# EDAPINENUT/CBGBench

Measured on AMD Instinct MI355X. Metric: denoising graph-steps/s (pocket+ligand graphs x reverse-diffusion steps per second), higher is better.
Workload: dtype f32; 1 GPU; configs/denovo targetdiff sampling, BASELINE configs[1] job: 100 pockets x 10 samples = 1000 graphs per GPU, 3 resident batch(es) of <= 340; N_rec~U[350,650], N_lig~U[10,45], k=32, 9 layers; bench step = 1 reverse-diffusion step of the job at each of 5 time blocks; graphs_per_gpu=1000, nodes_per_gpu=521351, denoising_steps_per_bench_step=5, graph_steps_per_bench_step_per_gpu=5000, ranks_seen=1, launch=stream launches, streams=3, edge_workgroups=256, devices_by_uuid=1

## Files before the change

cbgbench_amd/_native.py:

```python
import contextlib
import contextvars
import ctypes
import os

import torch

from .build import LIBPATH, XCHECK_LIBPATH

_LIB = None
_XLIB = None

_vp, _i, _sz = ctypes.c_void_p, ctypes.c_int, ctypes.c_size_t
FWD_H_ON_SOURCES, FWD_GEN_IS_LIGAND = 1, 2
ABI_VERSION = 6

EXPORTS = {
    "cbgx_abi_version": (_i, []),
    "cbgx_last_error": (ctypes.c_char_p, []),
    "cbgx_set_edge_workgroups": (_i, [_i]),
    "cbgx_packed_weights_floats": (_sz, [_i, _i]),
    "cbgx_pack_weights": (_i, [ctypes.POINTER(_vp), _i, _i, _i, _vp, _vp]),
    "cbgx_workspace_bytes": (_sz, [_i, _i]),
    "cbgx_unitransformer_forward": (_i, [_vp, _i, _i, _vp, _vp, _vp, _vp, _vp, _i, _i, _vp, _vp, _vp, _vp, _sz, _vp]),
    "cbgx_unitransformer_forward_v2": (_i, [_vp, _i, _i, _vp, _vp, _vp, _vp, _vp, _i, _i, _vp, _vp, _vp, ctypes.c_uint, _vp, _sz, _vp]),
    "cbgx_unitransformer_forward_cached": (_i, [_vp, _i, _i, _vp, _vp, _vp, _vp, _vp, _i, _i, _vp, _vp, _vp, _vp, _vp, _vp,
                                                _vp, _vp, _vp, ctypes.c_uint, _vp, _sz, _vp]),
    "cbgx_knn_graph": (_i, [_vp, _vp, _i, _i, _i, _vp, _vp, _vp]),
    "cbgx_edge_gate": (_i, [_vp, _vp, _vp, _vp, _i, _vp, _vp]),
    "cbgx_x2h_attention": (_i, [_vp, _i, _vp, _vp, _vp, _vp, _vp, _vp, _i, _vp, _vp, _sz, _vp]),
    "cbgx_h2x_attention": (_i, [_vp, _i, _vp, _vp, _vp, _vp, _vp, _vp, _vp, _i, _vp, _vp, _vp, _sz, _vp]),
    "cbgx_h2x_attention_v2": (_i, [_vp, _i, _vp, _vp, _vp, _vp, _vp, _vp, _vp, _i, _vp, _vp, ctypes.c_uint, _vp, _sz, _vp]),
    "cbgx_classifier": (_i, [_vp, _i, _i, _vp, _i, _vp, _vp, _sz, _vp]),
    "cbgx_node_stage": (_i, [_vp, _i, _i, _vp, _vp, _i, _vp, _vp, _i, _vp, _vp, _vp, _vp]),
    "cbgx_packed_h2x_stack_floats": (_sz, [_i]),
    "cbgx_pack_h2x_stack": (_i, [ctypes.POINTER(_vp), _i, _i, _vp, _vp]),
    "cbgx_h2x_stack_forward": (_i, [_vp, _i, _vp, _vp, _vp, _vp, _vp, _i, _i, _vp, _vp, _sz, _vp]),
    "cbgx_h2x_stack_forward_v2": (_i, [_vp, _i, _vp, _vp, _vp, _vp, _vp, _i, _i, _vp, ctypes.c_uint, _vp, _sz, _vp]),
    "cbgx_targetdiff_prologue": (_i, [_vp, _vp, _vp, _i, _i, _vp, _vp, _vp, _vp, _vp, _vp, _vp]),
    "cbgx_targetdiff_epilogue": (_i, [_vp, _vp, _vp, _vp, _vp, _vp, _i, _i, _i, _i, ctypes.POINTER(_vp), _vp, _vp, _vp, _vp,
                                      _vp, _vp]),
    "cbgx_targetdiff_step_boundary": (_i, [_vp, _vp, _vp, _vp, _vp, _vp, _i, _i, _i, _i, ctypes.POINTER(_vp), _vp, _vp, _vp, _vp,
                                           _vp, _vp, _vp, _vp, _vp, _vp, _vp]),
    "cbgx_targetdiff_prologue_traj": (_i, [_vp, _vp, _vp, _vp, _i, _i, _vp, _vp, _vp, _vp, _vp, _vp, _vp]),
    "cbgx_targetdiff_epilogue_traj": (_i, [_vp, _vp, _vp, _vp, _vp, _vp, _i, _i, _vp, ctypes.POINTER(_vp), _vp, _vp, _vp]),
    "cbgx_diffbp_epilogue": (_i, [_vp, _vp, _vp, _vp, _vp, _vp, _vp, _vp, _vp, _i, _i, _i, _i, _i, _vp, _vp, _i, _vp, _vp, _vp,
                                  _vp, _vp]),
    "cbgx_diffsbdd_step": (_i, [_vp, _vp, _vp, _vp, _vp, _vp, _vp, _vp, _i, _i, _i, ctypes.c_float, ctypes.c_float,
                                ctypes.c_float, _i, _i, _vp, _vp, _vp, _vp, _vp, _vp, _vp, _vp, _vp, _vp, _vp, _vp, _vp]),
    "cbgx_noise_fill": (_i, [_vp, _vp, _i, _i, _i, _i, _i, _i, _vp, _vp, _vp]),
    "cbgx_targetdiff_epilogue_rng": (_i, [_vp, _vp, _vp, _vp, _vp, _vp, _i, _i, _i, _i, ctypes.POINTER(_vp), _vp, _vp, _vp, _i, _i,
                                          _vp, _vp, _vp, _vp]),
    "cbgx_targetdiff_step_boundary_rng": (_i, [_vp, _vp, _vp, _vp, _vp, _vp, _i, _i, _i, _i, ctypes.POINTER(_vp), _vp, _vp, _vp, _i,
                                               _i, _vp, _vp, _vp, _vp, _vp, _vp, _vp, _vp, _vp]),
    "cbgx_targetdiff_epilogue_traj_rng": (_i, [_vp, _vp, _vp, _vp, _vp, _vp, _i, _i, _vp, ctypes.POINTER(_vp), _vp, _vp, _vp, _i, _i,
                                               _vp]),
    "cbgx_targetdiff_train_noise": (_i, [_vp, _vp, _vp, _vp, _vp, _i, _i, _vp, _vp, _vp, _vp, _vp, _vp, _vp, _vp, _vp]),
    "cbgx_train_noise_draw": (_i, [_vp, _vp, _i, _i, _i, _i, _vp, _vp, _vp, _vp, _i, _i, _i, _vp]),
    "cbgx_targetdiff_train_noise_rng": (_i, [_vp, _vp, _vp, _vp, _i, _i, _vp, _vp, _vp, _vp, _vp, _i, _i, _i, _vp, _vp, _vp, _vp, _vp,
                                             _vp]),
    "cbgx_train_transform": (_i, [_vp] * 5 + [_i, _i, _i, ctypes.c_float, _i, _vp] + [_vp] * 4),
    "cbgx_train_transform_rng": (_i, [_vp] * 5 + [_i, _i, _i, ctypes.c_float, _i, _vp, _i] + [_vp] * 4),
    "cbgx_train_transform_choose": (_i, [_vp] * 8 + [_i] * 5 + [ctypes.c_float, _i, _vp] + [_vp] * 6),
    "cbgx_train_transform_choose_rng": (_i, [_vp] * 7 + [_i] * 5 + [ctypes.c_float, _i, _vp, _i] + [_vp] * 6),
    "cbgx_targetdiff_loss": (_i, [_vp, _vp, _vp, _vp, _vp, _vp, _vp, _vp, _vp, _i, _i, _i, ctypes.POINTER(_vp), _vp, _vp, _vp,
                                  _vp, _vp, _vp]),
    "cbgx_targetdiff_loss_backward": (_i, [_vp, _vp, _vp, _i, _i, _i, _vp, _vp, _vp, _vp, _vp]),
    "cbgx_diffsbdd_train_noise": (_i, [_vp] * 9 + [_i] * 4 + [_vp, _vp, _i] + [_vp] * 5),
    "cbgx_diffsbdd_loss": (_i, [_vp] * 7 + [_i] * 4 + [_vp] * 8),
    "cbgx_compose_plan": (_i, [_vp, _vp, _i, _i, _i] + [_vp] * 7),
    "cbgx_embed_compose": (_i, [_vp] * 8 + [_i] * 5 + [ctypes.POINTER(_vp)] + [_vp] * 5),
    "cbgx_embed_compose_backward": (_i, [_vp, _vp, _i, _i, _i, _i, _vp, _i, _vp, _vp]),
    "cbgx_diffbp_loss": (_i, [_vp] * 13 + [_i, _i, _i, _i, _vp, _vp, ctypes.c_float, ctypes.c_float] + [_vp] * 9 + [_vp]),
    "cbgx_diffbp_loss_knn": (_i, [_vp] * 13 + [_i, _i, _i, _i, _vp, _vp, ctypes.c_float, ctypes.c_float] + [_vp] * 9 + [_vp, _vp]),
    "cbgx_diffbp_train_noise": (_i, [_vp] * 8 + [_i] * 4 + [_vp, _i, _i] + [_vp] * 6 + [_vp]),
    "cbgx_train_tape_bytes": (_sz, [_i, _i]),
    "cbgx_train_workspace_bytes": (_sz, [_i]),
    "cbgx_unitransformer_forward_train": (_i, [_vp, _i, _i, _vp, _vp, _vp, _vp, _vp, _i, _i, _vp, _vp, _vp, _vp, _sz,
                                               _vp, _sz, _vp]),
    "cbgx_unitransformer_forward_train_ex": (_i, [_vp, _i, _i, _vp, _vp, _vp, _vp, _vp, _i, _i, _vp, _vp, _vp, ctypes.c_uint, _vp, _sz,
                                                  _vp, _sz, _vp]),
    "cbgx_unitransformer_backward": (_i, [_vp, _i, _i, _vp, _sz, _vp, _vp, _i, _vp, _vp, _vp, ctypes.POINTER(_vp), _i,
                                          _vp, _vp, _sz, _vp]),
    "cbgx_unitransformer_backward_ex": (_i, [_vp, _i, _i, _vp, _sz, _vp, _vp, _i, _vp, _vp, _vp, ctypes.POINTER(_vp), _i,
                                             _vp, _vp, _vp, _sz, _vp]),
    "cbgx_x2h_attention_backward": (_i, [_vp, _i, _vp, _vp, _vp, _vp, _vp, _vp, _i, _vp, _vp, _vp, _vp,
                                         ctypes.POINTER(_vp), _vp, _sz, _vp]),
    "cbgx_h2x_attention_backward": (_i, [_vp, _i, _vp, _vp, _vp, _vp, _vp, _vp, _vp, _i, _vp, _vp, _vp, _vp,
                                         ctypes.POINTER(_vp), _vp, _sz, _vp]),
    "cbgx_h2x_stack_tape_bytes": (_sz, [_i, _i]),
    "cbgx_h2x_stack_forward_train": (_i, [_vp, _i, _vp, _vp, _vp, _vp, _vp, _i, _i, _vp, _vp, _sz, _vp, _sz, _vp]),
    "cbgx_h2x_stack_backward": (_i, [_vp, _i, _vp, _sz, _vp, _vp, _vp, _i, _vp, ctypes.POINTER(_vp), _i, _vp, _vp, _sz,
                                     _vp]),
    "cbgx_h2x_stack_backward_ex": (_i, [_vp, _i, _vp, _sz, _vp, _vp, _vp, _i, _vp, ctypes.POINTER(_vp), _i, _vp, _vp, _vp,
                                        _sz, _vp]),
    "cbgx_ligand_geometry": (_i, [_vp, _vp, _vp, _i, _vp, _vp, _vp, _i, _i, _vp, _vp, _vp, _vp]),
    "cbgx_ligand_geometry_tables": (_i, [_vp] * 7),
    "cbgx_ligand_bonds_count": (_i, [_vp, _vp, _vp, _i, _i, _vp, _vp, _vp, _vp]),
    "cbgx_ligand_bonds_fill": (_i, [_vp, _vp, _vp, _i, _i, _vp, _i, _vp, _vp, _vp, _vp]),
    "cbgx_ligand_rings": (_i, [_vp, _i, _i, _vp, _vp, _i, _vp, _vp, _vp]),
    "cbgx_ligand_aromatic": (_i, [_vp, _vp, _vp, _vp, _i, _i, _vp, _vp, _i, _vp, _vp, _vp, _vp]),
    "cbgx_ligand_pair_hist": (_i, [_vp, _vp, _vp, _i, _i, _vp, _i, _vp, _i, _vp, _vp]),
    "cbgx_ligand_angles": (_i, [_vp, _vp, _vp, _i, _i, _vp, _vp, _vp, _i, _vp, _i, _vp, _i, _vp, _vp, _vp, _vp, _vp]),
    "cbgx_profile_begin": (_i, [_i]),
    "cbgx_profile_end": (_i, [ctypes.POINTER(ctypes.c_double), ctypes.POINTER(_i), _i]),
}

XCHECK_EXPORTS = {
    "cbgx_debug_set_edge_kernel": (_i, [_i]),
    "cbgx_debug_gate_backward": (_i, [_vp, _vp, _vp, _vp, _i, _vp, _vp, _vp, ctypes.POINTER(_vp), _vp, _vp, _sz, _vp]),
    "cbgx_debug_forward_view": (_i, [_vp, _i, ctypes.POINTER(_vp)]),
}

PROFILE_CLASSES = ("knn", "gate", "node_gemm", "node_query", "edge_x2h", "edge_h2x", "edge_x2h_listed",
                   "edge_x2h_bwd", "edge_h2x_bwd", "train_gemm", "edge_x2h_bwd_listed", "edge_rows_reduce")


class NativeError(RuntimeError):
    pass


def _load(path, extra=None):
    dll = ctypes.CDLL(path)
    exports = dict(EXPORTS)
    exports.update(extra or {})
    for name, (res, args) in exports.items():
        fn = getattr(dll, name)
        fn.restype = res
        fn.argtypes = args
    if dll.cbgx_abi_version() != ABI_VERSION:
        raise NativeError(f"{path}: ABI version {dll.cbgx_abi_version()} != {ABI_VERSION} (stale build? run `python -m cbgbench_amd.build`)")
    return dll


_OVERRIDE = contextvars.ContextVar("cbgx_library_override", default=None)


def lib():
    global _LIB
    over = _OVERRIDE.get()
    if over is not None:
        return over
    if _LIB is None:
        path = os.environ.get("CBGX_LIBRARY", LIBPATH)
        if not os.path.exists(path):
            raise NativeError(
                f"{path} not found: build it with `python -m cbgbench_amd.build` "
                "(there is no CPU / PyTorch fallback for the message-passing path)")
        _LIB = _load(path)
    return _LIB


@contextlib.contextmanager
def first_generation_kernels(impl=1):
    global _XLIB
    if _XLIB is None:
        if not os.path.exists(XCHECK_LIBPATH):
            raise NativeError(f"{XCHECK_LIBPATH} not found: build it with `python -m cbgbench_amd.build`")
        _XLIB = _load(XCHECK_LIBPATH, XCHECK_EXPORTS)
    old = _XLIB.cbgx_debug_set_edge_kernel(impl)
    token = _OVERRIDE.set(_XLIB)
    try:
        yield _XLIB
    finally:
        _OVERRIDE.reset(token)
        _XLIB.cbgx_debug_set_edge_kernel(old)


def check(rc, what):
    if rc != 0:
        msg = lib().cbgx_last_error().decode(errors="replace")
        if rc == -1:
            raise ValueError(f"{what}: {msg}")
        raise NativeError(f"{what} failed ({rc}): {msg}")


def ptr(t):
    if t is None:
        return None
    if not t.is_contiguous():
        raise ValueError("libcbgx needs contiguous tensors")
    return ctypes.c_void_p(t.data_ptr())


def current_stream(device):
    return ctypes.c_void_p(torch.cuda.current_stream(device).cuda_stream)



def version(t):
    if t.is_inference():
        return _NeverEqual()
    return t._version


class _NeverEqual:
    __slots__ = ()

    def __eq__(self, other):
        return False

    def __ne__(self, other):
        return True

    def __hash__(self):
        return id(self)
```

cbgbench_amd/csrc/api.hip:

```cpp
#include <hip/hip_runtime.h>

#include <cmath>
#include <cstdarg>
#include <cstdio>
#include <cstring>
#include <cstdlib>
#include <vector>

#include "../../include/cbgx.h"
#ifdef CBGX_XCHECK
#include "../../include/cbgx_xcheck.h"
#endif
#include "kernels.h"
#include "layout.h"
#include "workspace.h"

using namespace cbgx;

static thread_local char g_err[512] = "";

namespace cbgx {
int set_error(int code, const char* fmt, ...) {
    va_list ap;
    va_start(ap, fmt);
    vsnprintf(g_err, sizeof(g_err), fmt, ap);
    va_end(ap);
    return code;
}
}
static constexpr auto& fail = cbgx::set_error;

#define HIP_TRY(expr)                                                                          \
    do {                                                                                       \
        hipError_t _e = (expr);                                                                \
        if (_e != hipSuccess) return fail(CBGX_E_HIP, "%s: %s", #expr, hipGetErrorString(_e)); \
    } while (0)

struct Workspace {
    int32_t *nbr, *deg;
    float* e_w;
    NodeBufs set[3];
    NodeList act;
    NodeList A1, A2, A3;
    NodeList D1, S1, D2, S2;
    NodeList all_gen, all_pp, D2_gen, D2_pp, A1_gen, A1_pp, A2_gen, A2_pp;
    NodeList empty;
    uint8_t *fa1, *fa2, *fa3, *fD1, *fD2, *fS1, *fS2;
    uint8_t* d1flag;
    float *hbuf[2], *xbuf[2];
    unsigned* newmask;
    void* counters;
    size_t counters_bytes, total;
};

static Workspace carve(void* base, int n) {
    Workspace w;
    Carver c(base);
    size_t N = (size_t)(n > 0 ? n : 1);
    w.nbr = c.take<int32_t>(N * KNN * 4);
    w.deg = c.take<int32_t>(N * 4);
    w.e_w = c.take<float>(N * KNN * 4);
    for (NodeBufs& b : w.set) {
        b.P = c.take<float>(N * PROW * 4);
        b.Qt = c.take<float>(N * HEADS * H * 4);
        b.q = c.take<float>(N * H * 4);
    }
    for (NodeList* l : {&w.act, &w.A1, &w.A2, &w.A3, &w.D1, &w.S1, &w.D2, &w.S2}) l->rows = c.take<int>(N * 4);
    for (float*& h : w.hbuf) h = c.take<float>(N * H * 4);
    for (float*& x : w.xbuf) x = c.take<float>(N * 3 * 4);
    for (NodeList* l : {&w.all_gen, &w.all_pp, &w.D2_gen, &w.D2_pp, &w.A1_gen, &w.A1_pp, &w.A2_gen, &w.A2_pp})
        l->rows = c.take<int>(N * 4);
    w.empty.rows = w.all_pp.rows;
    w.newmask = c.take<unsigned>(N * 4);
    const size_t fl = align_up(N);
    w.counters_bytes = 8 * fl + 256 + 256 + 256 + 4 * 128 + 256;
    uint8_t* f = c.take<uint8_t>(w.counters_bytes);
    w.counters = f;
    w.d1flag = f; w.fa1 = w.d1flag + fl; w.fa2 = w.fa1 + fl; w.fa3 = w.fa2 + fl;
    w.fD1 = w.fa3 + fl; w.fD2 = w.fD1 + fl; w.fS1 = w.fD2 + fl; w.fS2 = w.fS1 + fl;
    auto counts = [&](size_t region, std::initializer_list<NodeList*> lists) {
        int k = 0;
        for (NodeList* l : lists) l->count = (int*)(f + 8 * fl + region + 64 * k++);
    };
    counts(0, {&w.act});
    counts(256, {&w.A1, &w.A2, &w.A3});
    counts(512, {&w.D1, &w.S1, &w.D2, &w.S2});
    counts(768, {&w.all_gen, &w.all_pp, &w.D2_gen, &w.D2_pp, &w.A1_gen, &w.A1_pp, &w.A2_gen, &w.A2_pp});
    counts(768 + 4 * 128, {&w.empty});
    w.total = c.off;
    return w;
}

static int carve_checked(const char* who, void* workspace, size_t workspace_bytes, int n_nodes, Workspace& w) {
    w = carve(workspace, n_nodes);
    if (workspace_bytes < w.total) return fail(CBGX_E_WORKSPACE, "%s: workspace %zu < %zu", who, workspace_bytes, w.total);
    return CBGX_OK;
}

constexpr int MAX_AUX = 8;
struct AuxTable {
    int dev = -1;
    int n = 0;
    int next_victim = 0;
    AuxStream e[MAX_AUX];
};
static thread_local AuxTable g_aux_table;
namespace cbgx {
AuxStream* aux_for(hipStream_t caller) {
    int dev = -1;
    if (hipGetDevice(&dev) != hipSuccess) return nullptr;
    AuxTable& t = g_aux_table;
    if (t.n && t.dev != dev) return nullptr;
    for (int k = 0; k < t.n; ++k)
        if (t.e[k].owner == caller) return &t.e[k];
    if (t.n == MAX_AUX) {
        AuxStream& e = t.e[t.next_victim];
        t.next_victim = (t.next_victim + 1) % MAX_AUX;
        e.owner = caller;
        return &e;
    }
    AuxStream a;
    a.owner = caller;
    static const bool low = [] { const char* e = getenv("CBGX_AUX_PRIORITY"); return e && e[0] == 'l'; }();
    int least = 0, greatest = 0;
    if (low && hipDeviceGetStreamPriorityRange(&least, &greatest) == hipSuccess && least != greatest) {
        if (hipStreamCreateWithPriority(&a.s, hipStreamNonBlocking, least) != hipSuccess) return nullptr;
    } else if (hipStreamCreateWithFlags(&a.s, hipStreamNonBlocking) != hipSuccess) return nullptr;
    if (hipEventCreateWithFlags(&a.fork, hipEventDisableTiming) != hipSuccess ||
        hipEventCreateWithFlags(&a.join, hipEventDisableTiming) != hipSuccess ||
        hipEventCreateWithFlags(&a.done[0], hipEventDisableTiming) != hipSuccess ||
        hipEventCreateWithFlags(&a.done[1], hipEventDisableTiming) != hipSuccess) {
        (void)hipStreamDestroy(a.s);
        return nullptr;
    }
    t.dev = dev;
    t.e[t.n] = a;
    return &t.e[t.n++];
}
}

extern "C" {

int cbgx_abi_version(void) { return CBGX_ABI_VERSION; }
const char* cbgx_last_error(void) { return g_err; }

#ifdef CBGX_XCHECK
int cbgx_debug_set_edge_kernel(int impl) {
    if (impl < 0 || impl > 2) return fail(CBGX_E_INVALID, "debug_set_edge_kernel: impl must be 0 (current), 1 (valu) or 2 (mfma, second-generation x2h backward)");
    int old = g_edge_impl;
    g_edge_impl = impl;
    return old;
}

int cbgx_debug_forward_view(void* workspace, int n_nodes, void** out) {
    if (!workspace || !out || n_nodes < 1) return fail(CBGX_E_INVALID, "debug_forward_view: bad argument");
    const Workspace w = carve(workspace, n_nodes);
    int k = 0;
    out[k++] = w.nbr; out[k++] = w.deg; out[k++] = w.e_w; out[k++] = w.d1flag; out[k++] = w.fD1;
    const NodeList lists[] = {w.act,     w.A1,     w.A2,     w.A3,    w.D1,     w.S1,    w.D2,     w.S2,
                              w.all_gen, w.all_pp, w.D2_gen, w.D2_pp, w.A1_gen, w.A1_pp, w.A2_gen, w.A2_pp};
    for (const NodeList& l : lists) { out[k++] = l.rows; out[k++] = l.count; }
    static_assert(sizeof(lists) / sizeof(lists[0]) == CBGX_FWD_VIEW_LISTS, "cbgx_debug_forward_view: list count");
    static_assert(CBGX_FWD_VIEW_PTRS == 5 + 2 * 16, "cbgx_debug_forward_view: list count");
    return k == CBGX_FWD_VIEW_PTRS ? CBGX_OK : fail(CBGX_E_INVALID, "debug_forward_view: %d pointers", k);
}
#endif

int cbgx_set_edge_workgroups(int n) { return set_edge_workgroup_limit(n); }

size_t cbgx_packed_weights_floats(int num_layers, int num_classes) {
    if (num_layers < 0 || num_classes < 1 || num_classes > CBGX_MAX_CLASSES) return 0;
    return packed_floats(num_layers, num_classes);
}

static thread_local PackBatch g_pack;
static int flush_pack(hipStream_t s) {
    if (g_pack.n) {
        HIP_TRY(launch_pack_copy_multi(g_pack, s));
        g_pack.n = 0;
    }
    return CBGX_OK;
}
static int queue_pack(const float* src, int ld, int off, int tr, float* dst, int dld, int rows, int cols, hipStream_t s) {
    if (g_pack.n == PACK_MAX) { int rc = flush_pack(s); if (rc) return rc; }
    g_pack.p[g_pack.n++] = PackPiece{src, dst, ld, off, tr, dld, rows, cols};
    return CBGX_OK;
}
#define CP(src, ld, off, tr, dst, dld, rows, cols)                                 \
    do {                                                                           \
        int _rc = queue_pack(src, ld, off, tr, dst, dld, rows, cols, s);           \
        if (_rc) return _rc;                                                       \
    } while (0)

static int pack_gate_section(const float* const* t, float* packed, hipStream_t s) {
    CP(t[0], G, 0, 0, packed + GATE_W1, G, GH, G);
    CP(t[1], GH, 0, 0, packed + GATE_B1, GH, 1, GH);
    CP(t[2], GH, 0, 0, packed + GATE_LNG, GH, 1, GH);
    CP(t[3], GH, 0, 0, packed + GATE_LNB, GH, 1, GH);
    CP(t[4], GH, 0, 0, packed + GATE_W2, GH, 1, GH);
    CP(t[5], 1, 0, 0, packed + GATE_B2, 1, 1, 1);
    HIP_TRY(launch_pack_gate_img(t[0], t[1], t[2], t[3], t[4], packed + GATE_IMG, s));
    return flush_pack(s);
}

struct BlockRef { const float* const* p; int blk; float* a; };

static int queue_block_copies(const BlockRef& r, hipStream_t s) {
    const float* const* p = r.p;
    float* a = r.a;
    const int blk = r.blk;
    const float *wk0 = p[0], *bk0 = p[1], *gk = p[2], *bek = p[3], *wk1 = p[4];
    const float *wv0 = p[6], *bv0 = p[7], *gv = p[8], *bev = p[9], *wv1 = p[10], *bv1 = p[11];
    const float *wq0 = p[12], *bq0 = p[13], *gq = p[14], *beq = p[15], *wq1 = p[16], *bq1 = p[17];
    CP(wk0, KV_IN, NT + NT * G, 1, a + A_WN + 0 * H, PROW, H, H);
    CP(wv0, KV_IN, NT + NT * G, 1, a + A_WN + 1 * H, PROW, H, H);
    CP(wk0, KV_IN, NT + NT * G + H, 1, a + A_WN + 2 * H, PROW, H, H);
    CP(wv0, KV_IN, NT + NT * G + H, 1, a + A_WN + 3 * H, PROW, H, H);
    CP(wq0, H, 0, 1, a + A_WN + 4 * H, PROW, H, H);
    CP(bk0, H, 0, 0, a + A_BN + 0 * H, H, 1, H);
    CP(bv0, H, 0, 0, a + A_BN + 1 * H, H, 1, H);
    CP(bq0, H, 0, 0, a + A_BN + 4 * H, H, 1, H);
    CP(wk0, KV_IN, 0, 1, a + A_WT, 2 * H, NT, H);
    CP(wv0, KV_IN, 0, 1, a + A_WT + H, 2 * H, NT, H);
    CP(wk0, KV_IN, NT, 1, a + A_WR, 2 * H, NT * G, H);
    CP(wv0, KV_IN, NT, 1, a + A_WR + H, 2 * H, NT * G, H);
    CP(gk, H, 0, 0, a + A_LNK_G, H, 1, H);
    CP(bek, H, 0, 0, a + A_LNK_B, H, 1, H);
    CP(gv, H, 0, 0, a + A_LNV_G, H, 1, H);
    CP(bev, H, 0, 0, a + A_LNV_B, H, 1, H);
    CP(gq, H, 0, 0, a + A_LNQ_G, H, 1, H);
    CP(beq, H, 0, 0, a + A_LNQ_B, H, 1, H);
    CP(wq1, H, 0, 1, a + A_WQ1T, H, H, H);
    CP(bq1, H, 0, 0, a + A_BQ1, H, 1, H);
    CP(wk1, H, 0, 0, a + A_WBK, H, H, H);
    CP(wk1, H, 0, 1, a + A_WBKT, H, H, H);
    CP(wq1, H, 0, 0, a + A_WQ1O, H, H, H);
    for (int ty = 0; ty < NT; ++ty) {
        CP(wk0, KV_IN, NT + G * ty, 0, a + A_WRT + (size_t)ty * 2 * H * 32, 32, H, G);
        CP(wv0, KV_IN, NT + G * ty, 0, a + A_WRT + ((size_t)ty * 2 * H + H) * 32, 32, H, G);
    }
    float* img = a + A_IMG;
    CP(gk, H, 0, 0, img + IMG_LN + 0 * H, H, 1, H);
    CP(bek, H, 0, 0, img + IMG_LN + 1 * H, H, 1, H);
    CP(gv, H, 0, 0, img + IMG_LN + 2 * H, H, 1, H);
    CP(bev, H, 0, 0, img + IMG_LN + 3 * H, H, 1, H);
    if (blk == 0) {
        CP(wv1, H, 0, 1, a + A_WBV, H, H, H);
        CP(bv1, H, 0, 0, a + A_BBV, H, 1, H);
    } else {
        CP(wv1, H, 0, 0, a + A_WBV, H, HEADS, H);
        CP(bv1, HEADS, 0, 0, a + A_BBV, HEADS, 1, HEADS);
    }
    return CBGX_OK;
}

static int queue_centred_copies(const BlockRef& r, hipStream_t s) {
    float* a = r.a;
    CP(a + A_WAKC, KV_IN, NT, 1, a + A_WRC, 2 * H, NT * G, H);
    CP(a + A_WAVC, KV_IN, NT, 1, a + A_WRC + H, 2 * H, NT * G, H);
    return CBGX_OK;
}

static int pack_attention_blocks(const BlockRef* refs, int n_blocks, hipStream_t s) {
    for (int k0 = 0; k0 < n_blocks; k0 += PACK_BLOCKS_MAX) {
        const int nb = n_blocks - k0 < PACK_BLOCKS_MAX ? n_blocks - k0 : PACK_BLOCKS_MAX;
        PackBlocks pb;
        memset(&pb, 0, sizeof(pb));
        pb.n = nb;
        for (int k = 0; k < nb; ++k) {
            const BlockRef& r = refs[k0 + k];
            pb.wk0[k] = r.p[0]; pb.bk0[k] = r.p[1]; pb.wk1[k] = r.p[4];
            pb.wv0[k] = r.p[6]; pb.bv0[k] = r.p[7]; pb.wv1[k] = r.p[10];
            pb.wq0[k] = r.p[12]; pb.bq0[k] = r.p[13]; pb.wq1[k] = r.p[16];
            pb.att[k] = r.a;
            pb.nsrc[k][0] = r.a + A_WAKC; pb.nsrc[k][1] = r.a + A_WAVC; pb.nsrc[k][2] = r.a + A_WAKC; pb.nsrc[k][3] = r.a + A_WAVC;
            pb.nsrc[k][4] = r.p[12];
            pb.x2h[k] = r.blk == 0;
            int rc = queue_block_copies(r, s);
            if (rc) return rc;
        }
        { int rc = flush_pack(s); if (rc) return rc; }
        HIP_TRY(launch_pack_stage1(pb, s));
        for (int k = 0; k < nb; ++k) { int rc = queue_centred_copies(refs[k0 + k], s); if (rc) return rc; }
        { int rc = flush_pack(s); if (rc) return rc; }
        HIP_TRY(launch_pack_stage2(pb, s));
    }
    return CBGX_OK;
}

int cbgx_pack_weights(const float* const* t, int num_tensors, int L, int C, float* packed, void* stream) {
    if (C > CBGX_MAX_CLASSES) return fail(CBGX_E_INVALID, "pack_weights: num_classes=%d > %d", C, CBGX_MAX_CLASSES);
    if (!t || !packed) return fail(CBGX_E_INVALID, "pack_weights: NULL pointer");
    if (L < 1 || C < 1) return fail(CBGX_E_INVALID, "pack_weights: num_layers=%d num_classes=%d", L, C);
    if (num_tensors != 6 + 36 * L + 4)
        return fail(CBGX_E_INVALID, "pack_weights: expected %d tensors, got %d", 6 + 36 * L + 4, num_tensors);
    for (int i = 0; i < num_tensors; ++i)
        if (!t[i]) return fail(CBGX_E_INVALID, "pack_weights: tensor %d is NULL", i);
    hipStream_t s = (hipStream_t)stream;
    HIP_TRY(hipMemsetAsync(packed, 0, packed_floats(L, C) * sizeof(float), s));
    { int rc = pack_gate_section(t, packed, s); if (rc) return rc; }
    {
        std::vector<BlockRef> refs;
        for (int l = 0; l < L; ++l)
            for (int blk = 0; blk < 2; ++blk)
                refs.push_back(BlockRef{t + 6 + 36 * l + 18 * blk , blk, packed + (blk == 0 ? x2h_off(l) : h2x_off(l))});
        int rc = pack_attention_blocks(refs.data(), (int)refs.size(), s);
        if (rc) return rc;
    }
    const float* const* c = t + 6 + 36 * L;
    float* cp = packed + cls_off(L);
    CP(c[0], H, 0, 1, cp + C_W0T, H, H, H);
    CP(c[1], H, 0, 0, cp + C_B0, H, 1, H);
    CP(c[2], H, 0, 1, cp + C_W1T, C, H, C);
    CP(c[3], C, 0, 0, cp + cls_b1(C), C, 1, C);
    return flush_pack(s);
}

size_t cbgx_packed_h2x_stack_floats(int num_layers) {
    if (num_layers < 1) return 0;
    return GATE_SIZE + (size_t)num_layers * ATT_SIZE;
}

int cbgx_pack_h2x_stack(const float* const* t, int num_tensors, int L, float* packed, void* stream) {
    if (!t || !packed) return fail(CBGX_E_INVALID, "pack_h2x_stack: NULL pointer");
    if (L < 1 || num_tensors != 6 + 18 * L)
        return fail(CBGX_E_INVALID, "pack_h2x_stack: expected %d tensors for %d layers, got %d", 6 + 18 * L, L, num_tensors);
    for (int i = 0; i < num_tensors; ++i)
        if (!t[i]) return fail(CBGX_E_INVALID, "pack_h2x_stack: tensor %d is NULL", i);
    hipStream_t s = (hipStream_t)stream;
    HIP_TRY(hipMemsetAsync(packed, 0, cbgx_packed_h2x_stack_floats(L) * sizeof(float), s));
    { int rc = pack_gate_section(t, packed, s); if (rc) return rc; }
    std::vector<BlockRef> refs;
    for (int l = 0; l < L; ++l) refs.push_back(BlockRef{t + 6 + 18 * l, 1, packed + GATE_SIZE + (size_t)l * ATT_SIZE});
    { int rc = pack_attention_blocks(refs.data(), (int)refs.size(), s); if (rc) return rc; }
    return flush_pack(s);
}

static bool h2x_lig_selected(unsigned flags) { return (flags & CBGX_FWD_GEN_IS_LIGAND) && g_edge_impl != 1 && h2x_fold_enabled(); }

int cbgx_h2x_stack_forward_v2(const float* packed, int num_layers, const float* x, const float* h,
                              const int32_t* graph_ptr, const uint8_t* lig_flag, const uint8_t* gen_flag, int n_nodes,
                              int n_graphs, float* x_out, unsigned flags, void* workspace, size_t workspace_bytes, void* stream) {
    if (n_nodes < 0 || n_graphs < 0 || num_layers < 1) return fail(CBGX_E_INVALID, "h2x_stack: bad sizes");
    if (flags & ~CBGX_FWD_GEN_IS_LIGAND) return fail(CBGX_E_INVALID, "h2x_stack: unknown flags 0x%x", flags);
    if (n_nodes == 0) return CBGX_OK;
    if (!packed || !x || !h || !graph_ptr || !lig_flag || !gen_flag || !x_out || !workspace)
        return fail(CBGX_E_INVALID, "h2x_stack: NULL pointer");
    Workspace w;
    if (int rc = carve_checked("h2x_stack", workspace, workspace_bytes, n_nodes, w)) return rc;
    hipStream_t s = (hipStream_t)stream;
    HIP_TRY(launch_build_active(gen_flag, n_nodes, w.act, s));
    if (g_edge_impl == 1) {
        HIP_TRY(launch_knn(x, graph_ptr, n_graphs, n_nodes, w.nbr, w.deg, s));
        HIP_TRY(launch_gate(packed, x, w.nbr, w.deg, n_nodes, w.e_w, s));
    } else {
        HIP_TRY(launch_knn_reg(x, graph_ptr, n_graphs, n_nodes, w.nbr, w.deg, s, w.act));
        HIP_TRY(launch_gate_mfma(packed, x, w.nbr, w.deg, n_nodes, w.e_w, s, w.act));
    }
    RowList src;
    if (g_edge_impl != 1) {
        HIP_TRY(launch_mark_seed(gen_flag, gen_flag, n_nodes, w.fa1, s));
        HIP_TRY(walk_receptive_field(w.fa1, w.act, w.nbr, w.deg, n_nodes, {w.A1}, s));
        src = w.A1;
    }
    const Graph g{w.nbr, w.deg, w.e_w, lig_flag, gen_flag, n_nodes};
    const float* xc = x;
    for (int l = 0; l < num_layers; ++l) {
        float* xn = (l == num_layers - 1) ? x_out : w.xbuf[l & 1];
        HIP_TRY(launch_attention(false, packed + GATE_SIZE + (size_t)l * ATT_SIZE, g, xc, h, w.set[0], xn, nullptr, w.act, src, s,
                                 h2x_lig_selected(flags)));
        xc = xn;
    }
    return CBGX_OK;
}

int cbgx_h2x_stack_forward(const float* packed, int num_layers, const float* x, const float* h,
                           const int32_t* graph_ptr, const uint8_t* lig_flag, const uint8_t* gen_flag, int n_nodes,
                           int n_graphs, float* x_out, void* workspace, size_t workspace_bytes, void* stream) {
    return cbgx_h2x_stack_forward_v2(packed, num_layers, x, h, graph_ptr, lig_flag, gen_flag, n_nodes, n_graphs, x_out, 0u, workspace,
                                     workspace_bytes, stream);
}

size_t cbgx_workspace_bytes(int n_nodes, int n_graphs) {
    (void)n_graphs;
    return carve(nullptr, n_nodes).total;
}

int cbgx_knn_graph(const float* x, const int32_t* graph_ptr, int n_graphs, int n_nodes, int k, int32_t* nbr,
                   int32_t* deg, void* stream) {
    if (k != KNN) return fail(CBGX_E_INVALID, "knn_graph: only k=%d is supported (got %d)", KNN, k);
    if (n_nodes < 0 || n_graphs < 0) return fail(CBGX_E_INVALID, "knn_graph: negative size");
    if (n_nodes == 0) return CBGX_OK;
    if (!x || !graph_ptr || !nbr || !deg || n_graphs < 1) return fail(CBGX_E_INVALID, "knn_graph: NULL pointer");
    HIP_TRY(launch_knn(x, graph_ptr, n_graphs, n_nodes, nbr, deg, (hipStream_t)stream));
    return CBGX_OK;
}

int cbgx_edge_gate(const float* packed, const float* x, const int32_t* nbr, const int32_t* deg, int n_nodes,
                   float* e_w, void* stream) {
    if (n_nodes == 0) return CBGX_OK;
    if (!packed || !x || !nbr || !deg || !e_w || n_nodes < 0) return fail(CBGX_E_INVALID, "edge_gate: bad argument");
    HIP_TRY(launch_gate(packed, x, nbr, deg, n_nodes, e_w, (hipStream_t)stream));
    return CBGX_OK;
}

int cbgx_x2h_attention(const float* packed, int layer, const float* x, const float* h, const int32_t* nbr,
                       const int32_t* deg, const uint8_t* lig_flag, const float* e_w, int n_nodes, float* h_out,
                       void* workspace, size_t workspace_bytes, void* stream) {
    if (n_nodes == 0) return CBGX_OK;
    if (!packed || !x || !h || !nbr || !deg || !lig_flag || !e_w || !h_out || !workspace || layer < 0 || n_nodes < 0)
        return fail(CBGX_E_INVALID, "x2h_attention: bad argument");
    Workspace w;
    if (int rc = carve_checked("x2h_attention", workspace, workspace_bytes, n_nodes, w)) return rc;
    const NodeBufs& b = w.set[0];
    const Graph g{nbr, deg, e_w, lig_flag, nullptr, n_nodes};
    const float* att = packed + x2h_off(layer);
    hipStream_t s = (hipStream_t)stream;
    if (g_edge_impl == 1) {
        HIP_TRY(launch_attention(true, att, g, x, h, b, h_out, nullptr, {}, {}, s));
        return CBGX_OK;
    }
    HIP_TRY(launch_mark_from_nbr(lig_flag, nbr, deg, n_nodes, w.d1flag, s));
    HIP_TRY(launch_split_list({}, n_nodes, w.d1flag, w.all_gen, w.all_pp, s));
    NodeStageOpts o;
    o.large_lists = true;
    o.fold = w.all_gen;
    HIP_TRY(launch_node_mfma(att, h, lig_flag, n_nodes, b, {}, {}, s, o));
    HIP_TRY(launch_edge_x2h_dual(att, g, x, h, b, h_out, w.all_pp, w.all_gen, true, s));
    return CBGX_OK;
}

int cbgx_h2x_attention_v2(const float* packed, int layer, const float* x, const float* h, const int32_t* nbr,
                          const int32_t* deg, const uint8_t* lig_flag, const uint8_t* gen_flag, const float* e_w,
                          int n_nodes, float* x_out, float* delta_x, unsigned flags, void* workspace, size_t workspace_bytes,
                          void* stream) {
    if (flags & ~CBGX_FWD_GEN_IS_LIGAND) return fail(CBGX_E_INVALID, "h2x_attention: unknown flags 0x%x", flags);
    if (n_nodes == 0) return CBGX_OK;
    if (!packed || !x || !h || !nbr || !deg || !lig_flag || !gen_flag || !e_w || !x_out || !workspace || layer < 0 ||
        n_nodes < 0)
        return fail(CBGX_E_INVALID, "h2x_attention: bad argument");
    Workspace w;
    if (int rc = carve_checked("h2x_attention", workspace, workspace_bytes, n_nodes, w)) return rc;
    const Graph g{nbr, deg, e_w, lig_flag, gen_flag, n_nodes};
    HIP_TRY(launch_build_active(gen_flag, n_nodes, w.act, (hipStream_t)stream));
    HIP_TRY(launch_attention(false, packed + h2x_off(layer), g, x, h, w.set[0], x_out, delta_x, w.act, {}, (hipStream_t)stream,
                             h2x_lig_selected(flags)));
    return CBGX_OK;
}

int cbgx_h2x_attention(const float* packed, int layer, const float* x, const float* h, const int32_t* nbr,
                       const int32_t* deg, const uint8_t* lig_flag, const uint8_t* gen_flag, const float* e_w,
                       int n_nodes, float* x_out, float* delta_x, void* workspace, size_t workspace_bytes,
                       void* stream) {
    return cbgx_h2x_attention_v2(packed, layer, x, h, nbr, deg, lig_flag, gen_flag, e_w, n_nodes, x_out, delta_x, 0u, workspace,
                                 workspace_bytes, stream);
}

int cbgx_node_stage(const float* packed, int layer, int x2h, const float* h, const uint8_t* lig_flag, int n_nodes,
                    const int32_t* rows, const int32_t* n_rows, int q_direct, float* P, float* q, float* Qt, void* stream) {
    if (n_nodes == 0) return CBGX_OK;
    if (!packed || !h || !lig_flag || !P || !q || !Qt || layer < 0 || n_nodes < 0 || (rows == nullptr) != (n_rows == nullptr))
        return fail(CBGX_E_INVALID, "node_stage: bad argument");
    NodeStageOpts o;
    o.large_lists = true;
    o.q_direct = q_direct != 0;
    HIP_TRY(launch_node_mfma(packed + (x2h ? x2h_off(layer) : h2x_off(layer)), h, lig_flag, n_nodes, NodeBufs{P, q, Qt},
                             RowList{rows, n_rows}, {}, (hipStream_t)stream, o));
    return CBGX_OK;
}

static int classifier_head(const float* packed, int num_layers, int num_classes, const float* h, int n_nodes, float* hidden,
                           float* logits, RowList rows, hipStream_t s) {
    const float* c = packed + cls_off(num_layers);
    HIP_TRY(launch_node_gemm(h, H, c + C_W0T, c + C_B0, hidden, H, n_nodes, H, 1, s, rows));
    HIP_TRY(launch_node_gemm(hidden, H, c + C_W1T, c + cls_b1(num_classes), logits, num_classes, n_nodes, num_classes, 0, s, rows));
    return CBGX_OK;
}

int cbgx_classifier(const float* packed, int num_layers, int num_classes, const float* h, int n_nodes, float* logits,
                    void* workspace, size_t workspace_bytes, void* stream) {
    if (num_classes > CBGX_MAX_CLASSES) return fail(CBGX_E_INVALID, "classifier: num_classes=%d > %d", num_classes, CBGX_MAX_CLASSES);
    if (n_nodes == 0) return CBGX_OK;
    if (!packed || !h || !logits || !workspace || num_layers < 0 || num_classes < 1 || n_nodes < 0)
        return fail(CBGX_E_INVALID, "classifier: bad argument");
    Workspace w;
    if (int rc = carve_checked("classifier", workspace, workspace_bytes, n_nodes, w)) return rc;
    return classifier_head(packed, num_layers, num_classes, h, n_nodes, w.set[0].P, logits, {}, (hipStream_t)stream);
}

struct LayerPlan {
    NodeList dst, src;
    NodeList gen, pp;
    bool full_layer;
    const uint8_t* fold_flag;
};

struct Forward {
    const float* packed; int num_layers, num_classes; const float *x, *h; const int32_t* graph_ptr; const uint8_t *lig_flag, *gen_flag;
    int n_nodes, n_graphs; float *x_out, *h_out, *logits;
    const float *static_h1, *static_h2; const int32_t *static_nbr, *static_deg; const float *static_ew, *static_r32sq;
    unsigned flags; void* workspace; size_t workspace_bytes; hipStream_t s;
    Workspace w;
    Graph graph;
    bool cached, graph_cached, prune, dual;
    bool h2x_lig;
    std::vector<LayerPlan> plan;
};

static int forward_graph_stage(const Forward& f) {
    const Workspace& w = f.w;
    const int n_nodes = f.n_nodes, n_graphs = f.n_graphs;
    hipStream_t s = f.s;
    if (!f.graph_cached) {
        HIP_TRY(launch_knn(f.x, f.graph_ptr, n_graphs, n_nodes, w.nbr, w.deg, s));
        HIP_TRY(launch_gate(f.packed, f.x, w.nbr, w.deg, n_nodes, w.e_w, s));
        return CBGX_OK;
    }
    HIP_TRY(launch_graph_cache_begin(f.x, f.graph_ptr, n_graphs, f.lig_flag, f.static_r32sq, n_nodes, w.fD1, w.D1.rows, w.D1.count,
                                     f.static_nbr, f.static_deg, f.static_ew, w.nbr, w.deg, w.e_w, f.static_h1, f.static_h2, w.hbuf[0],
                                     w.hbuf[1], s));
    static const int merge_gate = [] { const char* e = getenv("CBGX_MERGE_GATE"); return e ? atoi(e) : 1; }();
    if (merge_gate && n_nodes <= GRAPH_LISTS_MAX_NODES) {
        HIP_TRY(launch_knn_merge_gate(f.packed, f.x, f.graph_ptr, n_graphs, n_nodes, f.lig_flag, f.static_nbr, f.static_deg, f.static_ew,
                                      w.nbr, w.deg, w.e_w, s, w.D1));
    } else {
        const bool carry = merge_gate != 0;
        HIP_TRY(launch_knn_merge(f.x, f.graph_ptr, n_graphs, n_nodes, f.lig_flag, f.static_nbr, f.static_deg, w.nbr, w.deg, s, w.D1,
                                 carry ? f.static_ew : nullptr, carry ? w.e_w : nullptr, carry ? w.newmask : nullptr));
        HIP_TRY(launch_gate_mfma(f.packed, f.x, w.nbr, w.deg, n_nodes, w.e_w, s, w.D1, carry ? w.newmask : nullptr));
    }
    return CBGX_OK;
}

static int forward_list_stage(const Forward& f) {
    const Workspace& w = f.w;
    hipStream_t s = f.s;
    const bool per_graph = f.n_nodes <= GRAPH_LISTS_MAX_NODES && g_edge_impl != 1;
    const GraphFlags gf{f.gen_flag, f.lig_flag, f.graph_cached ? w.fD1 : w.d1flag, w.d1flag, w.fa1, w.fa2, w.fa3, w.fD2, w.fS1, w.fS2};
    const uint8_t* flag_ptr[GF_COUNT] = {f.gen_flag, f.lig_flag, gf.D1, w.d1flag, w.fa1, w.fa2, w.fa3, w.fD2, w.fS1, w.fS2};
    ListJobs jobs;
    GraphListJobs gjobs;
    memset(&jobs, 0, sizeof(jobs));
    memset(&gjobs, 0, sizeof(gjobs));
    bool jobs_overflow = false;
    auto add = [&](int flag, int flag2, int want2, NodeList l) {
        if (jobs.n_jobs >= LIST_JOBS_MAX) { jobs_overflow = true; return; }
        const int k = jobs.n_jobs++;
        jobs.flag[k] = flag == GF_ALL ? nullptr : flag_ptr[flag]; jobs.flag2[k] = flag2 == GF_ALL ? nullptr : flag_ptr[flag2];
        jobs.want2[k] = want2; jobs.list[k] = l.rows; jobs.count[k] = l.count;
        gjobs.flag[k] = (signed char)flag; gjobs.flag2[k] = (signed char)flag2; gjobs.want2[k] = (signed char)want2;
        gjobs.list[k] = l.rows; gjobs.count[k] = l.count;
        gjobs.n_jobs = jobs.n_jobs;
    };
    auto pair = [&](int flag, NodeList gen, NodeList pp) { add(flag, GF_d1, 1, gen); add(flag, GF_d1, 0, pp); };
    add(GF_GEN, GF_ALL, 0, w.act);
    add(GF_a1, GF_ALL, 0, w.A1);
    if (f.prune) {
        add(GF_a2, GF_ALL, 0, w.A2);
        add(GF_a3, GF_ALL, 0, w.A3);
    }
    if (f.cached) {
        if (!f.graph_cached) add(GF_d1, GF_ALL, 0, w.D1);
        add(GF_D2, GF_ALL, 0, w.D2);
        add(GF_S1, GF_ALL, 0, w.S1);
        add(GF_S2, GF_ALL, 0, w.S2);
    }
    if (f.dual) {
        pair(GF_ALL, w.all_gen, w.all_pp);
        if (f.cached) pair(GF_D2, w.D2_gen, w.D2_pp);
        if (f.prune) { pair(GF_a1, w.A1_gen, w.A1_pp); pair(GF_a2, w.A2_gen, w.A2_pp); }
    }
    if (jobs_overflow) return fail(CBGX_E_INVALID, "forward: more than %d node lists (LIST_JOBS_MAX)", LIST_JOBS_MAX);
    if (per_graph) {
        HIP_TRY(launch_graph_lists(f.gen_flag, f.lig_flag, f.graph_cached ? w.fD1 : nullptr, w.nbr, w.deg, f.graph_ptr, f.n_graphs, gjobs,
                                   f.cached, f.prune, w.d1flag, s));
    } else {
        HIP_TRY(launch_list_level(gf, w.nbr, w.deg, f.n_nodes, 0, f.cached, f.prune, s));
        if (f.cached || f.prune) {
            HIP_TRY(launch_list_level(gf, w.nbr, w.deg, f.n_nodes, 1, f.cached, f.prune, s));
            HIP_TRY(launch_list_level(gf, w.nbr, w.deg, f.n_nodes, 2, f.cached, f.prune, s));
        }
        HIP_TRY(launch_build_lists(jobs, f.n_nodes, s));
    }
    return CBGX_OK;
}

static void plan_layers(Forward& f) {
    const Workspace& w = f.w;
    const int L = f.num_layers;
    const NodeList every{nullptr, nullptr};
    f.plan.assign(L, LayerPlan{every, every, w.all_gen, w.all_pp, true, w.d1flag});
    if (f.cached) {
        f.plan[0] = LayerPlan{w.D1, w.S1, w.D1, w.empty, false, nullptr};
        f.plan[1] = LayerPlan{w.D2, w.S2, w.D2_gen, w.D2_pp, false, w.d1flag};
    }
    if (f.prune) {
        f.plan[L - 2] = LayerPlan{w.A2, w.A3, w.A2_gen, w.A2_pp, false, w.d1flag};
        f.plan[L - 1] = LayerPlan{w.A1, w.A2, w.A1_gen, w.A1_pp, false, w.d1flag};
    }
}

static hipError_t begin_layer(const Forward& f, int l, float*& hn, float*& xn) {
    const bool last = l == f.num_layers - 1;
    hn = (last && f.h_out) ? f.h_out : f.w.hbuf[l & 1];
    xn = last ? f.x_out : f.w.xbuf[l & 1];
    if (!f.cached || l >= 2 || f.graph_cached) return hipSuccess;
    return hipMemcpyAsync(hn, l == 0 ? f.static_h1 : f.static_h2, (size_t)f.n_nodes * H * sizeof(float), hipMemcpyDeviceToDevice, f.s);
}

static hipError_t edge_x2h(const Forward& f, int l, const NodeBufs& b, const float* xc, const float* hc, float* hn) {
    const LayerPlan& p = f.plan[l];
    return launch_edge_x2h_dual(f.packed + x2h_off(l), f.graph, xc, hc, b, hn, p.pp, p.gen, p.full_layer, f.s);
}
static hipError_t node_x2h(const Forward& f, int l, const NodeBufs& b, const float* h_in, hipStream_t on) {
    const LayerPlan& p = f.plan[l];
    NodeStageOpts o;
    o.large_lists = true;
    o.fold = p.gen;
    o.q_direct = node_qdirect_enabled();
    return launch_node_mfma(f.packed + x2h_off(l), h_in, f.lig_flag, f.n_nodes, b, p.dst, p.src, on, o);
}
static hipError_t block_h2x(const Forward& f, int l, const NodeBufs& b, const float* xc, const float* hn, float* xn) {
    return launch_attention(false, f.packed + h2x_off(l), f.graph, xc, hn, b, xn, nullptr, f.w.act, f.w.A1, f.s, f.h2x_lig);
}

static int forward_fused(const Forward& f) {
    const Workspace& w = f.w;
    hipStream_t s = f.s;
    auto add_x2h = [&](NodeStageJobs& jobs, int l) {
        const LayerPlan& p = f.plan[l];
        add_node_stage_jobs(jobs, f.packed + x2h_off(l), w.set[l & 1], p.dst, p.src, p.fold_flag);
    };
    NodeStageJobs jobs;
    jobs.n = 0;
    add_x2h(jobs, 0);
    HIP_TRY(launch_node_stage_jobs(jobs, f.h, f.lig_flag, f.n_nodes, s));
    const float *xc = f.x, *hc = f.h;
    for (int l = 0; l < f.num_layers; ++l) {
        float *hn, *xn;
        HIP_TRY(begin_layer(f, l, hn, xn));
        HIP_TRY(edge_x2h(f, l, w.set[l & 1], xc, hc, hn));
        jobs.n = 0;
        add_node_stage_jobs(jobs, f.packed + h2x_off(l), w.set[2], w.act, w.A1, nullptr, f.h2x_lig);
        if (l + 1 < f.num_layers) add_x2h(jobs, l + 1);
        HIP_TRY(launch_node_stage_jobs(jobs, hn, f.lig_flag, f.n_nodes, s));
        if (f.h2x_lig) HIP_TRY(launch_edge_h2x_lig(f.packed + h2x_off(l), f.graph, xc, hn, w.set[2], xn, nullptr, w.act, s));
        else HIP_TRY(launch_edge_mfma(false, f.packed + h2x_off(l), f.graph, xc, hn, w.set[2], xn, nullptr, w.act, s));
        xc = xn;
        hc = hn;
    }
    return CBGX_OK;
}

static int forward_two_streams(const Forward& f, AuxStream* aux) {
    hipStream_t s = f.s;
    HIP_TRY(node_x2h(f, 0, f.w.set[0], f.h, s));
    const float *xc = f.x, *hc = f.h;
    for (int l = 0; l < f.num_layers; ++l) {
        float *hn, *xn;
        HIP_TRY(begin_layer(f, l, hn, xn));
        if (l > 0) HIP_TRY(hipStreamWaitEvent(s, aux->join, 0));
        HIP_TRY(edge_x2h(f, l, f.w.set[l & 1], xc, hc, hn));
        if (l + 1 < f.num_layers) {
            HIP_TRY(hipEventRecord(aux->fork, s));
            HIP_TRY(hipStreamWaitEvent(aux->s, aux->fork, 0));
            HIP_TRY(node_x2h(f, l + 1, f.w.set[(l + 1) & 1], hn, aux->s));
            HIP_TRY(hipEventRecord(aux->join, aux->s));
        }
        HIP_TRY(block_h2x(f, l, f.w.set[2], xc, hn, xn));
        xc = xn;
        hc = hn;
    }
    return CBGX_OK;
}

static int forward_serial(const Forward& f) {
    const Workspace& w = f.w;
    const NodeBufs& b = w.set[0];
    const float *xc = f.x, *hc = f.h;
    for (int l = 0; l < f.num_layers; ++l) {
        float *hn, *xn;
        HIP_TRY(begin_layer(f, l, hn, xn));
        if (f.dual) {
            HIP_TRY(node_x2h(f, l, b, hc, f.s));
            HIP_TRY(edge_x2h(f, l, b, xc, hc, hn));
        } else {
            const LayerPlan& p = f.plan[l];
            HIP_TRY(launch_attention(true, f.packed + x2h_off(l), f.graph, xc, hc, b, hn, nullptr, p.dst, p.src, f.s));
        }
        HIP_TRY(block_h2x(f, l, b, xc, hn, xn));
        xc = xn;
        hc = hn;
    }
    return CBGX_OK;
}

static int forward_impl(Forward f) {
    if (f.n_nodes < 0 || f.n_graphs < 0 || f.num_layers < 1) return fail(CBGX_E_INVALID, "forward: bad sizes");
    if (f.flags & ~(CBGX_FWD_H_ON_SOURCES | CBGX_FWD_GEN_IS_LIGAND)) return fail(CBGX_E_INVALID, "forward: unknown flags 0x%x", f.flags);
    if (f.num_classes > CBGX_MAX_CLASSES) return fail(CBGX_E_INVALID, "forward: num_classes=%d > %d", f.num_classes, CBGX_MAX_CLASSES);
    if (f.n_nodes == 0) return CBGX_OK;
    if (!f.packed || !f.x || !f.h || !f.graph_ptr || !f.lig_flag || !f.gen_flag || !f.x_out || !f.workspace)
        return fail(CBGX_E_INVALID, "forward: NULL pointer");
    if (f.logits && f.num_classes < 1) return fail(CBGX_E_INVALID, "forward: num_classes=%d", f.num_classes);
    if (int rc = carve_checked("forward", f.workspace, f.workspace_bytes, f.n_nodes, f.w)) return rc;
    f.graph = Graph{f.w.nbr, f.w.deg, f.w.e_w, f.lig_flag, f.gen_flag, f.n_nodes};
    HIP_TRY(hipMemsetAsync(f.w.counters, 0, f.w.counters_bytes, f.s));
    f.cached = f.static_h1 && f.static_h2 && f.num_layers >= 4;
    f.graph_cached = f.cached && f.static_nbr && f.static_deg && f.static_ew && f.static_r32sq && g_edge_impl != 1;
    f.prune = (f.h_out == nullptr || (f.flags & CBGX_FWD_H_ON_SOURCES)) && f.num_layers >= 3;
    f.dual = g_edge_impl != 1;
    f.h2x_lig = h2x_lig_selected(f.flags);
    if (int rc = forward_graph_stage(f)) return rc;
    if (int rc = forward_list_stage(f)) return rc;
    plan_layers(f);
    static const bool overlap_env = [] { const char* e = getenv("CBGX_OVERLAP"); return !e || atoi(e) != 0; }();
    AuxStream* aux = (overlap_env && g_edge_impl != 1 && !profile_is_on() && f.num_layers > 1) ? aux_for(f.s) : nullptr;
    static const int fuse_rows = [] { const char* e = getenv("CBGX_FUSE_ROWS"); return e ? atoi(e) : NODE_STAGE_MAX_ROWS; }();
    int rc;
    if (f.dual && f.num_layers > 1 && f.n_nodes <= fuse_rows && f.n_nodes <= NODE_STAGE_MAX_ROWS) rc = forward_fused(f);
    else if (aux) rc = forward_two_streams(f, aux);
    else rc = forward_serial(f);
    if (rc || !f.logits) return rc;
    return classifier_head(f.packed, f.num_layers, f.num_classes, f.h_out ? f.h_out : f.w.hbuf[(f.num_layers - 1) & 1], f.n_nodes,
                           f.w.set[0].P, f.logits, f.prune ? RowList(f.w.A1) : RowList(), f.s);
}

int cbgx_unitransformer_forward_v2(const float* packed, int num_layers, int num_classes, const float* x, const float* h,
                                   const int32_t* graph_ptr, const uint8_t* lig_flag, const uint8_t* gen_flag,
                                   int n_nodes, int n_graphs, float* x_out, float* h_out, float* logits, unsigned flags,
                                   void* workspace, size_t workspace_bytes, void* stream) {
    return forward_impl(Forward{packed, num_layers, num_classes, x, h, graph_ptr, lig_flag, gen_flag, n_nodes, n_graphs, x_out,
                                h_out, logits, nullptr, nullptr, nullptr, nullptr, nullptr, nullptr, flags, workspace, workspace_bytes,
                                (hipStream_t)stream});
}

int cbgx_unitransformer_forward(const float* packed, int num_layers, int num_classes, const float* x, const float* h,
                                const int32_t* graph_ptr, const uint8_t* lig_flag, const uint8_t* gen_flag,
                                int n_nodes, int n_graphs, float* x_out, float* h_out, float* logits, void* workspace,
                                size_t workspace_bytes, void* stream) {
    return cbgx_unitransformer_forward_v2(packed, num_layers, num_classes, x, h, graph_ptr, lig_flag, gen_flag, n_nodes, n_graphs,
                                          x_out, h_out, logits, 0u, workspace, workspace_bytes, stream);
}

int cbgx_unitransformer_forward_cached(const float* packed, int num_layers, int num_classes, const float* x,
                                       const float* h, const int32_t* graph_ptr, const uint8_t* lig_flag,
                                       const uint8_t* gen_flag, int n_nodes, int n_graphs, const float* static_h1,
                                       const float* static_h2, const int32_t* static_nbr, const int32_t* static_deg,
                                       const float* static_ew, const float* static_r32sq, float* x_out, float* h_out,
                                       float* logits, unsigned flags, void* workspace, size_t workspace_bytes, void* stream) {
    if (!static_h1 || !static_h2) return fail(CBGX_E_INVALID, "forward_cached: NULL static context");
    return forward_impl(Forward{packed, num_layers, num_classes, x, h, graph_ptr, lig_flag, gen_flag, n_nodes, n_graphs, x_out,
                                h_out, logits, static_h1, static_h2, static_nbr, static_deg, static_ew, static_r32sq, flags, workspace,
                                workspace_bytes, (hipStream_t)stream});
}

static int noise_args(const char* who, const uint64_t* keys, const int32_t* lig_graph, bool need_graph, const int32_t* lig_ptr,
                      int n_graphs, int purpose_base) {
    if (!keys || !lig_ptr || (need_graph && !lig_graph)) return fail(CBGX_E_INVALID, "%s: NULL pointer (noise)", who);
    if (n_graphs < 1) return fail(CBGX_E_INVALID, "%s: n_graphs=%d", who, n_graphs);
    if (purpose_base < 0 || purpose_base % CBGX_NOISE_PURPOSE_STRIDE)
        return fail(CBGX_E_INVALID, "%s: purpose_base=%d is not a non-negative multiple of %d", who, purpose_base,
                    CBGX_NOISE_PURPOSE_STRIDE);
    return CBGX_OK;
}

struct StepArgs {
    const char* who = "";
    const float *x_den = nullptr, *logits = nullptr, *x_lig = nullptr, *c_lig = nullptr;
    const int32_t* lig_rows = nullptr;
    const uint8_t* gen_lig = nullptr;
    int n_lig = 0, num_classes = 0, t = 0, num_timesteps = 0;
    const float* const* tables = nullptr;
    float *x_next = nullptr, *c_next = nullptr;
    int32_t* v_next = nullptr;
    bool traj = false;
    int32_t* t_dev = nullptr;
    bool counter = false;
    StepNoise noise;
    bool boundary = false;
    const float *lig_emb_w = nullptr, *lig_emb_b = nullptr, *ind_w = nullptr, *ind_b = nullptr;
    float *x = nullptr, *h = nullptr;
};

static int step_prologue(const char* who, const float* x_lig, const float* c_lig, bool traj, const int32_t* t_dev,
                         const int32_t* lig_rows, int n_lig, int num_classes, const float* lig_emb_w, const float* lig_emb_b,
                         const float* ind_w, const float* ind_b, float* x, float* h, void* stream) {
    if (n_lig == 0) return CBGX_OK;
    if (n_lig < 0 || num_classes < 1 || num_classes > 32) return fail(CBGX_E_INVALID, "%s: bad sizes", who);
    if (!x_lig || !c_lig || (traj && !t_dev) || !lig_rows || !lig_emb_w || !lig_emb_b || !ind_w || !ind_b || !x || !h)
        return fail(CBGX_E_INVALID, "%s: NULL pointer", who);
    HIP_TRY(launch_step_prologue(x_lig, c_lig, lig_rows, n_lig, num_classes, lig_emb_w, lig_emb_b, ind_w, ind_b, x, h,
                                 (hipStream_t)stream, t_dev));
    return CBGX_OK;
}

static int step_epilogue_check(const StepArgs& a) {
    if (a.n_lig < 0 || a.num_classes < 1 || a.num_classes > 32 || (!a.traj && (a.t < 0 || a.t >= a.num_timesteps))) {
        if (a.traj) return fail(CBGX_E_INVALID, "%s: bad sizes", a.who);
        return fail(CBGX_E_INVALID, "%s: bad sizes (n_lig=%d C=%d t=%d T=%d)", a.who, a.n_lig, a.num_classes, a.t, a.num_timesteps);
    }
    if (!a.x_den || !a.logits || !a.lig_rows || !a.x_lig || !a.c_lig || !a.gen_lig || !a.tables || !a.x_next || !a.c_next ||
        (a.traj && !a.t_dev) || (!a.counter && (!a.noise.eps || !a.noise.u)) ||
        (a.boundary && (!a.lig_emb_w || !a.lig_emb_b || !a.ind_w || !a.ind_b || !a.x || !a.h)))
        return fail(CBGX_E_INVALID, "%s: NULL pointer", a.who);
    for (int i = 0; i < 7; ++i)
        if (!a.tables[i]) return fail(CBGX_E_INVALID, "%s: table %d is NULL", a.who, i);
    if (a.counter)
        return noise_args(a.who, a.noise.keys, a.noise.lig_graph, true, a.noise.lig_ptr, a.noise.n_graphs, a.noise.purpose_base);
    return CBGX_OK;
}

static int step_epilogue(const StepArgs& a, void* stream) {
    if (a.n_lig == 0) return CBGX_OK;
    if (int rc = step_epilogue_check(a)) return rc;
    const float log_c = (float)log((double)a.num_classes);
    if (a.boundary)
        HIP_TRY(launch_step_boundary(a.x_den, a.logits, a.lig_rows, a.x_lig, a.c_lig, a.gen_lig, a.n_lig, a.num_classes, a.t, a.tables,
                                     log_c, a.noise, a.x_next, a.c_next, a.lig_emb_w, a.lig_emb_b, a.ind_w, a.ind_b, a.x, a.h,
                                     (hipStream_t)stream));
    else
        HIP_TRY(launch_step_epilogue(a.x_den, a.logits, a.lig_rows, a.x_lig, a.c_lig, a.gen_lig, a.n_lig, a.num_classes, a.t, a.tables,
                                     log_c, a.noise, a.x_next, a.c_next, a.v_next, (hipStream_t)stream, a.t_dev));
    return CBGX_OK;
}

int cbgx_targetdiff_prologue(const float* x_lig, const float* c_lig, const int32_t* lig_rows, int n_lig, int num_classes,
                             const float* lig_emb_w, const float* lig_emb_b, const float* ind_w, const float* ind_b,
                             float* x, float* h, void* stream) {
    return step_prologue("prologue", x_lig, c_lig, false, nullptr, lig_rows, n_lig, num_classes, lig_emb_w, lig_emb_b, ind_w, ind_b, x, h,
                         stream);
}

int cbgx_targetdiff_epilogue(const float* x_den, const float* logits, const int32_t* lig_rows, const float* x_lig,
                             const float* c_lig, const uint8_t* gen_lig, int n_lig, int num_classes, int t,
                             int num_timesteps, const float* const* tables, const float* eps, const float* u,
                             float* x_next, float* c_next, int32_t* v_next, void* stream) {
    StepArgs a;
    a.who = "epilogue";
    a.x_den = x_den, a.logits = logits, a.lig_rows = lig_rows, a.x_lig = x_lig, a.c_lig = c_lig, a.gen_lig = gen_lig;
    a.n_lig = n_lig, a.num_classes = num_classes, a.t = t, a.num_timesteps = num_timesteps, a.tables = tables;
    a.noise.eps = eps, a.noise.u = u;
    a.x_next = x_next, a.c_next = c_next, a.v_next = v_next;
    return step_epilogue(a, stream);
}

int cbgx_targetdiff_step_boundary(const float* x_den, const float* logits, const int32_t* lig_rows, const float* x_lig,
                                  const float* c_lig, const uint8_t* gen_lig, int n_lig, int num_classes, int t,
                                  int num_timesteps, const float* const* tables, const float* eps, const float* u,
                                  float* x_next, float* c_next, const float* lig_emb_w, const float* lig_emb_b,
                                  const float* ind_w, const float* ind_b, float* x, float* h, void* stream) {
    StepArgs a;
    a.who = "step_boundary";
    a.x_den = x_den, a.logits = logits, a.lig_rows = lig_rows, a.x_lig = x_lig, a.c_lig = c_lig, a.gen_lig = gen_lig;
    a.n_lig = n_lig, a.num_classes = num_classes, a.t = t, a.num_timesteps = num_timesteps, a.tables = tables;
    a.noise.eps = eps, a.noise.u = u;
    a.x_next = x_next, a.c_next = c_next;
    a.boundary = true, a.lig_emb_w = lig_emb_w, a.lig_emb_b = lig_emb_b, a.ind_w = ind_w, a.ind_b = ind_b, a.x = x, a.h = h;
    return step_epilogue(a, stream);
}

int cbgx_diffbp_epilogue(const float* x_den, const float* x_com, const float* x_in, const float* logits,
                         const int32_t* lig_rows, const int32_t* lig_ptr, const float* x_lig, const float* c_lig,
                         const uint8_t* gen_lig, int n_lig, int n_graphs, int num_classes, int t, int num_timesteps,
                         const float* alphas_cumprod, const float* betas, int absorbing_state, const float* eps,
                         const float* u, float* x_next, float* c_next, void* stream) {
    if (n_lig == 0 || n_graphs == 0) return CBGX_OK;
    if (n_lig < 0 || n_graphs < 0 || num_classes < 1 || num_classes > 32 || t < 0 || t >= num_timesteps ||
        absorbing_state < 0 || absorbing_state >= num_classes)
        return fail(CBGX_E_INVALID, "diffbp_epilogue: bad sizes (n_lig=%d B=%d C=%d t=%d T=%d)", n_lig, n_graphs, num_classes, t,
                    num_timesteps);
    if (!x_den || !x_com || !x_in || !logits || !lig_rows || !lig_ptr || !x_lig || !c_lig || !gen_lig || !alphas_cumprod ||
        !betas || !eps || !u || !x_next || !c_next)
        return fail(CBGX_E_INVALID, "diffbp_epilogue: NULL pointer");
    HIP_TRY(launch_diffbp_epilogue(x_den, x_com, x_in, logits, lig_rows, lig_ptr, x_lig, c_lig, gen_lig, n_graphs, num_classes, t,
                                   num_timesteps, alphas_cumprod, betas, absorbing_state, eps, u, x_next, c_next,
                                   (hipStream_t)stream));
    return CBGX_OK;
}

int cbgx_diffsbdd_step(const float* x_den, const float* logits, const int32_t* graph_ptr, const int32_t* lig_rows,
                       const int32_t* lig_ptr, const uint8_t* lig_flag, const float* x_lig, const float* c_lig, int n_lig,
                       int n_graphs, int num_classes, float inv_alpha, float coef, float sigma, int update_positions,
                       int update_types, const float* eps_x, const float* eps_c, const float* lig_emb_w,
                       const float* lig_emb_b, const float* ind_w, const float* ind_b, float* x_next, float* c_next,
                       float* x, float* h, float* shift, float* frame_shift, void* stream) {
    if (n_lig == 0 || n_graphs == 0) return CBGX_OK;
    if (n_lig < 0 || n_graphs < 0 || num_classes < 1 || num_classes > 32)
        return fail(CBGX_E_INVALID, "diffsbdd_step: bad sizes (n_lig=%d B=%d C=%d)", n_lig, n_graphs, num_classes);
    if (!x_den || !logits || !graph_ptr || !lig_rows || !lig_ptr || !lig_flag || !x_lig || !c_lig || !lig_emb_w || !lig_emb_b ||
        !ind_w || !ind_b || !x_next || !c_next || !x || !h || (update_positions && !eps_x) || (update_types && !eps_c))
        return fail(CBGX_E_INVALID, "diffsbdd_step: NULL pointer");
    HIP_TRY(launch_diffsbdd_step(x_den, logits, graph_ptr, lig_rows, lig_ptr, lig_flag, x_lig, c_lig, n_graphs, num_classes,
                                 inv_alpha, coef, sigma, update_positions, update_types, eps_x, eps_c, lig_emb_w, lig_emb_b, ind_w,
                                 ind_b, x_next, c_next, x, h, shift, frame_shift, (hipStream_t)stream));
    return CBGX_OK;
}

int cbgx_targetdiff_prologue_traj(const float* traj_x, const float* traj_c, const int32_t* t_dev, const int32_t* lig_rows,
                                  int n_lig, int num_classes, const float* lig_emb_w, const float* lig_emb_b,
                                  const float* ind_w, const float* ind_b, float* x, float* h, void* stream) {
    return step_prologue("prologue_traj", traj_x, traj_c, true, t_dev, lig_rows, n_lig, num_classes, lig_emb_w, lig_emb_b, ind_w, ind_b,
                         x, h, stream);
}

int cbgx_targetdiff_epilogue_traj(const float* x_den, const float* logits, const int32_t* lig_rows, float* traj_x,
                                  float* traj_c, const uint8_t* gen_lig, int n_lig, int num_classes, int32_t* t_dev,
                                  const float* const* tables, const float* eps, const float* u, void* stream) {
    StepArgs a;
    a.who = "epilogue_traj";
    a.x_den = x_den, a.logits = logits, a.lig_rows = lig_rows, a.x_lig = traj_x, a.c_lig = traj_c, a.gen_lig = gen_lig;
    a.n_lig = n_lig, a.num_classes = num_classes, a.tables = tables;
    a.noise.eps = eps, a.noise.u = u;
    a.x_next = traj_x, a.c_next = traj_c;
    a.traj = true, a.t_dev = t_dev;
    return step_epilogue(a, stream);
}

int cbgx_noise_fill(const uint64_t* stream_keys, const int32_t* lig_ptr, int n_graphs, int n_lig, int cols, int uniform,
                    int purpose, int step, const int32_t* step_dev, float* out, void* stream) {
    if (n_lig == 0 || n_graphs == 0 || cols == 0) return CBGX_OK;
    if (n_lig < 0 || n_graphs < 0 || cols < 0 || purpose < 0 || (!step_dev && step < 0))
        return fail(CBGX_E_INVALID, "noise_fill: bad sizes (n_lig=%d B=%d cols=%d purpose=%d step=%d)", n_lig, n_graphs, cols, purpose,
                    step);
    if (!stream_keys || !lig_ptr || !out) return fail(CBGX_E_INVALID, "noise_fill: NULL pointer");
    HIP_TRY(launch_noise_fill(stream_keys, lig_ptr, n_graphs, n_lig, cols, uniform, (uint32_t)purpose, step, step_dev, out,
                              (hipStream_t)stream));
    return CBGX_OK;
}

int cbgx_targetdiff_epilogue_rng(const float* x_den, const float* logits, const int32_t* lig_rows, const float* x_lig,
                                 const float* c_lig, const uint8_t* gen_lig, int n_lig, int num_classes, int t,
                                 int num_timesteps, const float* const* tables, const uint64_t* stream_keys,
                                 const int32_t* lig_graph, const int32_t* lig_ptr, int n_graphs, int purpose_base, float* x_next,
                                 float* c_next, int32_t* v_next, void* stream) {
    StepArgs a;
    a.who = "epilogue_rng";
    a.x_den = x_den, a.logits = logits, a.lig_rows = lig_rows, a.x_lig = x_lig, a.c_lig = c_lig, a.gen_lig = gen_lig;
    a.n_lig = n_lig, a.num_classes = num_classes, a.t = t, a.num_timesteps = num_timesteps, a.tables = tables;
    a.counter = true, a.noise.keys = stream_keys, a.noise.lig_graph = lig_graph, a.noise.lig_ptr = lig_ptr;
    a.noise.n_graphs = n_graphs, a.noise.purpose_base = purpose_base;
    a.x_next = x_next, a.c_next = c_next, a.v_next = v_next;
    return step_epilogue(a, stream);
}

int cbgx_targetdiff_step_boundary_rng(const float* x_den, const float* logits, const int32_t* lig_rows, const float* x_lig,
                                      const float* c_lig, const uint8_t* gen_lig, int n_lig, int num_classes, int t,
                                      int num_timesteps, const float* const* tables, const uint64_t* stream_keys,
                                      const int32_t* lig_graph, const int32_t* lig_ptr, int n_graphs, int purpose_base,
                                      float* x_next, float* c_next, const float* lig_emb_w, const float* lig_emb_b,
                                      const float* ind_w, const float* ind_b, float* x, float* h, void* stream) {
    StepArgs a;
    a.who = "step_boundary_rng";
    a.x_den = x_den, a.logits = logits, a.lig_rows = lig_rows, a.x_lig = x_lig, a.c_lig = c_lig, a.gen_lig = gen_lig;
    a.n_lig = n_lig, a.num_classes = num_classes, a.t = t, a.num_timesteps = num_timesteps, a.tables = tables;
    a.counter = true, a.noise.keys = stream_keys, a.noise.lig_graph = lig_graph, a.noise.lig_ptr = lig_ptr;
    a.noise.n_graphs = n_graphs, a.noise.purpose_base = purpose_base;
    a.x_next = x_next, a.c_next = c_next;
    a.boundary = true, a.lig_emb_w = lig_emb_w, a.lig_emb_b = lig_emb_b, a.ind_w = ind_w, a.ind_b = ind_b, a.x = x, a.h = h;
    return step_epilogue(a, stream);
}

int cbgx_targetdiff_epilogue_traj_rng(const float* x_den, const float* logits, const int32_t* lig_rows, float* traj_x,
                                      float* traj_c, const uint8_t* gen_lig, int n_lig, int num_classes, int32_t* t_dev,
                                      const float* const* tables, const uint64_t* stream_keys, const int32_t* lig_graph,
                                      const int32_t* lig_ptr, int n_graphs, int purpose_base, void* stream) {
    StepArgs a;
    a.who = "epilogue_traj_rng";
    a.x_den = x_den, a.logits = logits, a.lig_rows = lig_rows, a.x_lig = traj_x, a.c_lig = traj_c, a.gen_lig = gen_lig;
    a.n_lig = n_lig, a.num_classes = num_classes, a.tables = tables;
    a.counter = true, a.noise.keys = stream_keys, a.noise.lig_graph = lig_graph, a.noise.lig_ptr = lig_ptr;
    a.noise.n_graphs = n_graphs, a.noise.purpose_base = purpose_base;
    a.x_next = traj_x, a.c_next = traj_c;
    a.traj = true, a.t_dev = t_dev;
    return step_epilogue(a, stream);
}

}
```

cbgbench_amd/csrc/graph_mfma.hip:

```cpp
#include <hip/hip_runtime.h>
#include <stdint.h>

#include "kernels.h"
#include "layout.h"

namespace cbgx {

typedef float floatx4 __attribute__((ext_vector_type(4)));
#define MFMA(a, b, c) __builtin_amdgcn_mfma_f32_16x16x4f32((a), (b), (c), 0, 0, 0)

__constant__ float c_mu2[G] = {0.f, 1.f, 1.25f, 1.5f, 1.75f, 2.f, 2.25f, 2.5f, 2.75f, 3.f,
                               3.5f, 4.f, 4.5f, 5.f, 5.5f, 6.f, 7.f, 8.f, 9.f, 10.f};

template <int CTRL>
__device__ __forceinline__ unsigned dpp_u32(unsigned v) {
    return (unsigned)__builtin_amdgcn_update_dpp(0, (int)v, CTRL, 0xf, 0xf, false);
}
__device__ __forceinline__ float g_xrow_sum(float v) {
    auto r = __builtin_amdgcn_permlane16_swap(__float_as_uint(v), __float_as_uint(v), false, false);
    v = __uint_as_float(r[0]) + __uint_as_float(r[1]);
    r = __builtin_amdgcn_permlane32_swap(__float_as_uint(v), __float_as_uint(v), false, false);
    return __uint_as_float(r[0]) + __uint_as_float(r[1]);
}

// ... 209 lines not shown
    }
}

constexpr int GT = GH / 16;
#ifndef CBGX_GATE_WAVES_PER_EU
#define CBGX_GATE_WAVES_PER_EU 4
#endif
constexpr int GATE_WAVES_PER_EU = CBGX_GATE_WAVES_PER_EU;

__device__ __forceinline__ const float* gate_image_of_this_tile(const float* lds_img) {
    if (GATE_WAVES_PER_EU <= 1) return lds_img;
    int off = 0;
    asm volatile("" : "+v"(off));
    return lds_img + off;
}

__device__ __forceinline__ float gate_tile_value(const float* lds, const float (&mu)[5], float b2, int lane, int q,
                                                 float xi, float yi, float zi, float xj, float yj, float zj) {
    lds = gate_image_of_this_tile(lds);
    const float* l_frag = lds;
    const float* l_b1 = lds + GT * 5 * 64;
    const float* l_g = l_b1 + GH;
    const float* l_be = l_g + GH;
    const float* l_w2 = l_be + GH;
    const float rx = xi - xj, ry = yi - yj, rz = zi - zj;
    const float dist = sqrtf(rx * rx + ry * ry + rz * rz);
    float R[5];
#pragma unroll
    for (int s = 0; s < 5; ++s) { const float u = dist - mu[s]; R[s] = expf(-0.5f * (u * u)); }
    floatx4 acc[GT];
#pragma unroll
    for (int t = 0; t < GT; ++t) {
        const float4 b = *reinterpret_cast<const float4*>(l_b1 + 16 * t + 4 * q);
        acc[t] = floatx4{b.x, b.y, b.z, b.w};
    }
#pragma unroll
    for (int s = 0; s < 5; ++s)
#pragma unroll
        for (int t = 0; t < GT; ++t) acc[t] = MFMA(l_frag[(t * 5 + s) * 64 + lane], R[s], acc[t]);
    float v = 0.f;
#pragma unroll
    for (int t = 0; t < GT; ++t)
        v += (acc[t].x * acc[t].x + acc[t].y * acc[t].y) + (acc[t].z * acc[t].z + acc[t].w * acc[t].w);
    v = g_xrow_sum(v);
    const float rstd = 1.f / sqrtf(v * (1.f / GH) + 1e-5f);
    float z = 0.f;
#pragma unroll
    for (int t = 0; t < GT; ++t) {
        const float4 g = *reinterpret_cast<const float4*>(l_g + 16 * t + 4 * q);
        const float4 be = *reinterpret_cast<const float4*>(l_be + 16 * t + 4 * q);
        const float4 w2 = *reinterpret_cast<const float4*>(l_w2 + 16 * t + 4 * q);
        z = fmaf(fmaxf((acc[t].x * rstd) * g.x + be.x, 0.f), w2.x, z);
        z = fmaf(fmaxf((acc[t].y * rstd) * g.y + be.y, 0.f), w2.y, z);
        z = fmaf(fmaxf((acc[t].z * rstd) * g.z + be.z, 0.f), w2.z, z);
        z = fmaf(fmaxf((acc[t].w * rstd) * g.w + be.w, 0.f), w2.w, z);
    }
    z = g_xrow_sum(z) + b2;
    return 1.f / (1.f + expf(-z));
}

__global__ __launch_bounds__(256, GATE_WAVES_PER_EU) void edge_gate_mfma_kernel(const float* __restrict__ wts,
                                                             const float* __restrict__ x,
                                                             const int32_t* __restrict__ nbr,
                                                             const int32_t* __restrict__ deg, int n_nodes,
                                                             float* __restrict__ e_w, const int* __restrict__ rows,
                                                             const int* __restrict__ n_rows_ptr,
                                                             const unsigned* __restrict__ newmask) {
    __shared__ __attribute__((aligned(16))) float lds[GATE_IMG_SIZE];
    __shared__ int s_rank[4][KNN];
    {
        typedef float fx4 __attribute__((ext_vector_type(4)));
        constexpr int NV = ((int)GATE_IMG_SIZE / 4 + 255) / 256;
        fx4 v[NV];
#pragma unroll
        for (int u = 0; u < NV; ++u) {
            const int t = threadIdx.x + 256 * u;
            v[u] = reinterpret_cast<const fx4*>(wts + GATE_IMG)[t < (int)GATE_IMG_SIZE / 4 ? t : (int)GATE_IMG_SIZE / 4 - 1];
        }
        __builtin_amdgcn_sched_barrier(0);
#pragma unroll
        for (int u = 0; u < NV; ++u) {
            const int t = threadIdx.x + 256 * u;
            if (t < (int)GATE_IMG_SIZE / 4) reinterpret_cast<fx4*>(lds)[t] = v[u];
        }
    }
    __syncthreads();
    const float b2 = wts[GATE_B2];
    const int lane = threadIdx.x & 63, wave = threadIdx.x >> 6, c = lane & 15, q = lane >> 4;
    float mu[5];
#pragma unroll
    for (int s = 0; s < 5; ++s) mu[s] = c_mu2[4 * s + q];
    const int count = rows ? *n_rows_ptr : n_nodes;
    for (int idx = blockIdx.x * 4 + wave; idx < count; idx += gridDim.x * 4) {
        const int i = __builtin_amdgcn_readfirstlane(rows ? rows[idx] : idx);
        const int d = deg[i];
        const float xi = x[3 * i], yi = x[3 * i + 1], zi = x[3 * i + 2];
        if (newmask) {
            const unsigned m = newmask[i];
            const int cnt = __popc(m);
            __builtin_amdgcn_fence(__ATOMIC_ACQ_REL, "wavefront");
            __builtin_amdgcn_wave_barrier();
            if (lane < KNN && (m >> lane & 1u)) s_rank[wave][__popc(m & ((1u << lane) - 1u))] = lane;
            __builtin_amdgcn_fence(__ATOMIC_ACQ_REL, "wavefront");
            __builtin_amdgcn_wave_barrier();
            for (int t0 = 0; t0 < cnt; t0 += 16) {
                const int k = t0 + c;
                const bool valid = k < cnt;
                const int rank = valid ? s_rank[wave][k] : 0;
                const int j = valid ? nbr[(size_t)i * KNN + rank] : i;
                const float gv = gate_tile_value(lds, mu, b2, lane, q, xi, yi, zi, x[3 * j], x[3 * j + 1], x[3 * j + 2]);
                if (q == 0 && valid) e_w[(size_t)i * KNN + rank] = gv;
            }
            continue;
        }
#pragma unroll
        for (int hf = 0; hf < 2; ++hf) {
            const int e = c + 16 * hf;
            const bool valid = e < d;
            const int j = valid ? nbr[(size_t)i * KNN + e] : i;
            const float gv = gate_tile_value(lds, mu, b2, lane, q, xi, yi, zi, x[3 * j], x[3 * j + 1], x[3 * j + 2]);
            if (q == 0) e_w[(size_t)i * KNN + e] = valid ? gv : 0.f;
        }
    }
}

__device__ __forceinline__ void gm_wave_sync() {
    __builtin_amdgcn_fence(__ATOMIC_ACQ_REL, "wavefront");
    __builtin_amdgcn_wave_barrier();
}

__global__ __launch_bounds__(256, GATE_WAVES_PER_EU) void knn_merge_gate_kernel(
    const float* __restrict__ wts, const float* __restrict__ x, const int32_t* __restrict__ graph_ptr, int n_graphs,
    const uint8_t* __restrict__ lig, const int32_t* __restrict__ s_nbr, const int32_t* __restrict__ s_deg,
    const float* __restrict__ s_ew, int32_t* __restrict__ nbr, int32_t* __restrict__ deg, float* __restrict__ e_w,
    const int* __restrict__ rows, const int* __restrict__ n_rows_ptr) {
    __shared__ __attribute__((aligned(16))) float lds[GATE_IMG_SIZE];
    __shared__ int s_j[4][KNN], s_rank[4][KNN], s_sel[4][KNN];
    const int count = *n_rows_ptr;
    if ((int)blockIdx.x * 4 >= count) return;
    {
        typedef float fx4 __attribute__((ext_vector_type(4)));
        constexpr int NV = ((int)GATE_IMG_SIZE / 4 + 255) / 256;
        fx4 v[NV];
#pragma unroll
        for (int u = 0; u < NV; ++u) {
            const int t = threadIdx.x + 256 * u;
            v[u] = reinterpret_cast<const fx4*>(wts + GATE_IMG)[t < (int)GATE_IMG_SIZE / 4 ? t : (int)GATE_IMG_SIZE / 4 - 1];
        }
        __builtin_amdgcn_sched_barrier(0);
#pragma unroll
        for (int u = 0; u < NV; ++u) {
            const int t = threadIdx.x + 256 * u;
            if (t < (int)GATE_IMG_SIZE / 4) reinterpret_cast<fx4*>(lds)[t] = v[u];
        }
    }
    __syncthreads();
    const float b2 = wts[GATE_B2];
    const int lane = threadIdx.x & 63, wave = threadIdx.x >> 6, c = lane & 15, q = lane >> 4;
    float mu[5];
#pragma unroll
    for (int s = 0; s < 5; ++s) mu[s] = c_mu2[4 * s + q];
    const unsigned NONE = 0xffffffffu;
    for (int idx = blockIdx.x * 4 + wave; idx < count; idx += gridDim.x * 4) {
        const int i = __builtin_amdgcn_readfirstlane(rows[idx]);
        const unsigned lig_i = lig[i];
        const int sd_raw = s_deg[i];
        const int js_raw = s_nbr[(size_t)i * KNN + (lane & (KNN - 1))];
        const float ews = s_ew[(size_t)i * KNN + (lane & (KNN - 1))];
        const float xi = x[3 * i], yi = x[3 * i + 1], zi = x[3 * i + 2];
        int lo_g = 0, hi_g = n_graphs;
        while (hi_g - lo_g > 1) {
            const int mid = (lo_g + hi_g) >> 1;
            if (graph_ptr[mid] <= i) lo_g = mid; else hi_g = mid;
        }
        const int gs = graph_ptr[lo_g], ge = graph_ptr[lo_g + 1];
        const int r0 = ge - 1 - lane, r1 = ge - 65 - lane;
        const unsigned l0 = lig[r0 >= gs ? r0 : gs], l1 = lig[r1 >= gs ? r1 : gs];
        const unsigned long long b0 = __ballot((r0 >= gs) & (l0 != 0u));
        const unsigned long long b1 = __ballot((r1 >= gs) & (l1 != 0u));
        const int n0 = b0 == ~0ull ? 64 : __builtin_ctzll(~b0);
        const int n1 = n0 < 64 ? 0 : (b1 == ~0ull ? 64 : __builtin_ctzll(~b1));
        const int nl = n0 + n1;
        float* ew_out = e_w + (size_t)i * KNN;
        int jr;
        if (lig_i != 0u || nl >= 128 || ge - gs > 64 * KNN_SLOTS) {
            jr = knn_scan_node(x, graph_ptr, n_graphs, i, lane, nbr, deg);
            if (lane < KNN && jr < 0) ew_out[lane] = 0.f;
        } else {
            const int sd = __builtin_amdgcn_readfirstlane(sd_raw);
            const bool vs = lane < sd && lane < KNN;
            const int js = vs ? js_raw : i;
            const int ls = ge - nl;
            const bool v0 = lane < nl, v1 = lane + 64 < nl;
            const int j0 = v0 ? ls + lane : i, j1 = v1 ? ls + 64 + lane : i;
            const float sx = x[3 * js], sy = x[3 * js + 1], sz = x[3 * js + 2];
            const float ax = x[3 * j0], ay = x[3 * j0 + 1], az = x[3 * j0 + 2];
            const float bx = x[3 * j1], by = x[3 * j1 + 1], bz = x[3 * j1 + 2];
            const unsigned ks_h = vs ? __float_as_uint(dist2_exact2(xi, yi, zi, sx, sy, sz)) : NONE;
            const unsigned ks_l = vs ? (unsigned)js : NONE;
            const unsigned k0_h = v0 ? __float_as_uint(dist2_exact2(xi, yi, zi, ax, ay, az)) : NONE;
            const unsigned k1_h = v1 ? __float_as_uint(dist2_exact2(xi, yi, zi, bx, by, bz)) : NONE;
            const unsigned k0_l = v0 ? (unsigned)j0 : NONE, k1_l = v1 ? (unsigned)j1 : NONE;
            int rs = lane, r0k = 0, r1k = 0;
            for (int t = 0; t < min(nl, 64); ++t) {
                const unsigned bh = __builtin_amdgcn_readlane(k0_h, t), bl = __builtin_amdgcn_readlane(k0_l, t);
                rs += key_less(bh, bl, ks_h, ks_l) ? 1 : 0;
                r0k += key_less(bh, bl, k0_h, k0_l) ? 1 : 0;
                r1k += key_less(bh, bl, k1_h, k1_l) ? 1 : 0;
            }
            for (int t = 0; t < nl - 64; ++t) {
                const unsigned bh = __builtin_amdgcn_readlane(k1_h, t), bl = __builtin_amdgcn_readlane(k1_l, t);
                rs += key_less(bh, bl, ks_h, ks_l) ? 1 : 0;
                r0k += key_less(bh, bl, k0_h, k0_l) ? 1 : 0;
                r1k += key_less(bh, bl, k1_h, k1_l) ? 1 : 0;
            }
            for (int p = 0; p < min(sd, KNN); ++p) {
                const unsigned bh = __builtin_amdgcn_readlane(ks_h, p), bl = __builtin_amdgcn_readlane(ks_l, p);
                r0k += key_less(bh, bl, k0_h, k0_l) ? 1 : 0;
                r1k += key_less(bh, bl, k1_h, k1_l) ? 1 : 0;
            }
            const int d = min(KNN, min(sd, KNN) + nl);
            int32_t* out = nbr + (size_t)i * KNN;
            if (lane >= d && lane < KNN) { out[lane] = -1; ew_out[lane] = 0.f; }
            if (vs && rs < KNN) { out[rs] = js; ew_out[rs] = ews; }
            if (v0 && r0k < KNN) out[r0k] = j0;
            if (v1 && r1k < KNN) out[r1k] = j1;
            if (lane == 0) deg[i] = d;
            if (lane < KNN) s_j[wave][lane] = -1;
            gm_wave_sync();
            if (v0 && r0k < KNN) s_j[wave][r0k] = j0;
            if (v1 && r1k < KNN) s_j[wave][r1k] = j1;
            gm_wave_sync();
            jr = lane < KNN ? s_j[wave][lane] : -1;
        }
        const bool need = lane < KNN && jr >= 0;
        const unsigned m = (unsigned)(__ballot(need) & 0xffffffffull);
        const int cnt = __popc(m);
        if (need) {
            const int pos = __popc(m & ((1u << lane) - 1u));
            s_rank[wave][pos] = lane;
            s_sel[wave][pos] = jr;
        }
        gm_wave_sync();
        for (int t0 = 0; t0 < cnt; t0 += 16) {
            const int k = t0 + c;
            const bool valid = k < cnt;
            const int j = valid ? s_sel[wave][k] : i;
            const int rank = valid ? s_rank[wave][k] : 0;
            const float gv = gate_tile_value(lds, mu, b2, lane, q, xi, yi, zi, x[3 * j], x[3 * j + 1], x[3 * j + 2]);
            if (q == 0 && valid) ew_out[rank] = gv;
        }
        gm_wave_sync();
    }
}

hipError_t launch_knn_merge_gate(const float* packed, const float* x, const int32_t* graph_ptr, int n_graphs, int n_nodes,
                                 const uint8_t* lig, const int32_t* s_nbr, const int32_t* s_deg, const float* s_ew, int32_t* nbr,
                                 int32_t* deg, float* e_w, hipStream_t s, RowList rows) {
    if (n_nodes == 0) return hipSuccess;
    int grid = (n_nodes + 3) / 4;
    if (grid > 2048) grid = 2048;
    profile_mark_begin(K_KNN, s);
    hipLaunchKernelGGL(knn_merge_gate_kernel, dim3(grid), dim3(256), 0, s, packed, x, graph_ptr, n_graphs, lig, s_nbr, s_deg, s_ew,
                       nbr, deg, e_w, rows.rows, rows.count);
    profile_mark_end(s);
    return hipGetLastError();
}

__global__ void pack_gate_img_kernel(const float* __restrict__ w1, const float* __restrict__ b1,
                                     const float* __restrict__ g, const float* __restrict__ be,
                                     const float* __restrict__ w2, float* __restrict__ img) {
    __shared__ float colmean[G + 1];
    if (threadIdx.x <= G) {
        float s = 0.f;
        for (int u = 0; u < GH; ++u) s += threadIdx.x < G ? w1[u * G + threadIdx.x] : b1[u];
        colmean[threadIdx.x] = s * (1.f / GH);
    }
    __syncthreads();
    for (int idx = threadIdx.x; idx < GT * 5 * 64; idx += blockDim.x) {
        const int lane = idx & 63, s = (idx >> 6) % 5, t = idx / 320;
        const int u = 16 * t + (lane & 15), gg = 4 * s + (lane >> 4);
        img[idx] = w1[u * G + gg] - colmean[gg];
    }
    float* p = img + GT * 5 * 64;
    for (int u = threadIdx.x; u < GH; u += blockDim.x) {
        p[u] = b1[u] - colmean[G];
        p[GH + u] = g[u];
        p[2 * GH + u] = be[u];
        p[3 * GH + u] = w2[u];
    }
}

hipError_t launch_pack_gate_img(const float* w1, const float* b1, const float* g, const float* be, const float* w2,
                                float* img, hipStream_t s) {
    hipLaunchKernelGGL(pack_gate_img_kernel, dim3(1), dim3(256), 0, s, w1, b1, g, be, w2, img);
    return hipGetLastError();
}

__global__ __launch_bounds__(1024) void graph_cache_begin_kernel(
    const float* __restrict__ x, const int32_t* __restrict__ graph_ptr, int n_graphs, const uint8_t* __restrict__ lig,
    const float* __restrict__ r32sq, int n, uint8_t* __restrict__ dirty, int* __restrict__ list, int* __restrict__ count,
    const int32_t* __restrict__ s_nbr, const int32_t* __restrict__ s_deg, const float* __restrict__ s_ew,
    int32_t* __restrict__ nbr, int32_t* __restrict__ deg, float* __restrict__ ew, const float* __restrict__ h1,
    const float* __restrict__ h2, float* __restrict__ out1, float* __restrict__ out2) {
    __shared__ int s_cnt[16];
    __shared__ int s_base;
    const long t = (long)blockIdx.x * 1024 + threadIdx.x;
    if (t < (long)n * (KNN / 4)) {
        reinterpret_cast<int4*>(nbr)[t] = reinterpret_cast<const int4*>(s_nbr)[t];
        reinterpret_cast<float4*>(ew)[t] = reinterpret_cast<const float4*>(s_ew)[t];
        if ((t & (KNN / 4 - 1)) == 0) deg[t / (KNN / 4)] = s_deg[t / (KNN / 4)];
    }
    if (t < (long)n * (H / 4)) {
        reinterpret_cast<float4*>(out1)[t] = reinterpret_cast<const float4*>(h1)[t];
        reinterpret_cast<float4*>(out2)[t] = reinterpret_cast<const float4*>(h2)[t];
    }
    if ((long)blockIdx.x * 1024 >= n) return;
    const int i = (int)t;
    bool a = false;
    if (i < n) {
        if (lig[i]) a = true;
        else {
            int g = 0;
            {
                const int first = (int)blockIdx.x * 1024;
                int lo_g = 0, hi_g = n_graphs;
                while (hi_g - lo_g > 1) {
                    const int mid = (lo_g + hi_g) >> 1;
                    if (graph_ptr[mid] <= first) lo_g = mid; else hi_g = mid;
                }
                g = lo_g;
            }
            while (g + 1 < n_graphs && graph_ptr[g + 1] <= i) ++g;
            const int gs = graph_ptr[g], ge = graph_ptr[g + 1];
            const float xi = x[3 * i], yi = x[3 * i + 1], zi = x[3 * i + 2];
            const float lim = r32sq[i];
            bool alive = true;
            for (int j = ge - 1; alive && j >= gs; j -= 4) {
                unsigned lf[4];
                float px[4], py[4], pz[4];
#pragma unroll
                for (int u = 0; u < 4; ++u) {
                    const int jj = j - u >= gs ? j - u : gs;
                    lf[u] = lig[jj];
                    px[u] = x[3 * jj]; py[u] = x[3 * jj + 1]; pz[u] = x[3 * jj + 2];
                }
#pragma unroll
                for (int u = 0; u < 4; ++u) {
                    alive = alive & (j - u >= gs) & (lf[u] != 0u);
                    a |= alive & (dist2_exact2(xi, yi, zi, px[u], py[u], pz[u]) < lim);
                }
            }
        }
        dirty[i] = a ? 1 : 0;
    }
    const unsigned long long m = __ballot(a);
    const int lane = threadIdx.x & 63, wave = threadIdx.x >> 6;
    if (lane == 0) s_cnt[wave] = __popcll(m);
    __syncthreads();
    if (threadIdx.x == 0) {
        int tot = 0;
#pragma unroll
        for (int w = 0; w < 16; ++w) { const int c = s_cnt[w]; s_cnt[w] = tot; tot += c; }
        s_base = tot ? atomicAdd(count, tot) : 0;
    }
    __syncthreads();
    if (a) list[s_base + s_cnt[wave] + __popcll(m & ((1ull << lane) - 1ull))] = i;
}

hipError_t launch_graph_cache_begin(const float* x, const int32_t* graph_ptr, int n_graphs, const uint8_t* lig, const float* r32sq,
                                    int n, uint8_t* dirty, int* list, int* count, const int32_t* s_nbr, const int32_t* s_deg,
                                    const float* s_ew, int32_t* nbr, int32_t* deg, float* ew, const float* h1, const float* h2,
                                    float* out1, float* out2, hipStream_t s) {
    if (n == 0) return hipSuccess;
    const long threads = (long)n * (H / 4);
    hipLaunchKernelGGL(graph_cache_begin_kernel, dim3((unsigned)((threads + 1023) / 1024)), dim3(1024), 0, s, x, graph_ptr, n_graphs,
                       lig, r32sq, n, dirty, list, count, s_nbr, s_deg, s_ew, nbr, deg, ew, h1, h2, out1, out2);
    return hipGetLastError();
}

hipError_t launch_knn_reg(const float* x, const int32_t* graph_ptr, int n_graphs, int n_nodes, int32_t* nbr,
                          int32_t* deg, hipStream_t s, RowList rows) {
    if (n_nodes == 0) return hipSuccess;
    profile_mark_begin(K_KNN, s);
    hipLaunchKernelGGL(knn_graph_reg_kernel, dim3((n_nodes + 3) / 4), dim3(256), 0, s, x, graph_ptr, n_graphs, n_nodes,
                       nbr, deg, rows.rows, rows.count);
    profile_mark_end(s);
    return hipGetLastError();
}

hipError_t launch_knn_merge(const float* x, const int32_t* graph_ptr, int n_graphs, int n_nodes, const uint8_t* lig,
                            const int32_t* s_nbr, const int32_t* s_deg, int32_t* nbr, int32_t* deg, hipStream_t s, RowList rows,
                            const float* s_ew, float* e_w, unsigned* newmask) {
    if (n_nodes == 0) return hipSuccess;
    profile_mark_begin(K_KNN, s);
    hipLaunchKernelGGL(knn_merge_kernel, dim3((n_nodes + 3) / 4), dim3(256), 0, s, x, graph_ptr, n_graphs, lig, s_nbr, s_deg, nbr,
                       deg, rows.rows, rows.count, s_ew, e_w, newmask);
    profile_mark_end(s);
    return hipGetLastError();
}

hipError_t launch_gate_mfma(const float* packed, const float* x, const int32_t* nbr, const int32_t* deg, int n_nodes,
                            float* e_w, hipStream_t s, RowList rows, const unsigned* newmask) {
    if (n_nodes == 0) return hipSuccess;
    int grid = (n_nodes + 3) / 4;
    if (grid > 2048) grid = 2048;
    profile_mark_begin(K_GATE, s);
    hipLaunchKernelGGL(edge_gate_mfma_kernel, dim3(grid), dim3(256), 0, s, packed, x, nbr, deg, n_nodes, e_w, rows.rows, rows.count, newmask);
    profile_mark_end(s);
    return hipGetLastError();
}

}
```

cbgbench_amd/csrc/kernels.h:

```cpp
#pragma once
#include <hip/hip_runtime.h>
#include <stdint.h>

namespace cbgx {

struct AuxStream {
    hipStream_t owner = nullptr;
    hipStream_t s = nullptr;
    hipEvent_t fork = nullptr, join = nullptr, done[2] = {nullptr, nullptr};
};
AuxStream* aux_for(hipStream_t caller);

struct NodeList {
    int* rows;
    int* count;
};
struct RowList {
    const int* rows = nullptr;
    const int* count = nullptr;
    RowList() = default;
    RowList(const int* r, const int* c) : rows(r), count(c) {}
    RowList(NodeList l) : rows(l.rows), count(l.count) {}
};
struct NodeBufs { float *P, *q, *Qt; };
struct Graph {
    const int32_t *nbr, *deg;
    const float* e_w;
    const uint8_t *lig, *gen;
    int n_nodes;
};

enum KernelClass { K_KNN = 0, K_GATE, K_NODE_GEMM, K_NODE_QUERY, K_EDGE_X2H, K_EDGE_H2X, K_EDGE_X2H_LISTED, K_EDGE_X2H_BWD, K_EDGE_H2X_BWD,
                   K_TRAIN_GEMM, K_EDGE_X2H_BWD_LISTED, K_EDGE_ROWS_REDUCE, K_NUM_CLASSES };
void profile_mark_begin(int cls, hipStream_t s);
void profile_mark_end(hipStream_t s);
bool profile_is_on();

hipError_t launch_knn(const float* x, const int32_t* graph_ptr, int n_graphs, int n_nodes, int32_t* nbr,
                      int32_t* deg, hipStream_t s);
hipError_t launch_gate(const float* packed, const float* x, const int32_t* nbr, const int32_t* deg, int n_nodes,
                       float* e_w, hipStream_t s);
hipError_t launch_node_gemm(const float* A, int lda, const float* Wt, const float* bias, float* C, int ldc, int M,
                            int nout, int act, hipStream_t s, RowList rows = {});
hipError_t launch_attention(bool x2h, const float* att, const Graph& g, const float* x, const float* h, const NodeBufs& b, float* out,
                            float* dx_out, RowList dst, RowList src, hipStream_t s, bool h2x_lig = false);
#ifdef CBGX_XCHECK
extern int g_edge_impl;
hipError_t launch_knn_v1(const float* x, const int32_t* graph_ptr, int n_graphs, int n_nodes, int32_t* nbr, int32_t* deg,
                         hipStream_t s);
hipError_t launch_gate_v1(const float* packed, const float* x, const int32_t* nbr, const int32_t* deg, int n_nodes,
                          float* e_w, hipStream_t s);
hipError_t launch_node_gemm_v1(const float* A, int lda, const float* Wt, const float* bias, float* C, int ldc, int M, int nout, int act,
                               hipStream_t s, RowList rows);
hipError_t launch_node_query_v1(const float* att, const float* P, float* Qt, int n_nodes, hipStream_t s);
hipError_t launch_attention_v1(bool x2h, const float* att, const Graph& g, const float* x, const float* h, const NodeBufs& b,
                               float* out, float* dx_out, hipStream_t s);
#else
constexpr int g_edge_impl = 0;
#endif
constexpr int PACK_BLOCKS_MAX = 20;
struct PackBlocks {
    const float* wk0[PACK_BLOCKS_MAX];
    const float* bk0[PACK_BLOCKS_MAX];
    const float* wv0[PACK_BLOCKS_MAX];
    const float* bv0[PACK_BLOCKS_MAX];
    const float* wq0[PACK_BLOCKS_MAX];
    const float* bq0[PACK_BLOCKS_MAX];
    const float* wq1[PACK_BLOCKS_MAX];
    const float* wk1[PACK_BLOCKS_MAX];
    const float* wv1[PACK_BLOCKS_MAX];
    float* att[PACK_BLOCKS_MAX];
    const float* nsrc[PACK_BLOCKS_MAX][5];
    unsigned char x2h[PACK_BLOCKS_MAX];
    int n;
};
hipError_t launch_pack_stage1(const PackBlocks& pb, hipStream_t s);
hipError_t launch_pack_stage2(const PackBlocks& pb, hipStream_t s);
hipError_t launch_pack_gate_img(const float* w1, const float* b1, const float* g, const float* be, const float* w2,
                                float* img, hipStream_t s);
hipError_t launch_knn_reg(const float* x, const int32_t* graph_ptr, int n_graphs, int n_nodes, int32_t* nbr,
                          int32_t* deg, hipStream_t s, RowList rows = {});
hipError_t launch_knn_merge(const float* x, const int32_t* graph_ptr, int n_graphs, int n_nodes, const uint8_t* lig,
                            const int32_t* s_nbr, const int32_t* s_deg, int32_t* nbr, int32_t* deg, hipStream_t s, RowList rows,
                            const float* s_ew = nullptr, float* e_w = nullptr, unsigned* newmask = nullptr);
hipError_t launch_knn_merge_gate(const float* packed, const float* x, const int32_t* graph_ptr, int n_graphs, int n_nodes,
                                 const uint8_t* lig, const int32_t* s_nbr, const int32_t* s_deg, const float* s_ew, int32_t* nbr,
                                 int32_t* deg, float* e_w, hipStream_t s, RowList rows);
hipError_t launch_gate_mfma(const float* packed, const float* x, const int32_t* nbr, const int32_t* deg, int n_nodes,
                            float* e_w, hipStream_t s, RowList rows = {}, const unsigned* newmask = nullptr);
hipError_t launch_graph_cache_begin(const float* x, const int32_t* graph_ptr, int n_graphs, const uint8_t* lig, const float* r32sq,
                                    int n, uint8_t* dirty, int* list, int* count, const int32_t* s_nbr, const int32_t* s_deg,
                                    const float* s_ew, int32_t* nbr, int32_t* deg, float* ew, const float* h1, const float* h2,
                                    float* out1, float* out2, hipStream_t s);
hipError_t launch_pack_node_tables(const PackBlocks& pb, hipStream_t s);
hipError_t launch_build_active(const uint8_t* flag, int n, NodeList out, hipStream_t s, bool counter_zeroed = false);
hipError_t launch_mark_seed(const uint8_t* a, const uint8_t* b, int n, uint8_t* m, hipStream_t s);
hipError_t launch_mark_from_nbr(const uint8_t* flag, const int32_t* nbr, const int32_t* deg, int n, uint8_t* out,
                                hipStream_t s);
hipError_t launch_mark_nbr(RowList rows, int n_upper, const int32_t* nbr, const int32_t* deg, uint8_t* m, hipStream_t s);
struct NodeStageOpts {
    bool large_lists = false;
    RowList fold;
    bool q_direct = false;
    bool no_fold = false;
};
hipError_t launch_node_mfma(const float* att, const float* h, const uint8_t* lig, int n_nodes, const NodeBufs& b, RowList dst,
                            RowList src, hipStream_t s, const NodeStageOpts& o = {});
bool node_qdirect_enabled();
struct NodeStageJob {
    const float* att;
    float *P, *q, *Qt;
    const int *rows, *n_rows;
    unsigned chunk_mask;
    int proj_only;
    const uint8_t* fold_flag;
    int no_fold;
};
constexpr int NS_JOBS_MAX = 4;
struct NodeStageJobs { NodeStageJob j[NS_JOBS_MAX]; int n; };
constexpr int NODE_STAGE_MAX_ROWS = 8192;
bool add_node_stage_jobs(NodeStageJobs& jobs, const float* att, const NodeBufs& b, RowList dst, RowList src,
                         const uint8_t* fold_flag = nullptr, bool no_fold = false);
hipError_t launch_node_stage_jobs(const NodeStageJobs& jobs, const float* h, const uint8_t* lig, int n_nodes, hipStream_t s);
struct GraphFlags {
    const uint8_t *gen, *lig;
    const uint8_t* D1;
    uint8_t *d1, *a1, *a2, *a3, *D2, *S1, *S2;
};
constexpr int LIST_JOBS_MAX = 20;
struct ListJobs {
    const uint8_t* flag[LIST_JOBS_MAX];
    const uint8_t* flag2[LIST_JOBS_MAX];
    int want2[LIST_JOBS_MAX];
    int* list[LIST_JOBS_MAX];
    int* count[LIST_JOBS_MAX];
    int n_jobs;
};
hipError_t launch_list_level(const GraphFlags& f, const int32_t* nbr, const int32_t* deg, int n, int level, bool cached, bool prune,
                             hipStream_t s);
enum GraphFlagId { GF_GEN = 0, GF_LIG, GF_D1IN, GF_d1, GF_a1, GF_a2, GF_a3, GF_D2, GF_S1, GF_S2, GF_COUNT, GF_ALL = -1 };
constexpr int GRAPH_LISTS_MAX_NODES = 8192;
struct GraphListJobs {
    signed char flag[LIST_JOBS_MAX];
    signed char flag2[LIST_JOBS_MAX];
    signed char want2[LIST_JOBS_MAX];
    int* list[LIST_JOBS_MAX];
    int* count[LIST_JOBS_MAX];
    int n_jobs;
};
hipError_t launch_graph_lists(const uint8_t* gen, const uint8_t* lig, const uint8_t* d1_in, const int32_t* nbr, const int32_t* deg,
                              const int32_t* graph_ptr, int n_graphs, const GraphListJobs& jobs, bool cached, bool prune,
                              uint8_t* d1_out, hipStream_t s);
hipError_t launch_build_lists(const ListJobs& jobs, int n, hipStream_t s);
hipError_t launch_split_list(RowList in, int n, const uint8_t* flag, NodeList out1, NodeList out0, hipStream_t s,
                             bool counters_zeroed = false);
int set_edge_workgroup_limit(int n);
hipError_t launch_edge_mfma(bool x2h, const float* att, const Graph& g, const float* x, const float* h, const NodeBufs& b, float* out,
                            float* dx_out, RowList dst, hipStream_t s);
hipError_t launch_edge_x2h_dual(const float* att, const Graph& g, const float* x, const float* h, const NodeBufs& b, float* out,
                                RowList pp, RowList gen, bool full_layer, hipStream_t s);
hipError_t launch_edge_h2x_lig(const float* att, const Graph& g, const float* x, const float* h, const NodeBufs& b, float* out,
                               float* dx_out, RowList dst, hipStream_t s);
hipError_t launch_pack_h2l_image(const PackBlocks& pb, hipStream_t s);
bool h2x_fold_enabled();
void launch_edge_x2h_f16_grid(int grid, const float* att, const Graph& g, const float* x, const float* h, const NodeBufs& b,
                              float* out, RowList pp, RowList gen, bool full_layer, hipStream_t s);
hipError_t launch_step_prologue(const float* x_lig, const float* c_lig, const int32_t* lig_rows, int n_lig, int C,
                                const float* emb_w, const float* emb_b, const float* ind_w, const float* ind_b, float* x,
                                float* h, hipStream_t s, const int32_t* t_ptr = nullptr);
struct StepNoise {
    const float *eps = nullptr, *u = nullptr;
    const uint64_t* keys = nullptr;
    const int32_t *lig_graph = nullptr, *lig_ptr = nullptr;
    int n_graphs = 0, purpose_base = 0;
};
hipError_t launch_step_epilogue(const float* x_den, const float* logits, const int32_t* lig_rows, const float* x_lig,
                                const float* c_lig, const uint8_t* gen_lig, int n_lig, int C, int t,
                                const float* const* tabs, float log_c, const StepNoise& noise, float* x_next, float* c_next,
                                int32_t* v_next, hipStream_t s, int32_t* t_ptr = nullptr);
hipError_t launch_step_boundary(const float* x_den, const float* logits, const int32_t* lig_rows, const float* x_lig,
                                const float* c_lig, const uint8_t* gen_lig, int n_lig, int C, int t, const float* const* tabs,
                                float log_c, const StepNoise& noise, float* x_next, float* c_next, const float* emb_w,
                                const float* emb_b, const float* ind_w, const float* ind_b, float* x, float* h, hipStream_t s);
hipError_t launch_noise_fill(const uint64_t* keys, const int32_t* lig_ptr, int n_graphs, int n_lig, int cols, int uniform,
                             uint32_t purpose, int step, const int32_t* step_ptr, float* out, hipStream_t s);
hipError_t launch_diffbp_epilogue(const float* x_den, const float* x_com, const float* x_in, const float* logits,
                                  const int32_t* lig_rows, const int32_t* lig_ptr, const float* x_lig, const float* c_lig,
                                  const uint8_t* gen_lig, int n_graphs, int C, int t, int T, const float* acp_tab,
                                  const float* beta_tab, int absorbing, const float* eps, const float* u, float* x_next,
                                  float* c_next, hipStream_t s);
hipError_t launch_diffsbdd_step(const float* x_den, const float* logits, const int32_t* graph_ptr, const int32_t* lig_rows,
                                const int32_t* lig_ptr, const uint8_t* lig_flag, const float* x_lig, const float* c_lig,
                                int n_graphs, int C, float inv_alpha, float coef, float sigma, int do_x, int do_c,
                                const float* eps_x, const float* eps_c, const float* emb_w, const float* emb_b,
                                const float* ind_w, const float* ind_b, float* x_next, float* c_next, float* x, float* h,
                                float* shift_out, float* frame, hipStream_t s);
hipError_t launch_ligand_geometry(const float* x_lig, const uint8_t* z_lig, const int32_t* lig_ptr, int n_lig, const float* x_rec,
                                  const uint8_t* z_rec, const int32_t* rec_ptr, int n_rec, int n_graphs, int32_t* nr_bonds,
                                  uint8_t* flags, int32_t* graph_out, hipStream_t s);
void ligand_geometry_tables(int32_t* bond_pm, int32_t* margins, int32_t* allowed, uint8_t* elements, uint8_t* vdw_z, double* vdw_r,
                            double* tolerance);
hipError_t launch_ligand_bonds_count(const float* x_lig, const uint8_t* z_lig, const int32_t* lig_ptr, int n_lig, int n_graphs,
                                     int32_t* deg_up, int32_t* fragment, int32_t* graph_out, hipStream_t s);
hipError_t launch_ligand_bonds_fill(const float* x_lig, const uint8_t* z_lig, const int32_t* lig_ptr, int n_lig, int n_graphs,
                                    const int32_t* bond_ptr, int n_bonds, int32_t* bond_index, uint8_t* bond_order, double* bond_length,
                                    hipStream_t s);
hipError_t launch_ligand_rings(const int32_t* lig_ptr, int n_lig, int n_graphs, const int32_t* bond_ptr, const int32_t* bond_index,
                               int n_bonds, uint8_t* atom_ring_min, int32_t* graph_out, hipStream_t s);
hipError_t launch_ligand_aromatic(const uint8_t* z_lig, const uint8_t* flag_lig, const uint8_t* atom_ring_min, const int32_t* lig_ptr,
                                  int n_lig, int n_graphs, const int32_t* bond_ptr, const int32_t* bond_index, int n_bonds,
                                  uint8_t* atom_out, uint8_t* bond_aromatic, int32_t* graph_out, hipStream_t s);
hipError_t launch_ligand_pair_hist(const float* x_lig, const uint8_t* z_lig, const int32_t* lig_ptr, int n_lig, int n_graphs,
                                   const double* edges_all, int n_edges_all, const double* edges_cc, int n_edges_cc, int32_t* pair_hist,
                                   hipStream_t s);
hipError_t launch_ligand_angles(const float* x_lig, const uint8_t* z_lig, const int32_t* lig_ptr, int n_lig, int n_graphs,
                                const int32_t* adj_ptr, const int32_t* adj_nbr, const uint8_t* adj_order, int n_adj,
                                const int32_t* angle_ptr, int n_angles, const double* cos_edges, int n_cos_edges, int32_t* angle_index,
                                double* angle_cos, uint8_t* angle_bin, int16_t* angle_type, hipStream_t s);
constexpr int PACK_MAX = 64;
struct PackPiece {
    const float* src; float* dst; int src_ld, src_off, transpose, dst_ld, rows, cols;
};
struct PackBatch {
    PackPiece p[PACK_MAX]; int n;
};
hipError_t launch_pack_copy_multi(const PackBatch& b, hipStream_t s);
hipError_t launch_pack_copy(const float* src, int src_ld, int src_off, int transpose, float* dst, int dst_ld,
                            int rows, int cols, hipStream_t s);

}
```

cbgbench_amd/csrc/node_mfma.hip:

```cpp
#include <hip/hip_runtime.h>
#include <stdint.h>
#include <stdlib.h>

#include "kernels.h"
#include "layout.h"

namespace cbgx {

typedef float floatx4 __attribute__((ext_vector_type(4)));
#define MFMA(a, b, c) __builtin_amdgcn_mfma_f32_16x16x4f32((a), (b), (c), 0, 0, 0)
typedef _Float16 half8 __attribute__((ext_vector_type(8)));
#define MFMAH32(a, b, c) __builtin_amdgcn_mfma_f32_16x16x32_f16((a), (b), (c), 0, 0, 0)

__device__ __forceinline__ float4 nld4(const float* p) { return *reinterpret_cast<const float4*>(p); }

__device__ __forceinline__ float nxrow_sum(float v) {
    auto r = __builtin_amdgcn_permlane16_swap(__float_as_uint(v), __float_as_uint(v), false, false);
    v = __uint_as_float(r[0]) + __uint_as_float(r[1]);
    r = __builtin_amdgcn_permlane32_swap(__float_as_uint(v), __float_as_uint(v), false, false);
    return __uint_as_float(r[0]) + __uint_as_float(r[1]);
}

__device__ __forceinline__ float nxrow_max(float v) {
    auto r = __builtin_amdgcn_permlane16_swap(__float_as_uint(v), __float_as_uint(v), false, false);
// ... 1026 lines not shown
            const bool a = f.a2[i] != 0;
            if (e == 0 && a) f.a3[i] = 1;
            if (a && valid) f.a3[j] = 1;
        }
        if (cached) {
            const bool d = f.D2[i] != 0;
            if (e == 0 && d) f.S2[i] = 1;
            if (d && valid) f.S2[j] = 1;
        }
    }
}

__global__ __launch_bounds__(BA_THREADS) void build_lists_kernel(ListJobs jobs, int n) {
    __shared__ int s_cnt[BA_THREADS / 64];
    __shared__ int s_base;
    const int job = blockIdx.y;
    const uint8_t* __restrict__ fa = jobs.flag[job];
    const uint8_t* __restrict__ fb = jobs.flag2[job];
    const int idx = blockIdx.x * BA_THREADS + threadIdx.x;
    bool a = idx < n && (fa == nullptr || fa[idx] != 0);
    if (a && fb) a = (fb[idx] != 0) == (jobs.want2[job] != 0);
    const unsigned long long m = __ballot(a);
    const int lane = threadIdx.x & 63, wave = threadIdx.x >> 6;
    if (lane == 0) s_cnt[wave] = __popcll(m);
    __syncthreads();
    if (threadIdx.x == 0) {
        int tot = 0;
#pragma unroll
        for (int w = 0; w < BA_THREADS / 64; ++w) { const int c = s_cnt[w]; s_cnt[w] = tot; tot += c; }
        s_base = tot ? atomicAdd(jobs.count[job], tot) : 0;
    }
    __syncthreads();
    if (a) jobs.list[job][s_base + s_cnt[wave] + __popcll(m & ((1ull << lane) - 1ull))] = idx;
}

__global__ __launch_bounds__(1024) void graph_lists_kernel(const uint8_t* __restrict__ gen, const uint8_t* __restrict__ lig,
                                                           const uint8_t* __restrict__ d1_in, const int32_t* __restrict__ nbr,
                                                           const int32_t* __restrict__ deg, const int32_t* __restrict__ graph_ptr,
                                                           GraphListJobs jobs, int cached, int prune,
                                                           uint8_t* __restrict__ d1_out) {
    __shared__ unsigned F[GRAPH_LISTS_MAX_NODES];
    __shared__ int s_cnt[LIST_JOBS_MAX][16];
    __shared__ int s_base[LIST_JOBS_MAX];
    const int gs = graph_ptr[blockIdx.x], n = graph_ptr[blockIdx.x + 1] - gs;
    if (n <= 0 || n > GRAPH_LISTS_MAX_NODES) return;
    const int tid = threadIdx.x, lane = tid & 63, wave = tid >> 6;
    const uint8_t* __restrict__ d1p = d1_in ? d1_in : lig;
    constexpr int GL_KEEP = 24;
    const int n_pairs = n * KNN;
    const bool keep = n_pairs <= GL_KEEP * 1024;
    int jl[GL_KEEP];
    if (keep) {
#pragma unroll
        for (int u = 0; u < GL_KEEP; ++u) {
            const int t = tid + 1024 * u;
            jl[u] = nbr[(size_t)gs * KNN + min(t, n_pairs - 1)];
        }
    }
    for (int k0 = 0; k0 < n; k0 += 1024) {
        const int k = min(k0 + tid, n - 1);
        const unsigned fg = gen[gs + k], fl = lig[gs + k], fd = d1p[gs + k];
        if (k0 + tid < n)
            F[k] = (fg ? 1u << GF_GEN : 0u) | (fl ? 1u << GF_LIG : 0u) | ((d1_in != nullptr && fd) ? 1u << GF_D1IN : 0u);
    }
    __syncthreads();
    const unsigned Dx = d1_in ? GF_D1IN : GF_d1;
    const int levels = (cached || prune) ? 3 : 1;
    const bool hi = lane >= 32;
    const bool e0 = (lane & 31) == 0;
    for (int level = 0; level < levels; ++level) {
        for (int u0 = 0; u0 * 1024 < n_pairs; u0 += GL_KEEP) {
            if (!keep) {
#pragma unroll
                for (int u = 0; u < GL_KEEP; ++u) {
                    const int t = tid + 1024 * (u0 + u);
                    jl[u] = nbr[(size_t)gs * KNN + min(t, n_pairs - 1)];
                }
            }
            constexpr int GL_BATCH = 12;
#pragma unroll
            for (int ub = 0; ub < GL_KEEP; ub += GL_BATCH) {
            if ((u0 + ub) * 1024 + (tid & ~63) >= n_pairs) break;
            unsigned fi_[GL_BATCH], fj_[GL_BATCH];
#pragma unroll
            for (int v = 0; v < GL_BATCH; ++v) {
                const int u = ub + v;
                const int t = tid + 1024 * (u0 + u);
                const int i = min(t, n_pairs - 1) >> 5;
                const bool valid = t < n_pairs && (unsigned)(jl[u] - gs) < (unsigned)n;
                fi_[v] = F[i];
                fj_[v] = F[valid ? jl[u] - gs : i];
            }
            __builtin_amdgcn_sched_barrier(0);
#pragma unroll
            for (int v = 0; v < GL_BATCH; ++v) {
                const int u = ub + v;
                if ((u0 + u) * 1024 + (tid & ~63) >= n_pairs) break;
                const int t = tid + 1024 * (u0 + u);
                const bool in = t < n_pairs;
                const int i = min(t, n_pairs - 1) >> 5;
                const bool valid = in && (unsigned)(jl[u] - gs) < (unsigned)n;
                const int j = valid ? jl[u] - gs : i;
                const unsigned fi = fi_[v], fj = fj_[v];
                unsigned from_j, to_j, self;
                if (level == 0) {
                    from_j = (valid && (fj >> GF_LIG & 1u)) ? 1u << GF_d1 : 0u;
                    self = ((fi >> GF_GEN | fi >> GF_LIG) & 1u) << GF_a1 | (fi >> GF_LIG & 1u) << GF_d1;
                    to_j = (valid && (fi >> GF_GEN & 1u)) ? 1u << GF_a1 : 0u;
                } else if (level == 1) {
                    const unsigned a = prune ? fi >> GF_a1 & 1u : 0u, d = cached ? fi >> Dx & 1u : 0u;
                    from_j = (cached && valid && (fj >> Dx & 1u)) ? 1u << GF_D2 : 0u;
                    self = a << GF_a2 | d << GF_D2 | d << GF_S1;
                    to_j = valid ? (a << GF_a2 | d << GF_S1) : 0u;
                } else {
                    const unsigned a = prune ? fi >> GF_a2 & 1u : 0u, d = cached ? fi >> GF_D2 & 1u : 0u;
                    from_j = 0u;
                    self = a << GF_a3 | d << GF_S2;
                    to_j = valid ? (a << GF_a3 | d << GF_S2) : 0u;
                }
                const unsigned long long bal = __ballot(from_j != 0u);
                const bool any = ((hi ? bal >> 32 : bal) & 0xffffffffull) != 0ull;
                const unsigned own = in ? (self | (any ? (level == 0 ? 1u << GF_d1 : 1u << GF_D2) : 0u)) : 0u;
                if (e0 && own) atomicOr(&F[i], own);
                if (__ballot(to_j != 0u) != 0ull) {
                    if (to_j) atomicOr(&F[j], to_j);
                }
            }
            }
        }
        __syncthreads();
    }
    if (d1_out)
        for (int k = tid; k < n; k += 1024) d1_out[gs + k] = (uint8_t)(F[k] >> GF_d1 & 1u);
    for (int base = 0; base < n; base += 1024) {
        const int k = base + tid;
        const unsigned fk = k < n ? F[k] : 0u;
        unsigned member = 0u;
        for (int job = 0; job < jobs.n_jobs; ++job) {
            const int fa = jobs.flag[job], fb = jobs.flag2[job];
            bool a = k < n && (fa == GF_ALL || (fk >> (fa == GF_D1IN ? Dx : (unsigned)fa) & 1u));
            if (a && fb != GF_ALL) a = ((fk >> (fb == GF_D1IN ? Dx : (unsigned)fb) & 1u) != 0u) == (jobs.want2[job] != 0);
            const unsigned long long m = __ballot(a);
            if (lane == 0) s_cnt[job][wave] = __popcll(m);
            member |= a ? 1u << job : 0u;
        }
        __syncthreads();
        if (tid < jobs.n_jobs) {
            int tot = 0;
#pragma unroll
            for (int w = 0; w < 16; ++w) { const int c = s_cnt[tid][w]; s_cnt[tid][w] = tot; tot += c; }
            s_base[tid] = tot ? atomicAdd(jobs.count[tid], tot) : 0;
        }
        __syncthreads();
        for (int job = 0; job < jobs.n_jobs; ++job) {
            const bool a = (member >> job) & 1u;
            const unsigned long long m = __ballot(a);
            if (a) jobs.list[job][s_base[job] + s_cnt[job][wave] + __popcll(m & ((1ull << lane) - 1ull))] = gs + k;
        }
        __syncthreads();
    }
}

hipError_t launch_graph_lists(const uint8_t* gen, const uint8_t* lig, const uint8_t* d1_in, const int32_t* nbr, const int32_t* deg,
                              const int32_t* graph_ptr, int n_graphs, const GraphListJobs& jobs, bool cached, bool prune,
                              uint8_t* d1_out, hipStream_t s) {
    if (n_graphs == 0 || jobs.n_jobs == 0) return hipSuccess;
    hipLaunchKernelGGL(graph_lists_kernel, dim3(n_graphs), dim3(1024), 0, s, gen, lig, d1_in, nbr, deg, graph_ptr, jobs,
                       cached ? 1 : 0, prune ? 1 : 0, d1_out);
    return hipGetLastError();
}

hipError_t launch_list_level(const GraphFlags& f, const int32_t* nbr, const int32_t* deg, int n, int level, bool cached, bool prune,
                             hipStream_t s) {
    if (n == 0) return hipSuccess;
    const long threads = (long)n * 32;
    hipLaunchKernelGGL(list_level_kernel, dim3((unsigned)((threads + 255) / 256)), dim3(256), 0, s, f, nbr, deg, n, level,
                       cached ? 1 : 0, prune ? 1 : 0);
    return hipGetLastError();
}

hipError_t launch_build_lists(const ListJobs& jobs, int n, hipStream_t s) {
    if (n == 0 || jobs.n_jobs == 0) return hipSuccess;
    hipLaunchKernelGGL(build_lists_kernel, dim3((n + BA_THREADS - 1) / BA_THREADS, jobs.n_jobs), dim3(BA_THREADS), 0, s, jobs, n);
    return hipGetLastError();
}

__global__ void mark_seed_kernel(const uint8_t* __restrict__ a, const uint8_t* __restrict__ b, int n,
                                 uint8_t* __restrict__ m) {
    const int i = blockIdx.x * blockDim.x + threadIdx.x;
    if (i < n) m[i] = (a[i] | b[i]) ? 1 : 0;
}

__global__ void mark_nbr_kernel(const int* __restrict__ list, const int* __restrict__ count,
                                const int32_t* __restrict__ nbr, const int32_t* __restrict__ deg,
                                uint8_t* __restrict__ m) {
    const int t = blockIdx.x * blockDim.x + threadIdx.x;
    const int k = t >> 5, e = t & 31;
    if (k >= *count) return;
    const int i = list[k];
    if (e < deg[i]) m[nbr[(size_t)i * KNN + e]] = 1;
}

__global__ void mark_from_nbr_kernel(const uint8_t* __restrict__ flag, const int32_t* __restrict__ nbr,
                                     const int32_t* __restrict__ deg, int n, uint8_t* __restrict__ out) {
    const long t = (long)blockIdx.x * blockDim.x + threadIdx.x;
    const int i = (int)(t >> 5), e = (int)(t & 31);
    if (i >= n || e >= deg[i]) return;
    if (flag[nbr[(size_t)i * KNN + e]]) out[i] = 1;
}

hipError_t launch_mark_from_nbr(const uint8_t* flag, const int32_t* nbr, const int32_t* deg, int n, uint8_t* out,
                                hipStream_t s) {
    if (n == 0) return hipSuccess;
    hipError_t e = hipMemcpyAsync(out, flag, (size_t)n, hipMemcpyDeviceToDevice, s);
    if (e != hipSuccess) return e;
    const long threads = (long)n * 32;
    hipLaunchKernelGGL(mark_from_nbr_kernel, dim3((unsigned)((threads + 255) / 256)), dim3(256), 0, s, flag, nbr, deg, n, out);
    return hipGetLastError();
}

hipError_t launch_mark_seed(const uint8_t* a, const uint8_t* b, int n, uint8_t* m, hipStream_t s) {
    if (n == 0) return hipSuccess;
    hipLaunchKernelGGL(mark_seed_kernel, dim3((n + 255) / 256), dim3(256), 0, s, a, b, n, m);
    return hipGetLastError();
}

hipError_t launch_mark_nbr(RowList rows, int n_upper, const int32_t* nbr, const int32_t* deg, uint8_t* m, hipStream_t s) {
    if (n_upper == 0) return hipSuccess;
    const long threads = (long)n_upper * 32;
    hipLaunchKernelGGL(mark_nbr_kernel, dim3((unsigned)((threads + 255) / 256)), dim3(256), 0, s, rows.rows, rows.count, nbr, deg, m);
    return hipGetLastError();
}

hipError_t launch_build_active(const uint8_t* flag, int n, NodeList out, hipStream_t s, bool counter_zeroed) {
    if (!counter_zeroed) {
        hipError_t e = hipMemsetAsync(out.count, 0, sizeof(int), s);
        if (e != hipSuccess) return e;
    }
    if (n == 0) return hipSuccess;
    hipLaunchKernelGGL(build_active_kernel, dim3((n + BA_THREADS - 1) / BA_THREADS), dim3(BA_THREADS), 0, s, flag, n, out.rows, out.count);
    return hipGetLastError();
}

constexpr unsigned CHUNKS_ALL = 0x3ffu;
constexpr unsigned CHUNKS_PS = 0x0f0u;
constexpr unsigned CHUNKS_OWN = 0x30fu;
constexpr unsigned CHUNKS_QH = 0x300u;


bool add_node_stage_jobs(NodeStageJobs& jobs, const float* att, const NodeBufs& b, RowList dst, RowList src, const uint8_t* fold_flag,
                         bool no_fold) {
    if (jobs.n + (dst.rows ? 2 : 1) > NS_JOBS_MAX) return false;
    jobs.j[jobs.n++] = NodeStageJob{att, b.P, b.q, b.Qt, dst.rows, dst.count, dst.rows ? CHUNKS_OWN : CHUNKS_ALL, 0, fold_flag, no_fold ? 1 : 0};
    if (dst.rows) jobs.j[jobs.n++] = NodeStageJob{att, b.P, b.q, b.Qt, src.rows, src.count, CHUNKS_PS, 1, nullptr, 0};
    return true;
}

static void launch_node_stage_grid(const NodeStageJobs& jobs, const float* h, const uint8_t* lig, int n_nodes, hipStream_t s) {
    static const int forced = [] { const char* e = getenv("CBGX_NODE_STAGE_WAVES"); return e ? atoi(e) : 0; }();
    const int tiles = (n_nodes + 15) / 16;
    const int nw = (forced == 4 || forced == 8 || forced == 16) ? forced : NODE_STAGE_WAVES;
    const dim3 grid(min(tiles, 1024), jobs.n);
    if (nw == 4) hipLaunchKernelGGL(node_stage_kernel<4>, grid, dim3(256), 0, s, jobs, h, lig, n_nodes);
    else if (nw == 8) hipLaunchKernelGGL(node_stage_kernel<8>, grid, dim3(512), 0, s, jobs, h, lig, n_nodes);
    else hipLaunchKernelGGL(node_stage_kernel<16>, grid, dim3(1024), 0, s, jobs, h, lig, n_nodes);
}

hipError_t launch_node_stage_jobs(const NodeStageJobs& jobs, const float* h, const uint8_t* lig, int n_nodes, hipStream_t s) {
    if (n_nodes == 0 || jobs.n == 0) return hipSuccess;
    if (n_nodes > NODE_STAGE_MAX_ROWS || jobs.n > NS_JOBS_MAX) return hipErrorInvalidValue;
    profile_mark_begin(K_NODE_QUERY, s);
    launch_node_stage_grid(jobs, h, lig, n_nodes, s);
    profile_mark_end(s);
    return hipGetLastError();
}

bool node_qdirect_enabled() {
    static const bool on = [] { const char* e = getenv("CBGX_NODE_QDIRECT"); return !e || atoi(e) != 0; }();
    return on;
}

hipError_t launch_node_mfma(const float* att, const float* h, const uint8_t* lig, int n_nodes, const NodeBufs& b, RowList dst,
                            RowList src, hipStream_t s, const NodeStageOpts& o) {
    if (n_nodes == 0) return hipSuccess;
    const int tiles = (n_nodes + 63) / 64;
    const int grid = min(tiles, 512);
    const bool small = tiles <= 128 || (dst.rows != nullptr && !o.large_lists);
    auto proj_grid = [&](unsigned mask) {
        const int py = (__builtin_popcount(mask) + NP_CPW - 1) / NP_CPW;
        int gx = NP_RESIDENT_WGS / py;
        if (gx >= 8) gx &= ~7;
        return dim3((unsigned)min(tiles, gx), (unsigned)py);
    };
    const bool fused = n_nodes <= NODE_STAGE_MAX_ROWS;
    const bool direct = o.q_direct && !fused;
    const unsigned chunks_all = direct ? CHUNKS_ALL & ~CHUNKS_QH : CHUNKS_ALL, chunks_own = direct ? CHUNKS_OWN & ~CHUNKS_QH : CHUNKS_OWN;
    profile_mark_begin(K_NODE_GEMM, s);
    const bool two_jobs = fused && dst.rows != nullptr;
    if (!dst.rows) {
        if (!fused)
            hipLaunchKernelGGL(node_proj_kernel<false>, proj_grid(chunks_all), dim3(256), 0, s, att, h, lig, b.P, n_nodes,
                               (const int*)nullptr, (const int*)nullptr, chunks_all);
    } else {
        if (!two_jobs) {
            if (src.rows)
                hipLaunchKernelGGL(node_proj_kernel<true>, proj_grid(CHUNKS_PS), dim3(256), 0, s, att, h, lig, b.P, n_nodes, src.rows,
                                   src.count, CHUNKS_PS);
            else
                hipLaunchKernelGGL(node_proj_kernel<false>, proj_grid(CHUNKS_PS), dim3(256), 0, s, att, h, lig, b.P, n_nodes,
                                   (const int*)nullptr, (const int*)nullptr, CHUNKS_PS);
        }
        if (!fused)
            hipLaunchKernelGGL(node_proj_kernel<true>, proj_grid(chunks_own), dim3(256), 0, s, att, h, lig, b.P, n_nodes, dst.rows, dst.count,
                               chunks_own);
    }
    profile_mark_end(s);
    hipError_t e = hipGetLastError();
    if (e != hipSuccess) return e;
    profile_mark_begin(K_NODE_QUERY, s);
    if (fused) {
        NodeStageJobs jobs;
        jobs.n = 0;
        add_node_stage_jobs(jobs, att, b, dst, src, nullptr, o.no_fold);
        launch_node_stage_grid(jobs, h, lig, n_nodes, s);
    } else {
        if (direct)
            hipLaunchKernelGGL(node_query_kernel, dim3(min((n_nodes + NQK_ROWS - 1) / NQK_ROWS, NQK_GRID)), dim3(NQK_THREADS), 0, s, att, h,
                               b.q, n_nodes, dst.rows, dst.count);
        else
            hipLaunchKernelGGL(node_qmlp_kernel, dim3(grid, small ? 2 : 1), dim3(256), 0, s, att, b.P, b.q, n_nodes, dst.rows, dst.count);
        if (o.no_fold) {
        } else if (o.fold.rows)
            hipLaunchKernelGGL(node_qfold_kernel<4>, dim3(grid, 4), dim3(256), 0, s, att, b.q, b.Qt, n_nodes, o.fold.rows, o.fold.count);
        else if (small)
            hipLaunchKernelGGL(node_qfold_kernel<4>, dim3(grid, 4), dim3(256), 0, s, att, b.q, b.Qt, n_nodes, dst.rows, dst.count);
        else
            hipLaunchKernelGGL(node_qfold_kernel<16>, dim3(grid, 1), dim3(256), 0, s, att, b.q, b.Qt, n_nodes, dst.rows, dst.count);
    }
    profile_mark_end(s);
    return hipGetLastError();
}

}
```

cbgbench_amd/sampling.py:

```python
import os
import time

import torch
import torch.nn.functional as F

from . import _native
from . import noise as _noise
from .unitransformer import graph_ptr_from_batch

NUM_AA = 20

_OPERANDS = {"lig_rows32": ("lig_rows", torch.int32), "gen_l8": ("gen_l", torch.uint8), "lig8": ("lig_flag", torch.uint8),
             "gen8": ("gen_flag", torch.uint8)}


class _Lap:

    def __init__(self, timing, dev):
        self.timing, self.dev = timing, dev
        if timing is not None:
            if dev.type == "cuda":
                torch.cuda.synchronize(dev)
            self.t = time.perf_counter()

    def __call__(self, key):
        if self.timing is None:
            return
        if self.dev.type == "cuda":
            torch.cuda.synchronize(self.dev)
        now = time.perf_counter()
        self.timing[key] = self.timing.get(key, 0.0) + (now - self.t)
        self.t = now


class BatchesInFlight:

    _step_operands = ()

    @staticmethod
    def compose_plan(batch_idx_lig, batch_idx_rec, n_graphs=None):
        n_rec, n_lig = batch_idx_rec.shape[0], batch_idx_lig.shape[0]
        if (n_graphs is not None and batch_idx_rec.is_cuda and batch_idx_rec.dtype == torch.int64 and batch_idx_lig.dtype == torch.int64
                and 0 < n_graphs <= (1 << 20) and n_rec + n_lig > 0 and os.environ.get("CBGX_FUSED_COMPOSE", "1") != "0"):
            dev = batch_idx_rec.device
            N = n_rec + n_lig
            sort_idx = torch.empty(N, dtype=torch.int64, device=dev)
            batch_idx = torch.empty(N, dtype=torch.int64, device=dev)
            lig_flag = torch.empty(N, dtype=torch.bool, device=dev)
            lig_rows = torch.empty(n_lig, dtype=torch.int64, device=dev)
            graph_ptr = torch.empty(n_graphs + 1, dtype=torch.int32, device=dev)
            scratch = torch.empty(4 * n_graphs + 1, dtype=torch.int32, device=dev)
            _native.check(_native.lib().cbgx_compose_plan(
                _native.ptr(batch_idx_rec.contiguous()), _native.ptr(batch_idx_lig.contiguous()), n_rec, n_lig, int(n_graphs),
                _native.ptr(scratch), _native.ptr(sort_idx), _native.ptr(batch_idx), _native.ptr(lig_flag), _native.ptr(lig_rows),
                _native.ptr(graph_ptr), _native.current_stream(dev)), "cbgx_compose_plan")
            return sort_idx, batch_idx, lig_flag, lig_rows, graph_ptr
        batch_ctx = torch.cat([batch_idx_rec, batch_idx_lig], 0)
        sort_idx = torch.sort(batch_ctx, stable=True).indices
        batch_idx = batch_ctx[sort_idx]
        n_rec = batch_idx_rec.shape[0]
        lig_flag = sort_idx >= n_rec
        inv = torch.empty_like(sort_idx)
        inv[sort_idx] = torch.arange(sort_idx.numel(), device=sort_idx.device)
        lig_rows = inv[n_rec:]
        return sort_idx, batch_idx, lig_flag, lig_rows, graph_ptr_from_batch(batch_idx, n_graphs)

    def _plan_sampling(self, batch, noise, native, v_rec=None, pocket_order=False):
        x_rec = batch["protein_pos"]
        dev = x_rec.device
        bl, br = batch["ligand_element_batch"], batch["protein_element_batch"]
        gen_l = batch.get("ligand_gen_flag", batch["ligand_lig_flag"]).bool()
        gen_r = batch.get("protein_gen_flag", torch.zeros_like(batch["protein_lig_flag"])).bool()
        n_rec, n_lig = x_rec.shape[0], bl.shape[0]
        B = int(bl.max().item()) + 1
        sort_idx, batch_idx, lig_flag, lig_rows, graph_ptr = self.compose_plan(bl, br, B)
        gen_flag = torch.cat([gen_r, gen_l], 0)[sort_idx]
        rec_rows = torch.nonzero(~lig_flag).flatten()
        x = torch.empty(n_rec + n_lig, 3, dtype=torch.float32, device=dev)
        h = torch.empty(n_rec + n_lig, self.context_embedder.emb_dim, dtype=torch.float32, device=dev)
        if v_rec is None:
            v_rec = batch["protein_atom_feature"].float()
        h[rec_rows] = self.context_embedder.embed_protein(v_rec, F.one_hot(batch["protein_aa_type"], NUM_AA).float())
        st = {"B": B, "N": n_rec + n_lig, "n_lig": n_lig, "x": x, "h": h, "bl": bl, "br": br, "gen_l": gen_l, "batch_idx": batch_idx,
              "lig_flag": lig_flag, "gen_flag": gen_flag, "lig_rows": lig_rows, "rec_rows": rec_rows, "graph_ptr": graph_ptr,
              "traj_x": None, "traj_c": None, "static_h": None}
        st["gen_is_ligand"] = not bool(gen_r.any())
        csr = "lig_ptr" in self._step_operands
        if pocket_order:
            st["bl_sorted"], st["br_sorted"] = torch.stack([(bl[1:] >= bl[:-1]).all(), (br[1:] >= br[:-1]).all()]).tolist()
        elif noise is not None or (native and csr):
            st["bl_sorted"] = bool((bl[1:] >= bl[:-1]).all())
        st["native"] = bool(native and (st["bl_sorted"] if csr else True))
        if st.get("bl_sorted") and (noise is not None or (st["native"] and csr)):
            st["lig_ptr"] = _noise.ligand_csr(bl, B)
        if st["native"]:
            for key in self._step_operands:
                if key != "lig_ptr":
                    src, dtype = _OPERANDS[key]
                    st[key] = st[src].to(dtype).contiguous()
        return st

    def _finish_state(self, st, x_lig, c_lig, x_rec, keep_trajectory, static_cache, noise=None):
        dev, T, rec_rows = st["x"].device, self.num_diffusion_timesteps, st["rec_rows"]
        st["x"][rec_rows] = x_rec
        st["x_lig"], st["c_lig"] = x_lig.contiguous(), c_lig.contiguous()
        if dev.type == "cuda" and static_cache and st["gen_is_ligand"]:
            st["static_h"] = self.denoiser.static_context(x_rec, st["h"][rec_rows], st["br"], rec_rows, st["N"])
        if keep_trajectory:
            st["traj_x"] = torch.empty(T + 1, st["n_lig"], 3, dtype=torch.float32, device=dev)
            st["traj_c"] = torch.empty(T + 1, st["n_lig"], self.num_classes, dtype=torch.float32, device=dev)
            st["traj_x"][T], st["traj_c"][T] = x_lig, c_lig
        if noise is not None and st.get("noise") is None:
            self._attach_noise(st, noise)
        return st

    def _counter_refused(self, st):
        return None

    def _attach_noise(self, st, noise):
        why_not = self._counter_refused(st)
        if why_not is not None:
            raise ValueError(why_not)
        _noise.attach(st, noise, st["bl"], st["B"], lig_ptr=st.get("lig_ptr"), ordered=st.get("bl_sorted"))

    def _adopt_noise(self, st, noise):
        if st.get("noise") is None:
            self._attach_noise(st, noise)
        elif st["noise"] is not noise:
            raise ValueError("denoise_step: the state already runs on another CounterNoise")

    def _run_denoiser(self, st, need_h=True, h_on_sources=False, workspace=None):
        return self.denoiser(x=st["x"], h=st["h"], batch_idx=st["batch_idx"], lig_flag=st["lig_flag"], gen_flag=st["gen_flag"],
                             graph_ptr=st["graph_ptr"], need_h=need_h, static_h=st["static_h"], workspace=workspace,
                             h_on_sources=h_on_sources, gen_is_ligand=st["gen_is_ligand"])

    def _trajectory(self, st, out_dev, final=None):
        traj_x, traj_c, bl_out = st["traj_x"].to(out_dev), st["traj_c"].to(out_dev), st["bl"].to(out_dev)
        traj = {t - 1: (traj_x[t], traj_c[t], bl_out) for t in range(self.num_diffusion_timesteps + 1)}
        if final is not None:
            traj[0] = (final[0].to(out_dev), final[1].to(out_dev), bl_out)
        return traj

    def _begin(self, batch, noise, replay):
        if replay:
            batch = {k: v for k, v in batch.items() if k != "noise_keys"}
        return self.begin_sampling(batch, keep_trajectory=True, noise=None if replay else noise)

    def _many_begin(self, batch, tape, noise=None):
        return self._begin(batch, noise, tape is not None)

    def _many_step(self, st, t_idx, tape):
        self.denoise_step(st, t_idx, tape[t_idx] if tape is not None else None)

    def _many_finish(self, st, out_dev):
        return self._trajectory(st, out_dev)

    def _sample_loop(self, batch, tape, noise, return_device):
        st = self._many_begin(batch, tape, noise)
        for t_idx in reversed(range(self.num_diffusion_timesteps)):
            self._many_step(st, t_idx, tape)
        return self._many_finish(st, torch.device("cpu") if return_device is None else torch.device(return_device))

    def _side_streams(self, dev, n):
        pool = self.__dict__.setdefault("_stream_pool", {})
        have = pool.setdefault(str(dev), [])
        while len(have) < n:
            have.append(torch.cuda.Stream(dev))
        return have[:n]

    @torch.no_grad()
    def sample_many(self, batches, noise_tapes=None, return_device=None, streams=3, use_graph=False, noise_log=None, timing=None,
                    noise=None):
        dev = batches[0]["ligand_pos"].device
        lap = _Lap(timing, dev)
        out_dev = torch.device("cpu") if return_device is None else torch.device(return_device)
        tape = lambda k: None if noise_tapes is None else noise_tapes[k]
        if noise is not None and noise_tapes is not None:
            raise ValueError("sample_many: noise= (counter mode) and noise_tapes (replay) exclude each other")
        if noise is not None and len(noise) != len(batches):
            raise ValueError(f"sample_many: {len(noise)} noise entries for {len(batches)} batches")
        cn = lambda k: None if noise_tapes is not None else _noise.resolve(None if noise is None else noise[k], batches[k])
        T = self.num_diffusion_timesteps
        graphs = bool(use_graph) and noise_tapes is None and dev.type == "cuda" and hasattr(self, "make_step_graph")
        if dev.type != "cuda" or ((len(batches) == 1 or streams <= 1) and not graphs):
            out = []
            for k, b in enumerate(batches):
                st = self._many_begin(b, tape(k), cn(k))
                lap("begin_sampling_s")
                for t_idx in reversed(range(T)):
                    self._many_step(st, t_idx, tape(k))
                lap("steps_s")
                out.append(self._many_finish(st, out_dev))
                lap("traj_download_s")
            return out
        states = [self._many_begin(b, tape(k), cn(k)) for k, b in enumerate(batches)]
        lap("begin_sampling_s")
        cur = torch.cuda.current_stream(dev)
        side = self._side_streams(dev, max(1, min(streams, len(states))))
        for sx in side:
            sx.wait_stream(cur)
        if graphs:
            made = [self.make_step_graph(st, stream=side[k % len(side)]) for k, st in enumerate(states)]
            for n in range(T):
                for k, (st, (replay, done)) in enumerate(zip(states, made)):
                    if n < T - done:
                        with torch.cuda.stream(side[k % len(side)]):
                            replay()
                            if noise_log is not None and st.get("_noise") is not None:
                                side[k % len(side)].synchronize()
                                noise_log.append((k, T - 1 - done - n, st["_noise"][0].clone(), st["_noise"][1].clone()))
        else:
            for t_idx in reversed(range(T)):
                for k, st in enumerate(states):
                    with torch.cuda.stream(side[k % len(side)]):
                        self._many_step(st, t_idx, tape(k))
        for sx in side:
            cur.wait_stream(sx)
        lap("steps_s")
        out = [self._many_finish(st, out_dev) for st in states]
        lap("traj_download_s")
        return out
```

cbgbench_amd/unitransformer.py:

```python
import ctypes
import math

import torch
from torch import nn

from . import _native

RBF_OFFSETS = (0, 1, 1.25, 1.5, 1.75, 2, 2.25, 2.5, 2.75, 3, 3.5, 4, 4.5, 5, 5.5, 6, 7, 8, 9, 10)


class _Params(nn.Module):
    def forward(self, *a, **k):
        raise RuntimeError("parameter container: the computation lives in libcbgx (UniTransformer.forward)")


class GaussianSmearing(_Params):

    def __init__(self):
        super().__init__()
        self.register_buffer("offset", torch.tensor(RBF_OFFSETS, dtype=torch.float32))


class MLP(_Params):

    def __init__(self, in_dim, out_dim, hidden_dim):
        super().__init__()
        self.net = nn.Sequential(nn.Linear(in_dim, hidden_dim), nn.LayerNorm(hidden_dim), nn.ReLU(),
                                 nn.Linear(hidden_dim, out_dim))


class X2HAttention(_Params):

    def __init__(self, hidden, n_heads, kv_in):
        super().__init__()
        self.distance_expansion = GaussianSmearing()
        self.hk_func = MLP(kv_in, hidden, hidden)
        self.hv_func = MLP(kv_in, hidden, hidden)
        self.hq_func = MLP(hidden, hidden, hidden)


class H2XAttention(_Params):

    def __init__(self, hidden, n_heads, kv_in):
        super().__init__()
        self.distance_expansion = GaussianSmearing()
        self.xk_func = MLP(kv_in, hidden, hidden)
        self.xv_func = MLP(kv_in, n_heads, hidden)
        self.xq_func = MLP(hidden, hidden, hidden)


class E3DualAttentionLayer(_Params):
    def __init__(self, hidden, n_heads, kv_in):
        super().__init__()
        self.x2h_layers = nn.ModuleList([X2HAttention(hidden, n_heads, kv_in)])
        self.h2x_layers = nn.ModuleList([H2XAttention(hidden, n_heads, kv_in)])


_MLP_KEYS = ("net.0.weight", "net.0.bias", "net.1.weight", "net.1.bias", "net.3.weight", "net.3.bias")


def graph_ptr_from_batch(batch_idx, n_graphs=None):
    if n_graphs is None:
        n_graphs = int(batch_idx[-1].item()) + 1 if batch_idx.numel() else 0
    counts = torch.zeros(n_graphs, dtype=torch.int64, device=batch_idx.device).index_add_(0, batch_idx, torch.ones_like(batch_idx))
    ptr = torch.zeros(n_graphs + 1, dtype=torch.int32, device=batch_idx.device)
    ptr[1:] = torch.cumsum(counts, 0).to(torch.int32)
    return ptr


class _DenoiserFunction(torch.autograd.Function):

    @staticmethod
    def forward(ctx, module, ligand_outputs_only, x, h, graph_ptr, lig, gen, *params):
        h_on_sources = ligand_outputs_only == "h_on_sources"
        ligand_outputs_only = ligand_outputs_only is True
        device = x.device
        N, B = x.shape[0], graph_ptr.numel() - 1
        L, C = module.num_layers, module.out_classes
        lib = _native.lib()
        packed = module.packed_weights(device)
        tape = torch.empty(lib.cbgx_train_tape_bytes(N, L), dtype=torch.uint8, device=device)
        ws = module.train_workspace(N, device)
        x_out = torch.empty_like(x)
        h_out = None if ligand_outputs_only else torch.empty_like(h)
        logits = torch.empty(N, C, dtype=torch.float32, device=device)
        rc = lib.cbgx_unitransformer_forward_train_ex(
            _native.ptr(packed), L, C, _native.ptr(x), _native.ptr(h), _native.ptr(graph_ptr), _native.ptr(lig),
            _native.ptr(gen), N, B, _native.ptr(x_out), _native.ptr(h_out), _native.ptr(logits), 1 if h_on_sources else 0,
            _native.ptr(tape), tape.numel(), _native.ptr(ws), ws.numel(), _native.current_stream(device))
        _native.check(rc, "cbgx_unitransformer_forward_train_ex")
        if h_out is None:
            h_out = torch.empty(0, h.shape[1], dtype=torch.float32, device=device)
        ctx.module, ctx.tape, ctx.packed, ctx.flags, ctx.n = module, tape, packed, (lig, gen), N
        ctx.ligand_outputs_only = bool(ligand_outputs_only)
        ctx.param_shapes = [tuple(p.shape) for p in params]
        ctx.set_materialize_grads(False)
        return x_out, h_out, logits

    @staticmethod
    def backward(ctx, gx, gh, gl):
        module, N = ctx.module, ctx.n
        lig, gen = ctx.flags
        device = ctx.tape.device
        L, C = module.num_layers, module.out_classes
        direct = module._direct_grads and not module._direct_written
        arr = None
        if direct:
            params = module._ordered_params()
            views = [p.grad for p in params]
            cache = getattr(module, "_direct_cache", None)
            if (cache is not None and len(cache[0]) == len(views) and all(a is b for a, b in zip(cache[0], views))
                    and cache[2] == (views[0].data_ptr(), views[-1].data_ptr())):
                arr = cache[1]
            elif any(v is None or not v.is_contiguous() or v.dtype != torch.float32 or v.device != device for v in views):
                direct = False
        if not direct:
            sizes = [int(math.prod(s)) for s in ctx.param_shapes]
            flat = torch.empty(sum(sizes), dtype=torch.float32, device=device)
            views = list(flat.split(sizes))
        if arr is None:
            arr = (ctypes.c_void_p * len(views))(*[v.data_ptr() for v in views])
            if direct:
                module._direct_cache = (views, arr, (views[0].data_ptr(), views[-1].data_ptr()))
        need_h = ctx.needs_input_grad[3]
        gh_in = torch.empty(N, module.hidden_dim, dtype=torch.float32, device=device) if need_h else None
        ws = module.train_workspace(N, device)
        cont = lambda g: None if g is None else g.contiguous().float()
        gx, gh, gl = cont(gx), cont(gh), cont(gl)
        if gh is not None and ctx.ligand_outputs_only:
            raise RuntimeError("UniTransformer(ligand_outputs_only=True): the loss has a gradient on h' -- the taped forward was pruned "
                               "on the promise that h' is not read")
        if gh is None and not ctx.ligand_outputs_only:
            gh = torch.zeros(N, module.hidden_dim, dtype=torch.float32, device=device)
        if direct:
            module._direct_written = True
        args = (_native.ptr(ctx.packed), L, C, _native.ptr(ctx.tape), ctx.tape.numel(), _native.ptr(lig),
                _native.ptr(gen), N, _native.ptr(gx), _native.ptr(gh), _native.ptr(gl), arr, len(views), _native.ptr(gh_in))
        tail = (_native.ptr(ws), ws.numel(), _native.current_stream(device))
        gx_in = None
        if ctx.needs_input_grad[2]:
            gx_in = torch.empty(N, 3, dtype=torch.float32, device=device)
            rc = _native.lib().cbgx_unitransformer_backward_ex(*args, _native.ptr(gx_in), *tail)
        else:
            rc = _native.lib().cbgx_unitransformer_backward(*args, *tail)
        _native.check(rc, "cbgx_unitransformer_backward")
        if direct:
            return (None, None, gx_in, gh_in, None, None, None) + (None,) * len(views)
        grads = [v.view(s) for v, s in zip(views, ctx.param_shapes)]
        return (None, None, gx_in, gh_in, None, None, None, *grads)


class UniTransformer(nn.Module):
    def __init__(self, cfg):
        super().__init__()
        self.cfg = cfg
        g = cfg.get
        self.num_classes = g("num_classes", None)
        self.out_classes = g("out_classes", self.num_classes)
        self.num_blocks = g("num_blocks", 1)
        self.num_layers = g("num_layers", 6)
        self.hidden_dim = g("node_feat_dim", 128)
        self.n_heads = g("n_heads", 16)
        self.edge_feat_dim = g("edge_feat_dim", 4)
        self.num_r_gaussian = g("num_r_gaussian", 20)
        self.cutoff_mode = g("cutoff_mode", "knn")
        self.cut_off = g("k", 32)
        self.ew_net_type = g("ew_type", "global")
        unsupported = []
        if self.hidden_dim != 128: unsupported.append(f"node_feat_dim={self.hidden_dim}")
        if self.n_heads != 16: unsupported.append(f"n_heads={self.n_heads}")
        if self.num_r_gaussian != 20: unsupported.append(f"num_r_gaussian={self.num_r_gaussian}")
        if self.edge_feat_dim != 4: unsupported.append(f"edge_feat_dim={self.edge_feat_dim}")
        if int(self.cut_off) != 32: unsupported.append(f"k={self.cut_off}")
        if self.num_blocks != 1: unsupported.append(f"num_blocks={self.num_blocks}")
        if self.ew_net_type != "global": unsupported.append(f"ew_type={self.ew_net_type}")
        if g("num_x2h", 1) != 1 or g("num_h2x", 1) != 1: unsupported.append("num_x2h/num_h2x != 1")
        if g("act_fn", "relu") != "relu" or not g("norm", True): unsupported.append("act_fn/norm")
        if g("x2h_out_fc", False): unsupported.append("x2h_out_fc=True")
        if g("dist_emb_type", "gaussian_exp") != "gaussian_exp": unsupported.append("dist_emb_type")
        if self.cutoff_mode != "knn":
            raise ValueError(f"Not supported cutoff mode: {self.cutoff_mode}")
        if unsupported:
            raise ValueError("UniTransformer (libcbgx) does not support: " + ", ".join(unsupported))

        kv_in = 2 * self.hidden_dim + self.edge_feat_dim + 4 * self.num_r_gaussian
        self.dist_emb = nn.Sequential(GaussianSmearing(), MLP(self.num_r_gaussian, 1, self.num_r_gaussian * 8))
        self.blocks = nn.ModuleList([E3DualAttentionLayer(self.hidden_dim, self.n_heads, kv_in)
                                     for _ in range(self.num_layers)])
        if self.num_classes is not None:
            self.classifier = nn.Sequential(nn.Linear(self.hidden_dim, self.hidden_dim), _Params(),
                                            nn.Linear(self.hidden_dim, self.out_classes))
        else:
            self.classifier = None
        self._packed = None
        self._packed_key = None
        self._workspace = None
        self._train_workspace = None
        self._direct_grads = False
        self._direct_written = False

    def __repr__(self):
        return (f"UniTransformer[libcbgx/gfx950](num_layers={self.num_layers}, n_heads={self.n_heads}, "
                f"hidden={self.hidden_dim}, k={self.cut_off}, num_classes={self.num_classes})")

    def _apply(self, fn, *args, **kwargs):
        self._ordered = None
        self._direct_cache = None
        self.__dict__.pop("_flag_cache", None)
        return super()._apply(fn, *args, **kwargs)

    def _ordered_params(self):
        cached = getattr(self, "_ordered", None)
        if cached is not None and all(d.get(k) is p for (d, k), p in zip(self._ordered_slots, cached)):
            return cached
        sd = dict(self.named_parameters())
        names = [f"dist_emb.1.{k}" for k in _MLP_KEYS]
        for l in range(self.num_layers):
            for blk, fns in (("x2h_layers.0", ("hk_func", "hv_func", "hq_func")),
                             ("h2x_layers.0", ("xk_func", "xv_func", "xq_func"))):
                for fn in fns:
                    names += [f"blocks.{l}.{blk}.{fn}.{k}" for k in _MLP_KEYS]
        if self.classifier is not None:
            names += ["classifier.0.weight", "classifier.0.bias", "classifier.2.weight", "classifier.2.bias"]
        self._ordered_slots = [(self.get_submodule(n.rpartition(".")[0])._parameters, n.rpartition(".")[2]) for n in names]
        self._ordered = [sd[n] for n in names]
        return self._ordered

    def packed_weights(self, device):
        if self.classifier is None:
            raise ValueError("libcbgx needs the classifier head (num_classes) to pack weights")
        params = self._ordered_params()
        key = (str(device),) + tuple((p.data_ptr(), _native.version(p)) for p in params)
        if self._packed is None or self._packed_key != key:
            lib = _native.lib()
            n = lib.cbgx_packed_weights_floats(self.num_layers, self.out_classes)
            packed = torch.empty(n, dtype=torch.float32, device=device)
            srcs = [p.detach().to(device=device, dtype=torch.float32).contiguous() for p in params]
            arr = (ctypes.c_void_p * len(srcs))(*[s.data_ptr() for s in srcs])
            _native.check(lib.cbgx_pack_weights(arr, len(srcs), self.num_layers, self.out_classes,
                                                _native.ptr(packed), _native.current_stream(device)),
                          "cbgx_pack_weights")
            self._packed, self._packed_key, self._packed_srcs = packed, key, srcs
            self._packed_event = torch.cuda.Event()
            self._packed_event.record(torch.cuda.current_stream(device))
            self._packed_seen = {torch.cuda.current_stream(device).cuda_stream}
        cur = torch.cuda.current_stream(device)
        if cur.cuda_stream not in self._packed_seen and not torch.cuda.is_current_stream_capturing():
            cur.wait_event(self._packed_event)
            self._packed_seen.add(cur.cuda_stream)
        return self._packed

    @staticmethod
    def workspace_bytes(n_nodes, n_graphs):
        return int(_native.lib().cbgx_workspace_bytes(n_nodes, n_graphs))

    def workspace(self, n_nodes, n_graphs, device):
        need = _native.lib().cbgx_workspace_bytes(n_nodes, n_graphs)
        if self._workspace is None:
            self._workspace = {}
        key = (str(device), torch.cuda.current_stream(device).cuda_stream)
        ws = self._workspace.get(key)
        if ws is None or ws.numel() < need:
            ws = torch.empty(need, dtype=torch.uint8, device=device)
            self._workspace[key] = ws
        return ws

    def train_workspace(self, n_nodes, device):
        need = _native.lib().cbgx_train_workspace_bytes(n_nodes)
        ws = self._train_workspace
        if ws is None or ws.numel() < need or ws.device != device:
            ws = torch.empty(need, dtype=torch.uint8, device=device)
            self._train_workspace = ws
        return ws

    @torch.no_grad()
    def static_context(self, x_rec, h_rec, batch_idx_rec, rec_rows, n_nodes, graph_ptr_rec=None):
        if self.num_layers < 4:
            return None
        device = x_rec.device
        n = x_rec.shape[0]
        if graph_ptr_rec is None:
            graph_ptr_rec = graph_ptr_from_batch(batch_idx_rec)
        B = graph_ptr_rec.numel() - 1
        x_rec = x_rec.detach().float().contiguous()
        h_rec = h_rec.detach().float().contiguous()
        zeros = torch.zeros(n, dtype=torch.uint8, device=device)
        packed, ws = self.packed_weights(device), self.workspace(n, B, device)
        lib = _native.lib()
        out = []
        for L in (1, 2):
            x_o, h_o = torch.empty_like(x_rec), torch.empty_like(h_rec)
            rc = lib.cbgx_unitransformer_forward(
                _native.ptr(packed), L, self.out_classes, _native.ptr(x_rec), _native.ptr(h_rec),
                _native.ptr(graph_ptr_rec), _native.ptr(zeros), _native.ptr(zeros), n, B, _native.ptr(x_o),
                _native.ptr(h_o), None, _native.ptr(ws), ws.numel(), _native.current_stream(device))
            _native.check(rc, "cbgx_unitransformer_forward (static context)")
            full = torch.zeros(n_nodes, self.hidden_dim, dtype=torch.float32, device=device)
            full[rec_rows] = h_o
            out.append(full)
        from . import stages
        nbr_r, deg_r = stages.knn_graph(x_rec, graph_ptr_rec)
        ew_r = stages.edge_gate(packed, x_rec, nbr_r, deg_r)
        last = x_rec[nbr_r[:, 31].clamp(min=0).long()]
        dx, dy, dz = (x_rec[:, 0] - last[:, 0]), (x_rec[:, 1] - last[:, 1]), (x_rec[:, 2] - last[:, 2])
        r32 = (dx * dx + dy * dy) + dz * dz
        r32 = torch.where(deg_r >= 32, r32, torch.full_like(r32, float("inf")))
        rows32 = rec_rows.to(torch.int32)
        nbr = torch.full((n_nodes, 32), -1, dtype=torch.int32, device=device)
        nbr[rec_rows] = torch.where(nbr_r >= 0, rows32[nbr_r.clamp(min=0).long()], nbr_r)
        deg = torch.zeros(n_nodes, dtype=torch.int32, device=device)
        deg[rec_rows] = deg_r
        ew = torch.zeros(n_nodes, 32, dtype=torch.float32, device=device)
        ew[rec_rows] = ew_r
        r32sq = torch.full((n_nodes,), float("inf"), dtype=torch.float32, device=device)
        r32sq[rec_rows] = r32
        return (out[0], out[1], nbr.contiguous(), deg, ew, r32sq)

    def _as_u8(self, flag):
        if flag.dtype == torch.uint8:
            return flag.contiguous()
        if flag.is_cuda and torch.cuda.is_current_stream_capturing():
            return flag.to(torch.uint8).contiguous()
        cache = self.__dict__.setdefault("_flag_cache", {})
        hit = cache.get(id(flag))
        if hit is not None and hit[0] is flag and hit[1] == _native.version(flag) and hit[2].device == flag.device:
            return hit[2]
        u8 = flag.to(torch.uint8).contiguous()
        if len(cache) >= 64:
            cache.pop(next(iter(cache)))
        cache[id(flag)] = (flag, _native.version(flag), u8)
        return u8

    def forward(self, x, h, batch_idx, lig_flag, gen_flag, graph_ptr=None, need_h=True, static_h=None,
                ligand_outputs_only=False, workspace=None, h_on_sources=False, gen_is_ligand=False):
        if not x.is_cuda:
            raise RuntimeError("UniTransformer.forward runs on an MI355X through libcbgx; got a CPU tensor "
                               "(no CPU fallback exists; use oracle/ for CPU reference results)")
        device = x.device
        N = x.shape[0]
        if graph_ptr is None:
            graph_ptr = graph_ptr_from_batch(batch_idx)
        B = graph_ptr.numel() - 1
        lig, gen = self._as_u8(lig_flag), self._as_u8(gen_flag)
        if torch.is_grad_enabled() and (x.requires_grad or h.requires_grad or any(p.requires_grad for p in self.parameters())):
            return _DenoiserFunction.apply(self, "h_on_sources" if (h_on_sources and not ligand_outputs_only) else bool(ligand_outputs_only),
                                           (x if x.requires_grad else x.detach()).to(torch.float32).contiguous(),
                                           h.to(torch.float32).contiguous(), graph_ptr, lig, gen,
                                           *self._ordered_params())
        x = x.detach().to(torch.float32).contiguous()
        h = h.detach().to(torch.float32).contiguous()
        packed = self.packed_weights(device)
        if workspace is not None:
            if workspace.device != device or workspace.dtype != torch.uint8 or workspace.numel() < self.workspace_bytes(N, B):
                raise ValueError(f"workspace: need a uint8 tensor of >= {self.workspace_bytes(N, B)} bytes on {device}")
            ws = workspace
        else:
            ws = self.workspace(N, B, device)
        x_out = torch.empty_like(x)
        h_out = torch.empty_like(h) if need_h else None
        logits = torch.empty(N, self.out_classes, dtype=torch.float32, device=device)
        lib = _native.lib()
        flags = _native.FWD_GEN_IS_LIGAND if gen_is_ligand else 0
        if static_h is not None:
            rc = lib.cbgx_unitransformer_forward_cached(
                _native.ptr(packed), self.num_layers, self.out_classes, _native.ptr(x), _native.ptr(h),
                _native.ptr(graph_ptr), _native.ptr(lig), _native.ptr(gen), N, B, _native.ptr(static_h[0]),
                _native.ptr(static_h[1]), *[_native.ptr(t) for t in static_h[2:6]], _native.ptr(x_out),
                _native.ptr(h_out), _native.ptr(logits), flags | (_native.FWD_H_ON_SOURCES if (h_on_sources and need_h) else 0),
                _native.ptr(ws), ws.numel(),
                _native.current_stream(device))
        else:
            rc = lib.cbgx_unitransformer_forward_v2(
                _native.ptr(packed), self.num_layers, self.out_classes, _native.ptr(x), _native.ptr(h),
                _native.ptr(graph_ptr), _native.ptr(lig), _native.ptr(gen), N, B,
                _native.ptr(x_out), _native.ptr(h_out), _native.ptr(logits), flags,
                _native.ptr(ws), ws.numel(), _native.current_stream(device))
        _native.check(rc, "cbgx_unitransformer_forward")
        return x_out, h_out, logits
```

include/cbgx.h:

```cpp
#ifndef CBGX_H
#define CBGX_H

#include <stddef.h>
#include <stdint.h>

#ifdef __cplusplus
extern "C" {
#endif

#define CBGX_ABI_VERSION 6

#define CBGX_OK 0
#define CBGX_E_INVALID (-1)
#define CBGX_E_WORKSPACE (-2)
#define CBGX_E_HIP (-3)

#define CBGX_HIDDEN 128
#define CBGX_HEADS 16
#define CBGX_NUM_GAUSSIANS 20
#define CBGX_KNN 32
#define CBGX_EDGE_TYPES 4
#define CBGX_GATE_HIDDEN 160
#define CBGX_MAX_CLASSES 128

int cbgx_abi_version(void);
const char *cbgx_last_error(void);

int cbgx_set_edge_workgroups(int n);

size_t cbgx_packed_weights_floats(int num_layers, int num_classes);
int cbgx_pack_weights(const float *const *tensors, int num_tensors, int num_layers, int num_classes,
                      float *packed, void *stream);

size_t cbgx_workspace_bytes(int n_nodes, int n_graphs);
int cbgx_unitransformer_forward(const float *packed, int num_layers, int num_classes,
                                const float *x, const float *h, const int32_t *graph_ptr,
                                const uint8_t *lig_flag, const uint8_t *gen_flag,
                                int n_nodes, int n_graphs,
                                float *x_out, float *h_out, float *logits,
                                void *workspace, size_t workspace_bytes, void *stream);

#define CBGX_FWD_H_ON_SOURCES 1u
#define CBGX_FWD_GEN_IS_LIGAND 2u
int cbgx_unitransformer_forward_v2(const float *packed, int num_layers, int num_classes,
                                   const float *x, const float *h, const int32_t *graph_ptr,
                                   const uint8_t *lig_flag, const uint8_t *gen_flag,
                                   int n_nodes, int n_graphs,
                                   float *x_out, float *h_out, float *logits, unsigned flags,
                                   void *workspace, size_t workspace_bytes, void *stream);
int cbgx_unitransformer_forward_cached(const float *packed, int num_layers, int num_classes,
                                       const float *x, const float *h, const int32_t *graph_ptr,
                                       const uint8_t *lig_flag, const uint8_t *gen_flag, int n_nodes, int n_graphs,
                                       const float *static_h1, const float *static_h2,
                                       const int32_t *static_nbr, const int32_t *static_deg,
                                       const float *static_ew, const float *static_r32sq,
                                       float *x_out, float *h_out, float *logits, unsigned flags,
                                       void *workspace, size_t workspace_bytes, void *stream);


int cbgx_knn_graph(const float *x, const int32_t *graph_ptr, int n_graphs, int n_nodes, int k,
                   int32_t *nbr, int32_t *deg, void *stream);

int cbgx_edge_gate(const float *packed, const float *x, const int32_t *nbr, const int32_t *deg,
                   int n_nodes, float *e_w, void *stream);

int cbgx_x2h_attention(const float *packed, int layer, const float *x, const float *h,
                       const int32_t *nbr, const int32_t *deg, const uint8_t *lig_flag, const float *e_w,
                       int n_nodes, float *h_out, void *workspace, size_t workspace_bytes, void *stream);

int cbgx_h2x_attention(const float *packed, int layer, const float *x, const float *h,
                       const int32_t *nbr, const int32_t *deg, const uint8_t *lig_flag,
                       const uint8_t *gen_flag, const float *e_w, int n_nodes,
                       float *x_out, float *delta_x, void *workspace, size_t workspace_bytes, void *stream);
int cbgx_h2x_attention_v2(const float *packed, int layer, const float *x, const float *h,
                          const int32_t *nbr, const int32_t *deg, const uint8_t *lig_flag,
                          const uint8_t *gen_flag, const float *e_w, int n_nodes,
                          float *x_out, float *delta_x, unsigned flags, void *workspace, size_t workspace_bytes, void *stream);

int cbgx_node_stage(const float *packed, int layer, int x2h, const float *h, const uint8_t *lig_flag, int n_nodes,
                    const int32_t *rows, const int32_t *n_rows, int q_direct, float *P, float *q, float *Qt, void *stream);

int cbgx_classifier(const float *packed, int num_layers, int num_classes, const float *h, int n_nodes,
                    float *logits, void *workspace, size_t workspace_bytes, void *stream);

size_t cbgx_packed_h2x_stack_floats(int num_layers);
int cbgx_pack_h2x_stack(const float *const *tensors, int num_tensors, int num_layers, float *packed, void *stream);
int cbgx_h2x_stack_forward(const float *packed, int num_layers, const float *x, const float *h,
                           const int32_t *graph_ptr, const uint8_t *lig_flag, const uint8_t *gen_flag,
                           int n_nodes, int n_graphs, float *x_out, void *workspace, size_t workspace_bytes,
                           void *stream);
int cbgx_h2x_stack_forward_v2(const float *packed, int num_layers, const float *x, const float *h,
                              const int32_t *graph_ptr, const uint8_t *lig_flag, const uint8_t *gen_flag,
                              int n_nodes, int n_graphs, float *x_out, unsigned flags, void *workspace,
                              size_t workspace_bytes, void *stream);

int cbgx_targetdiff_prologue(const float *x_lig, const float *c_lig, const int32_t *lig_rows, int n_lig,
                             int num_classes, const float *lig_emb_w, const float *lig_emb_b, const float *ind_w,
                             const float *ind_b, float *x, float *h, void *stream);
int cbgx_targetdiff_epilogue(const float *x_den, const float *logits, const int32_t *lig_rows, const float *x_lig,
                             const float *c_lig, const uint8_t *gen_lig, int n_lig, int num_classes, int t,
                             int num_timesteps, const float *const *tables, const float *eps, const float *u,
                             float *x_next, float *c_next, int32_t *v_next, void *stream);

int cbgx_targetdiff_step_boundary(const float *x_den, const float *logits, const int32_t *lig_rows, const float *x_lig,
                                  const float *c_lig, const uint8_t *gen_lig, int n_lig, int num_classes, int t,
                                  int num_timesteps, const float *const *tables, const float *eps, const float *u,
                                  float *x_next, float *c_next, const float *lig_emb_w, const float *lig_emb_b,
                                  const float *ind_w, const float *ind_b, float *x, float *h, void *stream);

int cbgx_targetdiff_prologue_traj(const float *traj_x, const float *traj_c, const int32_t *t_dev,
                                  const int32_t *lig_rows, int n_lig, int num_classes, const float *lig_emb_w,
                                  const float *lig_emb_b, const float *ind_w, const float *ind_b, float *x, float *h,
                                  void *stream);
int cbgx_targetdiff_epilogue_traj(const float *x_den, const float *logits, const int32_t *lig_rows, float *traj_x,
                                  float *traj_c, const uint8_t *gen_lig, int n_lig, int num_classes, int32_t *t_dev,
                                  const float *const *tables, const float *eps, const float *u, void *stream);

int cbgx_diffbp_epilogue(const float *x_den, const float *x_com, const float *x_in, const float *logits,
                         const int32_t *lig_rows, const int32_t *lig_ptr, const float *x_lig, const float *c_lig,
                         const uint8_t *gen_lig, int n_lig, int n_graphs, int num_classes, int t, int num_timesteps,
                         const float *alphas_cumprod, const float *betas, int absorbing_state, const float *eps,
                         const float *u, float *x_next, float *c_next, void *stream);
int cbgx_diffsbdd_step(const float *x_den, const float *logits, const int32_t *graph_ptr, const int32_t *lig_rows,
                       const int32_t *lig_ptr, const uint8_t *lig_flag, const float *x_lig, const float *c_lig, int n_lig,
                       int n_graphs, int num_classes, float inv_alpha, float coef, float sigma, int update_positions,
                       int update_types, const float *eps_x, const float *eps_c, const float *lig_emb_w,
                       const float *lig_emb_b, const float *ind_w, const float *ind_b, float *x_next, float *c_next,
                       float *x, float *h, float *shift, float *frame_shift, void *stream);

#define CBGX_NOISE_POS_NORMAL 0
#define CBGX_NOISE_TYPE_UNIFORM 1
#define CBGX_NOISE_MASK_UNIFORM 2
#define CBGX_NOISE_TYPE_NORMAL 3
#define CBGX_NOISE_INIT_POS 4
#define CBGX_NOISE_INIT_TYPE 5
#define CBGX_NOISE_FINAL_POS 6
#define CBGX_NOISE_TRAIN_TIME 7
#define CBGX_NOISE_TRAIN_POS_NORMAL 8
#define CBGX_NOISE_TRAIN_TYPE_UNIFORM 9
#define CBGX_NOISE_TRAIN_MASK_UNIFORM 10
#define CBGX_NOISE_TRAIN_TYPE_NORMAL 11
#define CBGX_NOISE_TRAIN_PROTEIN_NORMAL 12
#define CBGX_NOISE_TRAIN_CHOOSE_CTX 13
#define CBGX_NOISE_PURPOSE_STRIDE 16
int cbgx_noise_fill(const uint64_t *stream_keys, const int32_t *lig_ptr, int n_graphs, int n_lig, int cols, int uniform,
                    int purpose, int step, const int32_t *step_dev, float *out, void *stream);
int cbgx_train_noise_draw(const uint64_t *stream_keys, const int32_t *lig_ptr, int n_graphs, int n_lig, int purpose_base, int n_t,
                          const int64_t *t_in, int64_t *t_out, float *a, float *b, int cols_b, int purpose_b, int uniform_b,
                          void *stream);
int cbgx_targetdiff_train_noise_rng(const float *x0, const int64_t *v0, const int64_t *batch, const uint8_t *gen, int n_lig,
                                    int num_classes, const float *alphas_cumprod, const float *log_alphas_cumprod,
                                    const float *log_one_minus_alphas_cumprod, const uint64_t *stream_keys,
                                    const int32_t *lig_ptr, int n_graphs, int purpose_base, int n_t, const int64_t *t_in,
                                    int64_t *t_out, float *x_t, float *c_t, int64_t *v_t, void *stream);
#define CBGX_CENTER_PROTEIN 0
#define CBGX_CENTER_CONTEXT 1
#define CBGX_CENTER_LIGAND 2
#define CBGX_CENTER_WHOLE 3
int cbgx_train_transform(const float *x_rec, const float *x_lig, const int32_t *rec_ptr, const int32_t *lig_ptr,
                         const uint8_t *ctx, int n_graphs, int n_rec, int n_lig, float sigma, int center_mode, const float *eps,
                         float *x_rec_out, float *x_lig_out, float *center_out, void *stream);
int cbgx_train_transform_rng(const float *x_rec, const float *x_lig, const int32_t *rec_ptr, const int32_t *lig_ptr,
                             const uint8_t *ctx, int n_graphs, int n_rec, int n_lig, float sigma, int center_mode,
                             const uint64_t *stream_keys, int purpose_base, float *x_rec_out, float *x_lig_out,
                             float *center_out, void *stream);
int cbgx_train_transform_choose(const float *x_rec, const float *x_lig, const int32_t *rec_ptr, const int32_t *lig_ptr,
                                const int32_t *dec_ptr, const int32_t *gen_ptr, const int32_t *gen_idx, const int32_t *choice_in,
                                int n_graphs, int n_rec, int n_lig, int n_dec, int n_idx, float sigma, int center_mode,
                                const float *eps, float *x_rec_out, float *x_lig_out, float *center_out, uint8_t *gen_flag_out,
                                int32_t *choice_out, void *stream);
int cbgx_train_transform_choose_rng(const float *x_rec, const float *x_lig, const int32_t *rec_ptr, const int32_t *lig_ptr,
                                    const int32_t *dec_ptr, const int32_t *gen_ptr, const int32_t *gen_idx, int n_graphs, int n_rec,
                                    int n_lig, int n_dec, int n_idx, float sigma, int center_mode, const uint64_t *stream_keys,
                                    int purpose_base, float *x_rec_out, float *x_lig_out, float *center_out,
                                    uint8_t *gen_flag_out, int32_t *choice_out, void *stream);
int cbgx_targetdiff_epilogue_rng(const float *x_den, const float *logits, const int32_t *lig_rows, const float *x_lig,
                                 const float *c_lig, const uint8_t *gen_lig, int n_lig, int num_classes, int t,
                                 int num_timesteps, const float *const *tables, const uint64_t *stream_keys,
                                 const int32_t *lig_graph, const int32_t *lig_ptr, int n_graphs, int purpose_base,
                                 float *x_next, float *c_next, int32_t *v_next, void *stream);
int cbgx_targetdiff_step_boundary_rng(const float *x_den, const float *logits, const int32_t *lig_rows, const float *x_lig,
                                      const float *c_lig, const uint8_t *gen_lig, int n_lig, int num_classes, int t,
                                      int num_timesteps, const float *const *tables, const uint64_t *stream_keys,
                                      const int32_t *lig_graph, const int32_t *lig_ptr, int n_graphs, int purpose_base,
                                      float *x_next, float *c_next, const float *lig_emb_w, const float *lig_emb_b,
                                      const float *ind_w, const float *ind_b, float *x, float *h, void *stream);
int cbgx_targetdiff_epilogue_traj_rng(const float *x_den, const float *logits, const int32_t *lig_rows, float *traj_x,
                                      float *traj_c, const uint8_t *gen_lig, int n_lig, int num_classes, int32_t *t_dev,
                                      const float *const *tables, const uint64_t *stream_keys, const int32_t *lig_graph,
                                      const int32_t *lig_ptr, int n_graphs, int purpose_base, void *stream);

size_t cbgx_train_tape_bytes(int n_nodes, int num_layers);
size_t cbgx_train_workspace_bytes(int n_nodes);
int cbgx_unitransformer_forward_train(const float *packed, int num_layers, int num_classes,
                                      const float *x, const float *h, const int32_t *graph_ptr,
                                      const uint8_t *lig_flag, const uint8_t *gen_flag, int n_nodes, int n_graphs,
                                      float *x_out, float *h_out, float *logits, void *tape, size_t tape_bytes,
                                      void *workspace, size_t workspace_bytes, void *stream);
int cbgx_unitransformer_backward(const float *packed, int num_layers, int num_classes, const void *tape,
                                 size_t tape_bytes, const uint8_t *lig_flag, const uint8_t *gen_flag, int n_nodes,
                                 const float *grad_x_out, const float *grad_h_out, const float *grad_logits,
                                 float *const *grads, int num_grads, float *grad_h_in, void *workspace,
                                 size_t workspace_bytes, void *stream);
int cbgx_unitransformer_backward_ex(const float *packed, int num_layers, int num_classes, const void *tape,
                                    size_t tape_bytes, const uint8_t *lig_flag, const uint8_t *gen_flag, int n_nodes,
                                    const float *grad_x_out, const float *grad_h_out, const float *grad_logits,
                                    float *const *grads, int num_grads, float *grad_h_in, float *grad_x_in, void *workspace,
                                    size_t workspace_bytes, void *stream);
int cbgx_unitransformer_forward_train_ex(const float *packed, int num_layers, int num_classes, const float *x, const float *h,
                                         const int32_t *graph_ptr, const uint8_t *lig_flag, const uint8_t *gen_flag,
                                         int n_nodes, int n_graphs, float *x_out, float *h_out, float *logits, unsigned flags,
                                         void *tape, size_t tape_bytes, void *workspace, size_t workspace_bytes, void *stream);
int cbgx_x2h_attention_backward(const float *packed, int layer, const float *x, const float *h,
                                const int32_t *nbr, const int32_t *deg, const uint8_t *lig_flag, const float *e_w,
                                int n_nodes, const float *grad_h_out, float *grad_h, float *grad_x, float *grad_e_w,
                                float *const *grads, void *workspace, size_t workspace_bytes, void *stream);
int cbgx_h2x_attention_backward(const float *packed, int layer, const float *x, const float *h,
                                const int32_t *nbr, const int32_t *deg, const uint8_t *lig_flag,
                                const uint8_t *gen_flag, const float *e_w, int n_nodes, const float *grad_x_out,
                                float *grad_h, float *grad_x, float *grad_e_w, float *const *grads, void *workspace,
                                size_t workspace_bytes, void *stream);

size_t cbgx_h2x_stack_tape_bytes(int n_nodes, int num_layers);
int cbgx_h2x_stack_forward_train(const float *packed, int num_layers, const float *x, const float *h,
                                 const int32_t *graph_ptr, const uint8_t *lig_flag, const uint8_t *gen_flag,
                                 int n_nodes, int n_graphs, float *x_out, void *tape, size_t tape_bytes,
                                 void *workspace, size_t workspace_bytes, void *stream);
int cbgx_h2x_stack_backward(const float *packed, int num_layers, const void *tape, size_t tape_bytes, const float *h,
                            const uint8_t *lig_flag, const uint8_t *gen_flag, int n_nodes, const float *grad_x_out,
                            float *const *grads, int num_grads, float *grad_h, void *workspace,
                            size_t workspace_bytes, void *stream);
int cbgx_h2x_stack_backward_ex(const float *packed, int num_layers, const void *tape, size_t tape_bytes, const float *h,
                               const uint8_t *lig_flag, const uint8_t *gen_flag, int n_nodes, const float *grad_x_out,
                               float *const *grads, int num_grads, float *grad_h, float *grad_x_in, void *workspace,
                               size_t workspace_bytes, void *stream);

int cbgx_targetdiff_train_noise(const float *x0, const int64_t *v0, const int64_t *t, const int64_t *batch,
                                const uint8_t *gen, int n_lig, int num_classes, const float *alphas_cumprod,
                                const float *log_alphas_cumprod, const float *log_one_minus_alphas_cumprod,
                                const float *eps, const float *u, float *x_t, float *c_t, int64_t *v_t, void *stream);
int cbgx_targetdiff_loss(const float *x_out, const float *logits, const int64_t *lig_rows, const float *x0,
                         const int64_t *v0, const int64_t *v_t, const int64_t *t, const int64_t *batch, const uint8_t *gen,
                         int n_lig, int n_graphs, int num_classes, const float *const *tables, float *losses, float *x_pred,
                         float *c_pred, float *grad_pos, float *grad_logit, void *stream);
int cbgx_targetdiff_loss_backward(const float *grad_pos, const float *grad_logit, const int64_t *sort_idx, int n_protein,
                                  int n_nodes, int num_classes, const float *g_loss_pos, const float *g_loss_atom,
                                  float *grad_x_out, float *grad_logits, void *stream);
int cbgx_diffbp_loss(const float *x_out, const float *x_in, const float *x_stack, const float *logits, const int64_t *sort_idx,
                     const int32_t *graph_ptr, const uint8_t *lig_flag, const float *pos_noise, const float *com_noise,
                     const int64_t *v0, const uint8_t *type_flag, const uint8_t *gen, const int64_t *t, int n_protein, int n_lig,
                     int n_graphs, int num_classes, const float *alphas_cumprod, const float *betas, float rho, float gamma,
                     float *losses, float *scal, float *gstats, float *a_pos, float *a_int, float *b_com, float *b_int,
                     float *z_atom, int32_t *bad, void *stream);
int cbgx_diffbp_loss_knn(const float *x_out, const float *x_in, const float *x_stack, const float *logits, const int64_t *sort_idx,
                         const int32_t *graph_ptr, const uint8_t *lig_flag, const float *pos_noise, const float *com_noise,
                         const int64_t *v0, const uint8_t *type_flag, const uint8_t *gen, const int64_t *t, int n_protein, int n_lig,
                         int n_graphs, int num_classes, const float *alphas_cumprod, const float *betas, float rho, float gamma,
                         float *losses, float *scal, float *gstats, float *a_pos, float *a_int, float *b_com, float *b_int,
                         float *z_atom, int32_t *bad, float *knn_scratch, void *stream);
int cbgx_diffbp_train_noise(const float *x0, const int64_t *v0, const int64_t *t, const uint8_t *gen, const float *eps, const float *u,
                            const int64_t *sort_idx, const int32_t *graph_ptr, int n_protein, int n_lig, int n_graphs,
                            int num_classes, const float *alphas_cumprod, int num_timesteps, int absorbing_state, float *x_t,
                            float *pos_noise, float *com_noise, int64_t *v_t, float *c_t, uint8_t *type_flag, void *stream);

int cbgx_compose_plan(const int64_t *batch_protein, const int64_t *batch_ligand, int n_protein, int n_ligand, int n_graphs,
                      int32_t *scratch, int64_t *sort_idx, int64_t *batch_idx, uint8_t *lig_flag, int64_t *lig_rows,
                      int32_t *graph_ptr, void *stream);

int cbgx_diffsbdd_train_noise(const float *x0, const float *x_protein, const int64_t *v0, const float *eps_x, const float *eps_c,
                              const uint8_t *gen, const int64_t *t, const int64_t *sort_idx, const int32_t *graph_ptr, int n_protein,
                              int n_lig, int n_graphs, int num_classes, const float *alpha_table, const float *sigma_table,
                              int num_timesteps, float *x_t, float *x_protein_t, float *c_t, float *gdata, void *stream);
int cbgx_diffsbdd_loss(const float *x_out, const float *logits, const float *eps_x, const float *eps_c, const int64_t *t,
                       const int64_t *sort_idx, const int32_t *graph_ptr, int n_protein, int n_lig, int n_graphs, int num_classes,
                       const float *gdata, float *glosses, float *losses, float *x_pred, float *c_pred, float *grad_pos,
                       float *grad_logit, void *stream);

int cbgx_embed_compose(const float *x_protein, const float *x_ligand, const float *protein_feat, const int64_t *protein_aa,
                       const float *ligand_feat, const int64_t *sort_idx, const uint8_t *gen_protein, const uint8_t *gen_ligand,
                       int n_protein, int n_ligand, int feat_dim, int num_aa, int lig_dim, const float *const *params, float *x,
                       float *h, float *ext, uint8_t *gen_flag, void *stream);
int cbgx_embed_compose_backward(const float *grad_h, const float *ext, int n_nodes, int feat_dim, int num_aa, int lig_dim,
                                float *partial, int groups, float *grad_out, void *stream);

#define CBGX_GEOMETRY_MAX_LIGAND 1024
#define CBGX_GEOMETRY_GRAPH_COLS 6
#define CBGX_GEOM_STABLE 1u
#define CBGX_GEOM_INTER_CLASH 2u
#define CBGX_GEOM_INTRA_CLASH 4u
#define CBGX_GEOM_UNKNOWN_ELEMENT 8u
int cbgx_ligand_geometry(const float *x_lig, const uint8_t *z_lig, const int32_t *lig_ptr, int n_lig, const float *x_rec,
                         const uint8_t *z_rec, const int32_t *rec_ptr, int n_rec, int n_graphs, int32_t *nr_bonds, uint8_t *flags,
                         int32_t *graph_out, void *stream);
int cbgx_ligand_geometry_tables(int32_t *bond_pm, int32_t *margins, int32_t *allowed, uint8_t *elements, uint8_t *vdw_z, double *vdw_r,
                                double *tolerance);

#define CBGX_BONDS_GRAPH_COLS 6
int cbgx_ligand_bonds_count(const float *x_lig, const uint8_t *z_lig, const int32_t *lig_ptr, int n_lig, int n_graphs, int32_t *deg_up,
                            int32_t *fragment, int32_t *graph_out, void *stream);
int cbgx_ligand_bonds_fill(const float *x_lig, const uint8_t *z_lig, const int32_t *lig_ptr, int n_lig, int n_graphs,
                           const int32_t *bond_ptr, int n_bonds, int32_t *bond_index, uint8_t *bond_order, double *bond_length,
                           void *stream);

#define CBGX_RINGS_MAX_SIZE 9
#define CBGX_RINGS_MAX_ATOMS 256
#define CBGX_RINGS_MAX_CYCLES 128
#define CBGX_RINGS_GRAPH_COLS 13
#define CBGX_RINGS_TOO_MANY_ATOMS 1
#define CBGX_RINGS_TOO_MANY_CYCLES 2
#define CBGX_RINGS_BAD_BONDS 4
int cbgx_ligand_rings(const int32_t *lig_ptr, int n_lig, int n_graphs, const int32_t *bond_ptr, const int32_t *bond_index, int n_bonds,
                      uint8_t *atom_ring_min, int32_t *graph_out, void *stream);

#define CBGX_AROMATIC_MAX_ATOMS 256
#define CBGX_AROMATIC_MAX_CYCLES 128
#define CBGX_AROMATIC_GRAPH_COLS 10
#define CBGX_AROMATIC_TOO_MANY_ATOMS 1
#define CBGX_AROMATIC_TOO_MANY_CYCLES 2
#define CBGX_AROMATIC_BAD_BONDS 4
#define CBGX_AROMATIC_NO_RINGS 8
#define CBGX_AROMATIC_BOND_TYPES 256
#define CBGX_AROMATIC_ANGLE_TYPES 8192
int cbgx_ligand_aromatic(const uint8_t *z_lig, const uint8_t *flag_lig, const uint8_t *atom_ring_min, const int32_t *lig_ptr, int n_lig,
                         int n_graphs, const int32_t *bond_ptr, const int32_t *bond_index, int n_bonds, uint8_t *atom_out,
                         uint8_t *bond_aromatic, int32_t *graph_out, void *stream);

#define CBGX_PAIR_HIST_MAX_EDGES 255
#define CBGX_ANGLES_MAX_EDGES 254
#define CBGX_ANGLES_MAX_PER_GRAPH 16384
#define CBGX_ANGLE_BIN_DEGENERATE 255
#define CBGX_ANGLE_TYPES 4608
#define CBGX_DISTRIBUTIONS_TOO_MANY_ANGLES 1
int cbgx_ligand_pair_hist(const float *x_lig, const uint8_t *z_lig, const int32_t *lig_ptr, int n_lig, int n_graphs,
                          const double *edges_all, int n_edges_all, const double *edges_cc, int n_edges_cc, int32_t *pair_hist,
                          void *stream);
int cbgx_ligand_angles(const float *x_lig, const uint8_t *z_lig, const int32_t *lig_ptr, int n_lig, int n_graphs, const int32_t *adj_ptr,
                       const int32_t *adj_nbr, const uint8_t *adj_order, int n_adj, const int32_t *angle_ptr, int n_angles,
                       const double *cos_edges, int n_cos_edges, int32_t *angle_index, double *angle_cos, uint8_t *angle_bin,
                       int16_t *angle_type, void *stream);

#define CBGX_PROFILE_CLASSES 12
int cbgx_profile_begin(int max_launches);
int cbgx_profile_end(double *ms_by_class, int *launches_by_class, int num_classes);

#ifdef __cplusplus
}
#endif
#endif
```

Measured before the change: 30040 graph-steps/s.

## Cache layer-0/1 node projections across reverse-diffusion steps, recomputing only changed rows

Adds a per-batch step cache that keeps the layer 0 and 1 node-stage projections (P, q) and hidden buffers across denoising steps. Each step recomputes only the rows that could have changed: ligand rows for layer 0, and for layer 1 the rows dirty now or dirty in the previous step. The static-context hidden copy also skips rows still valid from the previous step. This removes redundant per-step node-projection work on receptor rows, at the cost of extra device memory, list-building jobs and flag bookkeeping. Correctness depends on the dirty-set logic covering every row whose inputs changed.

```diff
diff --git a/cbgbench_amd/_native.py b/cbgbench_amd/_native.py
--- a/cbgbench_amd/_native.py
+++ b/cbgbench_amd/_native.py
@@ -25,6 +25,11 @@
     "cbgx_unitransformer_forward_v2": (_i, [_vp, _i, _i, _vp, _vp, _vp, _vp, _vp, _i, _i, _vp, _vp, _vp, ctypes.c_uint, _vp, _sz, _vp]),
     "cbgx_unitransformer_forward_cached": (_i, [_vp, _i, _i, _vp, _vp, _vp, _vp, _vp, _i, _i, _vp, _vp, _vp, _vp, _vp, _vp,
                                                 _vp, _vp, _vp, ctypes.c_uint, _vp, _sz, _vp]),
+    "cbgx_unitransformer_forward_step_cached": (_i, [_vp, _i, _i, _vp, _vp, _vp, _vp, _vp, _i, _i, _vp, _vp, _vp, _vp, _vp, _vp,
+                                                     _vp, _vp, _vp, ctypes.c_uint, _vp, _sz, _vp, _sz, _vp]),
+    "cbgx_step_cache_bytes": (_sz, [_i]),
+    "cbgx_step_cache_reset": (_i, [_vp, _sz, _i, _vp]),
+    "cbgx_step_cache_layout": (_i, [_i, ctypes.POINTER(_sz)]),
     "cbgx_knn_graph": (_i, [_vp, _vp, _i, _i, _i, _vp, _vp, _vp]),
     "cbgx_edge_gate": (_i, [_vp, _vp, _vp, _vp, _i, _vp, _vp]),
     "cbgx_x2h_attention": (_i, [_vp, _i, _vp, _vp, _vp, _vp, _vp, _vp, _i, _vp, _vp, _sz, _vp]),
diff --git a/cbgbench_amd/csrc/api.hip b/cbgbench_amd/csrc/api.hip
--- a/cbgbench_amd/csrc/api.hip
+++ b/cbgbench_amd/csrc/api.hip
@@ -45,6 +45,7 @@
     NodeList D1, S1, D2, S2;
     NodeList all_gen, all_pp, D2_gen, D2_pp, A1_gen, A1_pp, A2_gen, A2_pp;
     NodeList empty;
+    int* step_count[2];
     uint8_t *fa1, *fa2, *fa3, *fD1, *fD2, *fS1, *fS2;
     uint8_t* d1flag;
     float *hbuf[2], *xbuf[2];
@@ -86,7 +87,9 @@
     counts(256, {&w.A1, &w.A2, &w.A3});
     counts(512, {&w.D1, &w.S1, &w.D2, &w.S2});
     counts(768, {&w.all_gen, &w.all_pp, &w.D2_gen, &w.D2_pp, &w.A1_gen, &w.A1_pp, &w.A2_gen, &w.A2_pp});
-    counts(768 + 4 * 128, {&w.empty});
+    NodeList step_l0, step_u1;
+    counts(768 + 4 * 128, {&w.empty, &step_l0, &step_u1});
+    w.step_count[0] = step_l0.count; w.step_count[1] = step_u1.count;
     w.total = c.off;
     return w;
 }
@@ -95,6 +98,36 @@
     w = carve(workspace, n_nodes);
     if (workspace_bytes < w.total) return fail(CBGX_E_WORKSPACE, "%s: workspace %zu < %zu", who, workspace_bytes, w.total);
     return CBGX_OK;
+}
+
+struct StepCache {
+    float *P[2], *q[2], *hbuf[2];
+    NodeList L0, U1;
+    uint8_t *fresh0, *prevD1, *prevD2;
+    size_t flag_stride, total;
+};
+static StepCache carve_step_cache(void* base, int n) {
+    StepCache c;
+    Carver k(base);
+    const size_t N = (size_t)(n > 0 ? n : 1);
+    for (int l = 0; l < 2; ++l) {
+        c.P[l] = k.take<float>(N * PROW * 4);
+        c.q[l] = k.take<float>(N * H * 4);
+        c.hbuf[l] = k.take<float>(N * H * 4);
+    }
+    c.L0.rows = k.take<int>(N * 4);
+    c.U1.rows = k.take<int>(N * 4);
+    c.L0.count = c.U1.count = nullptr;
+    c.flag_stride = align_up(N);
+    c.fresh0 = k.take<uint8_t>(3 * c.flag_stride);
+    c.prevD1 = c.fresh0 + c.flag_stride;
+    c.prevD2 = c.prevD1 + c.flag_stride;
+    c.total = k.off;
+    return c;
+}
+static bool step_cache_enabled() {
+    static const bool on = [] { const char* e = getenv("CBGX_STEP_CACHE"); return !e || atoi(e) != 0; }();
+    return on;
 }
 
 constexpr int MAX_AUX = 8;
@@ -493,6 +526,7 @@
     NodeList gen, pp;
     bool full_layer;
     const uint8_t* fold_flag;
+    NodeList node;
 };
 
 struct Forward {
@@ -500,10 +534,13 @@
     int n_nodes, n_graphs; float *x_out, *h_out, *logits;
     const float *static_h1, *static_h2; const int32_t *static_nbr, *static_deg; const float *static_ew, *static_r32sq;
     unsigned flags; void* workspace; size_t workspace_bytes; hipStream_t s;
+    void* step_block = nullptr; size_t step_block_bytes = 0;
     Workspace w;
     Graph graph;
     bool cached, graph_cached, prune, dual;
     bool h2x_lig;
+    bool step;
+    StepCache sc;
     std::vector<LayerPlan> plan;
 };
 
@@ -517,8 +554,9 @@
         return CBGX_OK;
     }
     HIP_TRY(launch_graph_cache_begin(f.x, f.graph_ptr, n_graphs, f.lig_flag, f.static_r32sq, n_nodes, w.fD1, w.D1.rows, w.D1.count,
-                                     f.static_nbr, f.static_deg, f.static_ew, w.nbr, w.deg, w.e_w, f.static_h1, f.static_h2, w.hbuf[0],
-                                     w.hbuf[1], s));
+                                     f.static_nbr, f.static_deg, f.static_ew, w.nbr, w.deg, w.e_w, f.static_h1, f.static_h2,
+                                     f.step ? f.sc.hbuf[0] : w.hbuf[0], f.step ? f.sc.hbuf[1] : w.hbuf[1], s,
+                                     f.step ? f.sc.prevD1 : nullptr, f.step ? f.sc.prevD2 : nullptr));
     static const int merge_gate = [] { const char* e = getenv("CBGX_MERGE_GATE"); return e ? atoi(e) : 1; }();
     if (merge_gate && n_nodes <= GRAPH_LISTS_MAX_NODES) {
         HIP_TRY(launch_knn_merge_gate(f.packed, f.x, f.graph_ptr, n_graphs, n_nodes, f.lig_flag, f.static_nbr, f.static_deg, f.static_ew,
@@ -565,6 +603,17 @@
         add(GF_S1, GF_ALL, 0, w.S1);
         add(GF_S2, GF_ALL, 0, w.S2);
     }
+    if (f.step) {
+        auto add_ptr = [&](const uint8_t* flag, const uint8_t* flag2, NodeList l) {
+            if (jobs.n_jobs >= LIST_JOBS_MAX) { jobs_overflow = true; return; }
+            const int k = jobs.n_jobs++;
+            jobs.flag[k] = flag; jobs.flag2[k] = flag2; jobs.want2[k] = 0; jobs.list[k] = l.rows; jobs.count[k] = l.count;
+        };
+        add_ptr(f.lig_flag, nullptr, f.sc.L0);
+        add_ptr(f.sc.fresh0, f.lig_flag, f.sc.L0);
+        add_ptr(w.fD1, nullptr, f.sc.U1);
+        add_ptr(f.sc.prevD1, w.fD1, f.sc.U1);
+    }
     if (f.dual) {
         pair(GF_ALL, w.all_gen, w.all_pp);
         if (f.cached) pair(GF_D2, w.D2_gen, w.D2_pp);
@@ -582,6 +631,10 @@
         }
         HIP_TRY(launch_build_lists(jobs, f.n_nodes, s));
     }
+    if (f.step) {
+        HIP_TRY(hipMemsetAsync(f.sc.fresh0, 0, f.sc.flag_stride, s));
+        HIP_TRY(hipMemcpyAsync(f.sc.prevD1, w.fD1, 2 * f.sc.flag_stride, hipMemcpyDeviceToDevice, s));
+    }
     return CBGX_OK;
 }
 
@@ -589,20 +642,20 @@
     const Workspace& w = f.w;
     const int L = f.num_layers;
     const NodeList every{nullptr, nullptr};
-    f.plan.assign(L, LayerPlan{every, every, w.all_gen, w.all_pp, true, w.d1flag});
+    f.plan.assign(L, LayerPlan{every, every, w.all_gen, w.all_pp, true, w.d1flag, every});
     if (f.cached) {
-        f.plan[0] = LayerPlan{w.D1, w.S1, w.D1, w.empty, false, nullptr};
-        f.plan[1] = LayerPlan{w.D2, w.S2, w.D2_gen, w.D2_pp, false, w.d1flag};
+        f.plan[0] = LayerPlan{w.D1, w.S1, w.D1, w.empty, false, nullptr, f.step ? f.sc.L0 : every};
+        f.plan[1] = LayerPlan{w.D2, w.S2, w.D2_gen, w.D2_pp, false, w.d1flag, f.step ? f.sc.U1 : every};
     }
     if (f.prune) {
-        f.plan[L - 2] = LayerPlan{w.A2, w.A3, w.A2_gen, w.A2_pp, false, w.d1flag};
-        f.plan[L - 1] = LayerPlan{w.A1, w.A2, w.A1_gen, w.A1_pp, false, w.d1flag};
+        f.plan[L - 2] = LayerPlan{w.A2, w.A3, w.A2_gen, w.A2_pp, false, w.d1flag, every};
+        f.plan[L - 1] = LayerPlan{w.A1, w.A2, w.A1_gen, w.A1_pp, false, w.d1flag, every};
     }
 }
 
 static hipError_t begin_layer(const Forward& f, int l, float*& hn, float*& xn) {
     const bool last = l == f.num_layers - 1;
-    hn = (last && f.h_out) ? f.h_out : f.w.hbuf[l & 1];
+    hn = (last && f.h_out) ? f.h_out : ((f.step && l < 2) ? f.sc.hbuf[l] : f.w.hbuf[l & 1]);
     xn = last ? f.x_out : f.w.xbuf[l & 1];
     if (!f.cached || l >= 2 || f.graph_cached) return hipSuccess;
     return hipMemcpyAsync(hn, l == 0 ? f.static_h1 : f.static_h2, (size_t)f.n_nodes * H * sizeof(float), hipMemcpyDeviceToDevice, f.s);
@@ -618,7 +671,14 @@
     o.large_lists = true;
     o.fold = p.gen;
     o.q_direct = node_qdirect_enabled();
+    if (p.node.rows) {
+        o.dst_all_columns = true;
+        return launch_node_mfma(f.packed + x2h_off(l), h_in, f.lig_flag, f.n_nodes, b, p.node, {}, on, o);
+    }
     return launch_node_mfma(f.packed + x2h_off(l), h_in, f.lig_flag, f.n_nodes, b, p.dst, p.src, on, o);
+}
+static NodeBufs bufs_x2h(const Forward& f, int l, const NodeBufs& set) {
+    return (f.step && l < 2) ? NodeBufs{f.sc.P[l], f.sc.q[l], set.Qt} : set;
 }
 static hipError_t block_h2x(const Forward& f, int l, const NodeBufs& b, const float* xc, const float* hn, float* xn) {
     return launch_attention(false, f.packed + h2x_off(l), f.graph, xc, hn, b, xn, nullptr, f.w.act, f.w.A1, f.s, f.h2x_lig);
@@ -654,17 +714,17 @@
 
 static int forward_two_streams(const Forward& f, AuxStream* aux) {
     hipStream_t s = f.s;
-    HIP_TRY(node_x2h(f, 0, f.w.set[0], f.h, s));
+    HIP_TRY(node_x2h(f, 0, bufs_x2h(f, 0, f.w.set[0]), f.h, s));
     const float *xc = f.x, *hc = f.h;
     for (int l = 0; l < f.num_layers; ++l) {
         float *hn, *xn;
         HIP_TRY(begin_layer(f, l, hn, xn));
         if (l > 0) HIP_TRY(hipStreamWaitEvent(s, aux->join, 0));
-        HIP_TRY(edge_x2h(f, l, f.w.set[l & 1], xc, hc, hn));
+        HIP_TRY(edge_x2h(f, l, bufs_x2h(f, l, f.w.set[l & 1]), xc, hc, hn));
         if (l + 1 < f.num_layers) {
             HIP_TRY(hipEventRecord(aux->fork, s));
             HIP_TRY(hipStreamWaitEvent(aux->s, aux->fork, 0));
-            HIP_TRY(node_x2h(f, l + 1, f.w.set[(l + 1) & 1], hn, aux->s));
+            HIP_TRY(node_x2h(f, l + 1, bufs_x2h(f, l + 1, f.w.set[(l + 1) & 1]), hn, aux->s));
             HIP_TRY(hipEventRecord(aux->join, aux->s));
         }
         HIP_TRY(block_h2x(f, l, f.w.set[2], xc, hn, xn));
@@ -682,8 +742,8 @@
         float *hn, *xn;
         HIP_TRY(begin_layer(f, l, hn, xn));
         if (f.dual) {
-            HIP_TRY(node_x2h(f, l, b, hc, f.s));
-            HIP_TRY(edge_x2h(f, l, b, xc, hc, hn));
+            HIP_TRY(node_x2h(f, l, bufs_x2h(f, l, b), hc, f.s));
+            HIP_TRY(edge_x2h(f, l, bufs_x2h(f, l, b), xc, hc, hn));
         } else {
             const LayerPlan& p = f.plan[l];
             HIP_TRY(launch_attention(true, f.packed + x2h_off(l), f.graph, xc, hc, b, hn, nullptr, p.dst, p.src, f.s));
@@ -711,6 +771,14 @@
     f.prune = (f.h_out == nullptr || (f.flags & CBGX_FWD_H_ON_SOURCES)) && f.num_layers >= 3;
     f.dual = g_edge_impl != 1;
     f.h2x_lig = h2x_lig_selected(f.flags);
+    f.step = f.step_block && f.graph_cached && f.dual && f.n_nodes > NODE_STAGE_MAX_ROWS && step_cache_enabled();
+    if (f.step) {
+        f.sc = carve_step_cache(f.step_block, f.n_nodes);
+        if (f.step_block_bytes < f.sc.total)
+            return fail(CBGX_E_WORKSPACE, "forward: step cache %zu < %zu", f.step_block_bytes, f.sc.total);
+        f.sc.L0.count = f.w.step_count[0];
+        f.sc.U1.count = f.w.step_count[1];
+    }
     if (int rc = forward_graph_stage(f)) return rc;
     if (int rc = forward_list_stage(f)) return rc;
     plan_layers(f);
@@ -753,6 +821,43 @@
     return forward_impl(Forward{packed, num_layers, num_classes, x, h, graph_ptr, lig_flag, gen_flag, n_nodes, n_graphs, x_out,
                                 h_out, logits, static_h1, static_h2, static_nbr, static_deg, static_ew, static_r32sq, flags, workspace,
                                 workspace_bytes, (hipStream_t)stream});
+}
+
+int cbgx_unitransformer_forward_step_cached(const float* packed, int num_layers, int num_classes, const float* x,
+                                            const float* h, const int32_t* graph_ptr, const uint8_t* lig_flag,
+                                            const uint8_t* gen_flag, int n_nodes, int n_graphs, const float* static_h1,
+                                            const float* static_h2, const int32_t* static_nbr, const int32_t* static_deg,
+                                            const float* static_ew, const float* static_r32sq, float* x_out, float* h_out,
+                                            float* logits, unsigned flags, void* step_cache, size_t step_cache_bytes, void* workspace,
+                                            size_t workspace_bytes, void* stream) {
+    if (!static_h1 || !static_h2) return fail(CBGX_E_INVALID, "forward_step_cached: NULL static context");
+    Forward f{packed, num_layers, num_classes, x, h, graph_ptr, lig_flag, gen_flag, n_nodes, n_graphs, x_out,
+              h_out, logits, static_h1, static_h2, static_nbr, static_deg, static_ew, static_r32sq, flags, workspace,
+              workspace_bytes, (hipStream_t)stream};
+    f.step_block = step_cache;
+    f.step_block_bytes = step_cache_bytes;
+    return forward_impl(f);
+}
+
+size_t cbgx_step_cache_bytes(int n_nodes) {
+    if (n_nodes <= NODE_STAGE_MAX_ROWS || !step_cache_enabled()) return 0;
+    return carve_step_cache(nullptr, n_nodes).total;
+}
+
+int cbgx_step_cache_reset(void* step_cache, size_t step_cache_bytes, int n_nodes, void* stream) {
+    if (!step_cache || n_nodes < 1) return fail(CBGX_E_INVALID, "step_cache_reset: bad argument");
+    const StepCache c = carve_step_cache(step_cache, n_nodes);
+    if (step_cache_bytes < c.total) return fail(CBGX_E_WORKSPACE, "step_cache_reset: block %zu < %zu", step_cache_bytes, c.total);
+    HIP_TRY(hipMemsetAsync(c.fresh0, 1, 3 * c.flag_stride, (hipStream_t)stream));
+    return CBGX_OK;
+}
+
+int cbgx_step_cache_layout(int n_nodes, size_t* offsets) {
+    if (!offsets || n_nodes < 1) return fail(CBGX_E_INVALID, "step_cache_layout: bad argument");
+    const StepCache c = carve_step_cache(nullptr, n_nodes);
+    const void* p[CBGX_STEP_CACHE_ARRAYS] = {c.P[0], c.q[0], c.hbuf[0], c.P[1], c.q[1], c.hbuf[1], c.fresh0, c.prevD1, c.prevD2};
+    for (int k = 0; k < CBGX_STEP_CACHE_ARRAYS; ++k) offsets[k] = (size_t)reinterpret_cast<uintptr_t>(p[k]);
+    return CBGX_OK;
 }
 
 static int noise_args(const char* who, const uint64_t* keys, const int32_t* lig_graph, bool need_graph, const int32_t* lig_ptr,
diff --git a/cbgbench_amd/csrc/graph_mfma.hip b/cbgbench_amd/csrc/graph_mfma.hip
--- a/cbgbench_amd/csrc/graph_mfma.hip
+++ b/cbgbench_amd/csrc/graph_mfma.hip
@@ -535,7 +535,8 @@
     const float* __restrict__ r32sq, int n, uint8_t* __restrict__ dirty, int* __restrict__ list, int* __restrict__ count,
     const int32_t* __restrict__ s_nbr, const int32_t* __restrict__ s_deg, const float* __restrict__ s_ew,
     int32_t* __restrict__ nbr, int32_t* __restrict__ deg, float* __restrict__ ew, const float* __restrict__ h1,
-    const float* __restrict__ h2, float* __restrict__ out1, float* __restrict__ out2) {
+    const float* __restrict__ h2, float* __restrict__ out1, float* __restrict__ out2, const uint8_t* __restrict__ keep1,
+    const uint8_t* __restrict__ keep2) {
     __shared__ int s_cnt[16];
     __shared__ int s_base;
     const long t = (long)blockIdx.x * 1024 + threadIdx.x;
@@ -545,8 +546,9 @@
         if ((t & (KNN / 4 - 1)) == 0) deg[t / (KNN / 4)] = s_deg[t / (KNN / 4)];
     }
     if (t < (long)n * (H / 4)) {
-        reinterpret_cast<float4*>(out1)[t] = reinterpret_cast<const float4*>(h1)[t];
-        reinterpret_cast<float4*>(out2)[t] = reinterpret_cast<const float4*>(h2)[t];
+        const long row = t / (H / 4);
+        if (!keep1 || keep1[row]) reinterpret_cast<float4*>(out1)[t] = reinterpret_cast<const float4*>(h1)[t];
+        if (!keep2 || keep2[row]) reinterpret_cast<float4*>(out2)[t] = reinterpret_cast<const float4*>(h2)[t];
     }
     if ((long)blockIdx.x * 1024 >= n) return;
     const int i = (int)t;
@@ -604,11 +606,11 @@
 hipError_t launch_graph_cache_begin(const float* x, const int32_t* graph_ptr, int n_graphs, const uint8_t* lig, const float* r32sq,
                                     int n, uint8_t* dirty, int* list, int* count, const int32_t* s_nbr, const int32_t* s_deg,
                                     const float* s_ew, int32_t* nbr, int32_t* deg, float* ew, const float* h1, const float* h2,
-                                    float* out1, float* out2, hipStream_t s) {
+                                    float* out1, float* out2, hipStream_t s, const uint8_t* keep1, const uint8_t* keep2) {
     if (n == 0) return hipSuccess;
     const long threads = (long)n * (H / 4);
     hipLaunchKernelGGL(graph_cache_begin_kernel, dim3((unsigned)((threads + 1023) / 1024)), dim3(1024), 0, s, x, graph_ptr, n_graphs,
-                       lig, r32sq, n, dirty, list, count, s_nbr, s_deg, s_ew, nbr, deg, ew, h1, h2, out1, out2);
+                       lig, r32sq, n, dirty, list, count, s_nbr, s_deg, s_ew, nbr, deg, ew, h1, h2, out1, out2, keep1, keep2);
     return hipGetLastError();
 }
 
diff --git a/cbgbench_amd/csrc/kernels.h b/cbgbench_amd/csrc/kernels.h
--- a/cbgbench_amd/csrc/kernels.h
+++ b/cbgbench_amd/csrc/kernels.h
@@ -91,7 +91,8 @@
 hipError_t launch_graph_cache_begin(const float* x, const int32_t* graph_ptr, int n_graphs, const uint8_t* lig, const float* r32sq,
                                     int n, uint8_t* dirty, int* list, int* count, const int32_t* s_nbr, const int32_t* s_deg,
                                     const float* s_ew, int32_t* nbr, int32_t* deg, float* ew, const float* h1, const float* h2,
-                                    float* out1, float* out2, hipStream_t s);
+                                    float* out1, float* out2, hipStream_t s, const uint8_t* keep1 = nullptr,
+                                    const uint8_t* keep2 = nullptr);
 hipError_t launch_pack_node_tables(const PackBlocks& pb, hipStream_t s);
 hipError_t launch_build_active(const uint8_t* flag, int n, NodeList out, hipStream_t s, bool counter_zeroed = false);
 hipError_t launch_mark_seed(const uint8_t* a, const uint8_t* b, int n, uint8_t* m, hipStream_t s);
@@ -103,6 +104,7 @@
     RowList fold;
     bool q_direct = false;
     bool no_fold = false;
+    bool dst_all_columns = false;
 };
 hipError_t launch_node_mfma(const float* att, const float* h, const uint8_t* lig, int n_nodes, const NodeBufs& b, RowList dst,
                             RowList src, hipStream_t s, const NodeStageOpts& o = {});
diff --git a/cbgbench_amd/csrc/node_mfma.hip b/cbgbench_amd/csrc/node_mfma.hip
--- a/cbgbench_amd/csrc/node_mfma.hip
+++ b/cbgbench_amd/csrc/node_mfma.hip
@@ -1352,7 +1352,8 @@
             hipLaunchKernelGGL(node_proj_kernel<false>, proj_grid(chunks_all), dim3(256), 0, s, att, h, lig, b.P, n_nodes,
                                (const int*)nullptr, (const int*)nullptr, chunks_all);
     } else {
-        if (!two_jobs) {
+        if (o.dst_all_columns && !fused) {
+        } else if (!two_jobs) {
             if (src.rows)
                 hipLaunchKernelGGL(node_proj_kernel<true>, proj_grid(CHUNKS_PS), dim3(256), 0, s, att, h, lig, b.P, n_nodes, src.rows,
                                    src.count, CHUNKS_PS);
@@ -1361,8 +1362,11 @@
                                    (const int*)nullptr, (const int*)nullptr, CHUNKS_PS);
         }
         if (!fused)
-            hipLaunchKernelGGL(node_proj_kernel<true>, proj_grid(chunks_own), dim3(256), 0, s, att, h, lig, b.P, n_nodes, dst.rows, dst.count,
-                               chunks_own);
+        {
+            const unsigned chunks_dst = o.dst_all_columns ? chunks_all : chunks_own;
+            hipLaunchKernelGGL(node_proj_kernel<true>, proj_grid(chunks_dst), dim3(256), 0, s, att, h, lig, b.P, n_nodes, dst.rows, dst.count,
+                               chunks_dst);
+        }
     }
     profile_mark_end(s);
     hipError_t e = hipGetLastError();
diff --git a/cbgbench_amd/sampling.py b/cbgbench_amd/sampling.py
--- a/cbgbench_amd/sampling.py
+++ b/cbgbench_amd/sampling.py
@@ -83,7 +83,7 @@
         h[rec_rows] = self.context_embedder.embed_protein(v_rec, F.one_hot(batch["protein_aa_type"], NUM_AA).float())
         st = {"B": B, "N": n_rec + n_lig, "n_lig": n_lig, "x": x, "h": h, "bl": bl, "br": br, "gen_l": gen_l, "batch_idx": batch_idx,
               "lig_flag": lig_flag, "gen_flag": gen_flag, "lig_rows": lig_rows, "rec_rows": rec_rows, "graph_ptr": graph_ptr,
-              "traj_x": None, "traj_c": None, "static_h": None}
+              "traj_x": None, "traj_c": None, "static_h": None, "step_cache": None}
         st["gen_is_ligand"] = not bool(gen_r.any())
         csr = "lig_ptr" in self._step_operands
         if pocket_order:
@@ -106,6 +106,7 @@
         st["x_lig"], st["c_lig"] = x_lig.contiguous(), c_lig.contiguous()
         if dev.type == "cuda" and static_cache and st["gen_is_ligand"]:
             st["static_h"] = self.denoiser.static_context(x_rec, st["h"][rec_rows], st["br"], rec_rows, st["N"])
+            st["step_cache"] = None if st["static_h"] is None else self.denoiser.new_step_cache(st["N"], dev)
         if keep_trajectory:
             st["traj_x"] = torch.empty(T + 1, st["n_lig"], 3, dtype=torch.float32, device=dev)
             st["traj_c"] = torch.empty(T + 1, st["n_lig"], self.num_classes, dtype=torch.float32, device=dev)
@@ -132,7 +133,7 @@
     def _run_denoiser(self, st, need_h=True, h_on_sources=False, workspace=None):
         return self.denoiser(x=st["x"], h=st["h"], batch_idx=st["batch_idx"], lig_flag=st["lig_flag"], gen_flag=st["gen_flag"],
                              graph_ptr=st["graph_ptr"], need_h=need_h, static_h=st["static_h"], workspace=workspace,
-                             h_on_sources=h_on_sources, gen_is_ligand=st["gen_is_ligand"])
+                             h_on_sources=h_on_sources, gen_is_ligand=st["gen_is_ligand"], step_cache=st.get("step_cache"))
 
     def _trajectory(self, st, out_dev, final=None):
         traj_x, traj_c, bl_out = st["traj_x"].to(out_dev), st["traj_c"].to(out_dev), st["bl"].to(out_dev)
diff --git a/cbgbench_amd/unitransformer.py b/cbgbench_amd/unitransformer.py
--- a/cbgbench_amd/unitransformer.py
+++ b/cbgbench_amd/unitransformer.py
@@ -316,6 +316,16 @@
         r32sq[rec_rows] = r32
         return (out[0], out[1], nbr.contiguous(), deg, ew, r32sq)
 
+    @staticmethod
+    def new_step_cache(n_nodes, device):
+        lib = _native.lib()
+        need = lib.cbgx_step_cache_bytes(n_nodes)
+        if need == 0:
+            return None
+        block = torch.empty(need, dtype=torch.uint8, device=device)
+        _native.check(lib.cbgx_step_cache_reset(_native.ptr(block), need, n_nodes, _native.current_stream(device)), "cbgx_step_cache_reset")
+        return block
+
     def _as_u8(self, flag):
         if flag.dtype == torch.uint8:
             return flag.contiguous()
@@ -332,7 +342,7 @@
         return u8
 
     def forward(self, x, h, batch_idx, lig_flag, gen_flag, graph_ptr=None, need_h=True, static_h=None,
-                ligand_outputs_only=False, workspace=None, h_on_sources=False, gen_is_ligand=False):
+                ligand_outputs_only=False, workspace=None, h_on_sources=False, gen_is_ligand=False, step_cache=None):
         if not x.is_cuda:
             raise RuntimeError("UniTransformer.forward runs on an MI355X through libcbgx; got a CPU tensor "
                                "(no CPU fallback exists; use oracle/ for CPU reference results)")
@@ -361,7 +371,15 @@
         logits = torch.empty(N, self.out_classes, dtype=torch.float32, device=device)
         lib = _native.lib()
         flags = _native.FWD_GEN_IS_LIGAND if gen_is_ligand else 0
-        if static_h is not None:
+        if static_h is not None and step_cache is not None:
+            rc = lib.cbgx_unitransformer_forward_step_cached(
+                _native.ptr(packed), self.num_layers, self.out_classes, _native.ptr(x), _native.ptr(h),
+                _native.ptr(graph_ptr), _native.ptr(lig), _native.ptr(gen), N, B, _native.ptr(static_h[0]),
+                _native.ptr(static_h[1]), *[_native.ptr(t) for t in static_h[2:6]], _native.ptr(x_out),
+                _native.ptr(h_out), _native.ptr(logits), flags | (_native.FWD_H_ON_SOURCES if (h_on_sources and need_h) else 0),
+                _native.ptr(step_cache), step_cache.numel(), _native.ptr(ws), ws.numel(),
+                _native.current_stream(device))
+        elif static_h is not None:
             rc = lib.cbgx_unitransformer_forward_cached(
                 _native.ptr(packed), self.num_layers, self.out_classes, _native.ptr(x), _native.ptr(h),
                 _native.ptr(graph_ptr), _native.ptr(lig), _native.ptr(gen), N, B, _native.ptr(static_h[0]),
diff --git a/include/cbgx.h b/include/cbgx.h
--- a/include/cbgx.h
+++ b/include/cbgx.h
@@ -56,6 +56,20 @@
                                        const float *static_ew, const float *static_r32sq,
                                        float *x_out, float *h_out, float *logits, unsigned flags,
                                        void *workspace, size_t workspace_bytes, void *stream);
+
+#define CBGX_STEP_CACHE_ARRAYS 9
+size_t cbgx_step_cache_bytes(int n_nodes);
+int cbgx_step_cache_reset(void *step_cache, size_t step_cache_bytes, int n_nodes, void *stream);
+int cbgx_step_cache_layout(int n_nodes, size_t *offsets);
+int cbgx_unitransformer_forward_step_cached(const float *packed, int num_layers, int num_classes,
+                                            const float *x, const float *h, const int32_t *graph_ptr,
+                                            const uint8_t *lig_flag, const uint8_t *gen_flag, int n_nodes, int n_graphs,
+                                            const float *static_h1, const float *static_h2,
+                                            const int32_t *static_nbr, const int32_t *static_deg,
+                                            const float *static_ew, const float *static_r32sq,
+                                            float *x_out, float *h_out, float *logits, unsigned flags,
+                                            void *step_cache, size_t step_cache_bytes,
+                                            void *workspace, size_t workspace_bytes, void *stream);
 
 
 int cbgx_knn_graph(const float *x, const int32_t *graph_ptr, int n_graphs, int n_nodes, int k,
```

Result: faster. 30510 graph-steps/s (median of 6 runs) (+1.6%).
